# frankyeh/UNet-Studio

Measured on AMD Instinct MI355X. Metric: voxels/sec 3D U-Net train step @128^3 bf16, higher is better.
Workload: dtype bf16

## Files before the change

include/unet.hpp:

```cpp
#ifndef UNET_HPP
#define UNET_HPP
#ifdef QT_CORE_LIB
    #undef slots
#endif
#include <torch/torch.h>
#ifdef QT_CORE_LIB
    #define slots Q_SLOTS
#endif
#include <array>
#include <deque>
#include <map>
#include <mutex>
#include <string>
#include <vector>

#if __has_include("TIPL/tipl.hpp")
#include "TIPL/tipl.hpp"
namespace unet_types { typedef tipl::vector<3> vector3; typedef tipl::shape<3> shape3; }
#else
namespace unet_types {
struct vector3 {
    float v[3];
    vector3(float x = 1.f, float y = 1.f, float z = 1.f) : v{x, y, z} {}
    float& operator[](size_t i) { return v[i]; }
    const float& operator[](size_t i) const { return v[i]; }
};
struct shape3 {
    unsigned v[3];
    shape3(unsigned x = 0, unsigned y = 0, unsigned z = 0) : v{x, y, z} {}
    unsigned& operator[](size_t i) { return v[i]; }
    const unsigned& operator[](size_t i) const { return v[i]; }
    size_t size() const { return (size_t)v[0] * v[1] * v[2]; }
};
inline std::ostream& operator<<(std::ostream& o, const vector3& a) { return o << a[0] << " " << a[1] << " " << a[2]; }
inline std::ostream& operator<<(std::ostream& o, const shape3& a) { return o << a[0] << " " << a[1] << " " << a[2]; }
}
#endif

struct unet_plan;
struct unet_comm;

struct UNet3dImpl : torch::nn::Module
{
public:
    int in_count = 1;
    int out_count = 1;
    std::string architecture,preproc,postproc,orientation,fov_strategy,error_msg;
public:
    std::shared_ptr<torch::optim::SGD> optimizer;

    std::vector<float> testing_errors,training_errors;
    std::vector<unsigned int> single_component_label;
    mutable std::mutex error_mutex;
    auto get_training_errors(void) const
    {
        std::scoped_lock<std::mutex> lock(error_mutex);
        return std::vector<float>(training_errors);
    }
    auto get_testing_errors(void) const
    {
        std::scoped_lock<std::mutex> lock(error_mutex);
        return std::vector<float>(testing_errors);
    }

public:
    unet_types::vector3 voxel_size = {1.0f,1.0f,1.0f};
    unet_types::shape3 dim = {192,224,192};
    std::deque<torch::nn::Sequential> encoding,decoding,decoding_tail;
    std::vector<torch::nn::Sequential> output;
    int create_layer(torch::nn::Sequential& layers,const std::string& def, int in_c);
public:
    std::string get_info(void) const;
public:
    UNet3dImpl(void){}
    UNet3dImpl(int32_t in_count_,int32_t out_count_,std::string);
    ~UNet3dImpl(void);
    void copy_from(const UNet3dImpl& r);
    void add_gradient_from(const UNet3dImpl& r);
    void create_optimizer(float learning_rate);
public:
    std::vector<torch::Tensor> forward(torch::Tensor inputTensor);

    void set_requires_grad(bool req)
    {
        for (auto& p : parameters())
            p.set_requires_grad(req);
    }
    virtual void train(bool on = true) override
    {
        set_requires_grad(on);
        torch::nn::Module::train(on);
    }
    void print_layers(void);
    torch::Device device(void) const
    {
        return parameters().size() && parameters()[0].defined() ? parameters()[0].device() : torch::kCPU;
    }
    void prepare_for_inference(const torch::Device& device);

public:
    size_t pooled_workspaces(void) const;
    int engine_dtype = 1;
    torch::Tensor flat_params, flat_grads;
    void to_device(const torch::Device& device);
    torch::Tensor loss_and_backward(torch::Tensor input, torch::Tensor target_int64, bool ce, bool dice, bool mse, int collapse_before = 0);
    void sgd_step(float lr, float grad_scale, float clip_norm = 12.0f);
    void bind_optimizer_state(void);
    bool save_optimizer(const std::string& file_name);
    bool load_optimizer(const std::string& file_name);
    void attach_comm(struct unet_comm* comm) { comm_ = comm; reduced_from_ = -1; }
    void broadcast_parameters(int root = 0);
    void broadcast_buffers(int root = 0);
    void allreduce_gradients(void);
    torch::Tensor loss_and_backward_overlapped(torch::Tensor input, torch::Tensor target_int64, bool ce, bool dice, bool mse, int collapse_before = 0);
private:
    friend struct UNetForwardFn;
    std::vector<torch::Tensor> params_, buffers_;
    std::map<std::array<int64_t,3>, unet_plan*> plans_;
    struct WorkspacePool;
    std::shared_ptr<WorkspacePool> ws_pool_;
    std::mutex plans_mutex_;
    torch::Tensor trigger_, momentum_, scratch_;
    struct unet_comm* comm_ = nullptr;
    int64_t reduced_from_ = -1;
    unet_plan* plan_for(int64_t d,int64_t h,int64_t w);
    torch::Tensor workspace_for(unet_plan* plan);
    void bind_views(void);
    void ensure_flat(void);
    void rebind_grads(void);
    std::vector<torch::Tensor> run_forward(unet_plan* plan, torch::Tensor ws, torch::Tensor x, int mode);
    void run_backward(unet_plan* plan, torch::Tensor ws, const std::vector<torch::Tensor>& grad_outs);
};
TORCH_MODULE_IMPL(UNet3d, UNet3dImpl);

bool save_to_file(UNet3d& model,const char* file_name);
bool load_from_file(UNet3d& model,const char* file_name);


#endif
```

include/unet_hip.h:

```cpp
#ifndef UNET_HIP_H
#define UNET_HIP_H
#include <stddef.h>
#include <stdint.h>

#ifdef __cplusplus
extern "C" {
#endif

#define UNET_DTYPE_F32 0
#define UNET_DTYPE_BF16 1

#define UNET_IMPL_AUTO 0
#define UNET_IMPL_DIRECT 1

typedef struct unet_plan unet_plan;

const char* unet_last_error(void);
void unet_set_error(const char* msg);

int unet_init(int* n_devices);
int unet_device_info(int device, char* name, size_t name_len, size_t* total_mem, int* compute_units, int* gcn_arch_is_gfx950);

int unet_plan_create(const char* arch_dsl, int in_c, int out_c, int D, int H, int W, int dtype, int device, int impl,
                     unet_plan** out);
void unet_plan_destroy(unet_plan* plan);

int unet_plan_param_count(const unet_plan* plan, int* n);
int unet_plan_param_shape(const unet_plan* plan, int i, int64_t dims[5], int* ndim);
int unet_plan_param_name(const unet_plan* plan, int i, char* name, size_t name_len);
int unet_plan_param_decay(const unet_plan* plan, int i, int* decay);
int unet_plan_param_fan_in(const unet_plan* plan, int i, int64_t* fan_in, int* is_norm_weight);
int unet_plan_buffer_count(const unet_plan* plan, int* n);
int unet_plan_buffer_shape(const unet_plan* plan, int i, int64_t* numel);
int unet_plan_output_count(const unet_plan* plan, int* n);
int unet_plan_output_shape(const unet_plan* plan, int level, int64_t dims[5]);
int unet_plan_workspace_bytes(const unet_plan* plan, size_t* bytes);
int unet_plan_flops(const unet_plan* plan, double* fwd, double* bwd);
size_t unet_plan_describe(const unet_plan* plan, char* buf, size_t len);

int unet_plan_op_count(const unet_plan* plan, int* n);
int unet_plan_op_info(const unet_plan* plan, int i, int* kind, int* cin, int* cout, int* ks, int* stride, int64_t in_dims[3],
                      int64_t out_dims[3], char* name, size_t name_len);

#define UNET_PROF_CONV_FWD 0
#define UNET_PROF_DGRAD 1
#define UNET_PROF_WGRAD 2
#define UNET_PROF_NORM_FWD 3
#define UNET_PROF_NORM_BWD 4
#define UNET_PROF_OTHER 5
int unet_profile_begin(void);
int unet_profile_end(int max_records, int* op_index, int* category, float* ms, int* n_records);

#define UNET_MODE_PACKS_CURRENT 2
int unet_forward(const unet_plan* plan, const float* const* params, float* const* buffers, const float* x,
                 float* const* outs, void* workspace, int mode, void* stream);

int unet_backward(const unet_plan* plan, const float* const* params, const float* const* grad_outs,
                  float* const* grad_params, float* grad_x, void* workspace, void* stream);

int unet_plan_backward_buckets(const unet_plan* plan, int max_buckets, int* n_buckets, int* op_lo, int64_t* elem_lo);
int unet_backward_part(const unet_plan* plan, const float* const* params, const float* const* grad_outs, float* const* grad_params,
                       float* grad_x, void* workspace, int op_hi, int op_lo, void* stream);

int unet_loss_scratch_bytes(const unet_plan* plan, size_t* bytes);
int unet_loss(const unet_plan* plan, const float* const* outs, const int64_t* target, int cost_mask, int collapse_before,
              float* const* grad_outs, float* losses_out, void* scratch, void* stream);

int unet_forward_loss(const unet_plan* plan, const float* const* params, float* const* buffers, const float* x, float* const* outs,
                      const int64_t* target, int cost_mask, int collapse_before, float* const* grad_outs, float* losses_out,
                      void* loss_scratch, void* workspace, void* stream);
int unet_forward_loss_mode(const unet_plan* plan, const float* const* params, float* const* buffers, const float* x, float* const* outs,
                           const int64_t* target, int cost_mask, int collapse_before, float* const* grad_outs, float* losses_out,
                           void* loss_scratch, void* workspace, int mode, void* stream);

int unet_stream_create_cu_range(int device, int cu_first, int cu_count, void** stream);
int unet_stream_destroy(void* stream);
int unet_plan_side_cu_range(unet_plan* plan, int cu_first, int cu_count);

int unet_pack_filters(const unet_plan* plan, const float* const* params, void* workspace, int with_dgrad, int* made, void* stream);

#define UNET_SUM_MAX_BUFFERS 64
int unet_sum_buffers(const float* const* bufs, int n, float* out, int64_t count, int zero_inputs, void* stream);

int unet_sgd_step(const unet_plan* plan, float* params_flat, float* grads_flat, float* momentum_flat, float lr,
                  float momentum, int nesterov, float weight_decay, float clip_norm, float grad_scale, float* norm_out,
                  void* scratch, void* stream);

int unet_op_scratch_bytes(int cin, int cout, int D, int H, int W, size_t* bytes);
int unet_op_conv3d_fwd(int dtype, int impl, const void* x, const float* w, const float* b, void* y, int cin, int cout, int D,
                       int H, int W, int ks, int stride, void* scratch, void* stream);
int unet_op_conv3d_fwd_fused(int dtype, int impl, const void* x, const float* scale, const float* shift, int act, const float* w,
                             const float* b, void* y, float* stats, int cin, int cout, int D, int H, int W, int ks, int stride,
                             void* scratch, void* stream);
int unet_op_conv3d_pack(int dtype, const float* w, void* wpacked, int cin, int cout, int D, int H, int W, int ks, int stride,
                        void* stream);
int unet_op_conv3d_fwd_packed(int dtype, const void* x, const void* wpacked, const float* b, void* y, float* stats_partials,
                              int cin, int cout, int D, int H, int W, int ks, int stride, void* stream);
int unet_op_conv3d_bwd_data(int dtype, int impl, const void* dy, const float* w, void* dx, int cin, int cout, int D, int H,
                            int W, int ks, int stride, void* scratch, void* stream);
int unet_op_conv3d_fwd_norm(const void* x0, const void* x1, int cin0, int cin1, const float* w, const float* b, const float* gamma,
                            const float* beta, double eps, float* rm, float* rv, double momentum, int use_running, int act, void* y,
                            void* y_act, float* stat, int cout, int D, int H, int W, int stride, void* scratch, void* stream);
int unet_op_conv3d_bwd_data_norm(int transposed, const void* dy, const float* w, void* dx, int accumulate, const void* u, const float* stat,
                                 const float* gamma, int act, float* coef, float* dgamma, float* dbeta, int cin, int cout, int D, int H,
                                 int W, void* scratch, void* stream);
int unet_op_conv3d_bwd_weight(int dtype, int impl, const void* x, const void* dy, float* dw, float* db, int cin, int cout,
                              int D, int H, int W, int ks, int stride, void* scratch, void* stream);
int unet_op_convt_fwd(int dtype, int impl, const void* x, const float* w, const float* b, void* y, int cin, int cout, int D,
                      int H, int W, void* scratch, void* stream);
int unet_op_convt_bwd_data(int dtype, int impl, const void* dy, const float* w, void* dx, int cin, int cout, int D, int H,
                           int W, void* scratch, void* stream);
int unet_op_convt_bwd_weight(int dtype, int impl, const void* x, const void* dy, float* dw, float* db, int cin, int cout,
                             int D, int H, int W, void* scratch, void* stream);
int unet_op_pack_ndhwc(int dtype, const float* x_ncdhw, void* y_ndhwc, int C, int64_t S, void* stream);
int unet_op_unpack_ncdhw(int dtype, const void* x_ndhwc, float* y_ncdhw, int C, int64_t S, void* stream);

#define UNET_COMM_ID_BYTES 128
typedef struct unet_comm unet_comm;
int unet_comm_unique_id(void* id_bytes );
int unet_comm_create(int rank, int world, const void* id_bytes, int device, unet_comm** out);
int unet_comm_create_all(int n, const int* devices, unet_comm** out );
int unet_comm_destroy(unet_comm* comm);
int unet_comm_rank(const unet_comm* comm, int* rank, int* world);
int unet_allreduce_grads(unet_comm* comm, float* flat, int64_t elem_lo, int64_t elem_hi, void* stream);
int unet_allreduce_grads_all(unet_comm* const* comms, int n, float* const* flats, int64_t elem_lo, int64_t elem_hi, void* const* streams);
int unet_comm_broadcast(unet_comm* comm, float* buf, int64_t n, int root, void* stream);
int unet_comm_join(unet_comm* comm, void* stream);

#ifdef __cplusplus
}
#endif
#endif
```

unet-studio_amd/csrc/engine.cpp:

```cpp
#include <hip/hip_runtime.h>

#include <algorithm>
#include <atomic>
#include <cmath>
#include <cstdio>
#include <cstring>
#include <functional>
#include <stdexcept>
#include <string>
#include <mutex>
#include <random>
#include <unordered_map>
#include <vector>

#include "../../include/unet_hip.h"
#include "conv_select.h"
#include "graph.hpp"
#include "kernels.h"

using namespace unet;

namespace {

thread_local std::string g_err;
int fail(const std::string& m) { g_err = m; return 1; }

#define HIP_OK(expr)                                                                              \
    do {                                                                                          \
        hipError_t e_ = (expr);                                                                   \
        if (e_ != hipSuccess) throw std::runtime_error(std::string(#expr) + ": " + hipGetErrorString(e_)); \
    } while (0)

struct DeviceGuard {
    int prev = -1;
    explicit DeviceGuard(int dev) {
        HIP_OK(hipGetDevice(&prev));
        if (prev != dev) HIP_OK(hipSetDevice(dev));
        else prev = -1;
    }
    ~DeviceGuard() { if (prev >= 0) (void)hipSetDevice(prev); }
};

size_t align_up(size_t v, size_t a = 256) { return (v + a - 1) / a * a; }

struct EnvSwitches {
    bool no_side_stream = getenv("UNET_NO_SIDE_STREAM"), no_first_wgrad_fuse = getenv("UNET_NO_FIRST_WGRAD_FUSE"), op_polite = getenv("UNET_OP_POLITE");
};
const EnvSwitches& env() { static const EnvSwitches e; return e; }

struct ProfRec { int op, cat; hipEvent_t e0, e1; };
struct ProfSink { std::vector<ProfRec> recs; };
thread_local ProfSink* g_prof = nullptr;
struct ProfScope {
    ProfRec r{};
    hipStream_t s = nullptr;
    bool on = false;
    ProfScope(int op, int cat, hipStream_t st) {
        if (!g_prof) return;
        on = true; s = st; r.op = op; r.cat = cat;
        if (hipEventCreate(&r.e0) != hipSuccess || hipEventCreate(&r.e1) != hipSuccess) { on = false; return; }
        (void)hipEventRecord(r.e0, s);
    }
    ~ProfScope() {
        if (!on) return;
        (void)hipEventRecord(r.e1, s);
        g_prof->recs.push_back(r);
    }
};

}

struct unet_plan {
    Graph g;
    int dtype = 0, device = 0, impl = 0;
    size_t elsize = 4;
    std::vector<size_t> t_off, g_off;
    std::vector<size_t> a_off;
    std::vector<size_t> n_stat, n_coef;
    std::vector<size_t> w_fwd, w_dgrad;
    std::vector<size_t> wm_fwd, wm_dgrad;
    std::vector<int> n_consumers;
    std::vector<int> first_consumer;
    mutable std::mutex bn_mu;
    mutable std::unordered_map<const void*, std::pair<int, int>> bn_pending;
    mutable std::unordered_map<const void*, std::vector<int>> bn_done;
    std::vector<ConvChoice> conv;
    size_t wgrad_off = 0;
    std::vector<size_t> wz_off;
    std::vector<int> wz_job_of_op;
    std::vector<WgradReduceJob> wz_jobs;
    WgradReduceJob* wz_jobs_dev = nullptr;
    size_t partial_off = 0, partial_bytes = 0;
    size_t ws_bytes = 0;
    size_t loss_bytes = 0;
    std::vector<int64_t> p_off;
    std::vector<PackJob> pack_jobs;
    int64_t pack_blocks = 0;
    PackJob* jobs_dev = nullptr;
    SgdSeg* segs_dev = nullptr;
    int nseg = 0;
    int64_t n_param_elems = 0;

    hipStream_t side = nullptr;
    hipEvent_t ev_fork = nullptr, ev_join = nullptr, ev_pack = nullptr, ev_packd = nullptr;
    int pack_split_op = 0;
    int64_t pack_split_blocks = 0, pack_fwd_blocks = 0;
    size_t head_off = 0;
    size_t deep_part_off = 0, deep_part_bytes = 0, deep_cnt_off = 0;
    static constexpr int deep_ncnt = 4096;
    std::vector<size_t> head_op_off;

    ~unet_plan() {
        if (segs_dev) (void)hipFree(segs_dev);
        if (wz_jobs_dev) (void)hipFree(wz_jobs_dev);
        if (jobs_dev) (void)hipFree(jobs_dev);
        if (ev_fork) (void)hipEventDestroy(ev_fork);
        if (ev_join) (void)hipEventDestroy(ev_join);
        if (ev_pack) (void)hipEventDestroy(ev_pack);
        if (ev_packd) (void)hipEventDestroy(ev_packd);
        if (side) (void)hipStreamDestroy(side);
    }

    ConvGeom op_geom_of(const Op& op) const {
        const Tensor& a = g.tensors[op.src[0]];
        const Tensor& o = g.tensors[op.dst];
        ConvGeom cg;
        cg.Cin = op.cin; cg.Cout = op.cout; cg.D = a.D; cg.H = a.H; cg.W = a.W; cg.Do = o.D; cg.Ho = o.H; cg.Wo = o.W;
        cg.ks = op.ks; cg.stride = op.stride;
        return cg;
    }
    void src_chans(const Op& op, SrcDesc* sd) const {
        for (int k = 0; k < op.nsrc; ++k) sd[k].C = g.tensors[op.src[k]].C;
    }
    std::vector<int> side_polite;
    std::vector<char> wgrad_on_main;
    void choose_polite() {
        side_polite.assign(g.ops.size(), 0);
        wgrad_on_main.assign(g.ops.size(), 0);
        bool first = true, any_deep = false;
        for (size_t i = 0; i < g.ops.size(); ++i) {
            const Op& op = g.ops[i];
            if (op.kind != OP_CONV && op.kind != OP_CONVT) continue;
            if (g.tensors[op.dst].voxels() <= (int64_t)32 * 32 * 32) { any_deep = true; break; }
            if (!first && op.kind == OP_CONV && op.stride == 2) wgrad_on_main[i] = 1;
            first = false;
        }
        if (!any_deep) return;
        for (size_t i = 0; i < g.ops.size(); ++i) {
            const Op& op = g.ops[i];
            if (op.kind == OP_CONV || op.kind == OP_CONVT) side_polite[i] = wgrad_on_main[i] ? 0 : 1;
        }
    }

    bool head_only(size_t t) const {
        if (dtype != UNET_DTYPE_BF16 || g.tensors[t].norm < 0 || g.tensors[t].C % 16) return false;
        int readers = 0;
        for (size_t i = 0; i < g.ops.size(); ++i) {
            const Op& op = g.ops[i];
            if (op.kind == OP_NORM) continue;
            for (int k = 0; k < op.nsrc; ++k) {
                if (op.src[k] != (int)t) continue;
                if (conv[i].fwd != Fwd::head) return false;
                ++readers;
            }
        }
        return readers > 0;
    }
    void layout() {
        choose_polite();
        conv.assign(g.ops.size(), ConvChoice());
        for (size_t i = 0; i < g.ops.size(); ++i) {
            const Op& op = g.ops[i];
            if (op.kind != OP_CONV && op.kind != OP_CONVT) continue;
            SrcDesc sd[2];
            src_chans(op, sd);
            conv[i] = choose_conv(dtype, impl, op_geom_of(op), sd, op.nsrc, op.out_level >= 0, op.kind == OP_CONVT);
        }
        size_t off = 0;
        auto take = [&](size_t bytes) { size_t o = off; off = align_up(off + bytes); return o; };
        t_off.assign(g.tensors.size(), SIZE_MAX);
        g_off.assign(g.tensors.size(), SIZE_MAX);
        n_consumers.assign(g.tensors.size(), 0);
        first_consumer.assign(g.tensors.size(), -1);
        for (size_t oi = 0; oi < g.ops.size(); ++oi) {
            const Op& op = g.ops[oi];
            for (int k = 0; k < op.nsrc && op.kind != OP_NORM; ++k)
                if (op.src[k] >= 0) { ++n_consumers[op.src[k]]; if (first_consumer[op.src[k]] < 0) first_consumer[op.src[k]] = (int)oi; }
        }
        a_off.assign(g.tensors.size(), SIZE_MAX);
        for (size_t i = 0; i < g.tensors.size(); ++i) {
            t_off[i] = take((size_t)g.tensors[i].numel() * elsize);
            if (g.tensors[i].needs_grad) g_off[i] = take((size_t)g.tensors[i].numel() * elsize);
            if (impl == UNET_IMPL_AUTO && (g.tensors[i].norm >= 0 || g.tensors[i].act != ACT_NONE) && !head_only(i))
                a_off[i] = take((size_t)g.tensors[i].numel() * elsize);
        }
        n_stat.resize(g.norms.size()); n_coef.resize(g.norms.size());
        size_t pmax = 0;
        for (size_t i = 0; i < g.norms.size(); ++i) {
            n_stat[i] = take(4 * (size_t)g.norms[i].C * 4);
            n_coef[i] = take(3 * (size_t)g.norms[i].C * 4);
            size_t pb = (size_t)stats_blocks(g.tensors[g.norms[i].tensor].voxels()) * g.norms[i].C * 2 * (dtype == UNET_DTYPE_F32 ? 8 : 4);
            if (pb > pmax) pmax = pb;
        }
        w_fwd.assign(g.ops.size(), SIZE_MAX); w_dgrad.assign(g.ops.size(), SIZE_MAX);
        wm_fwd.assign(g.ops.size(), SIZE_MAX); wm_dgrad.assign(g.ops.size(), SIZE_MAX);
        auto grow = [](size_t& m, size_t b) { if (b > m) m = b; };
        for (size_t i = 0; i < g.ops.size(); ++i) {
            const Op& op = g.ops[i];
            if (op.kind != OP_CONV && op.kind != OP_CONVT) continue;
            const ConvChoice& c = conv[i];
            const ConvGeom cg = op_geom_of(op);
            int k3 = op.kind == OP_CONV ? op.ks * op.ks * op.ks : 8;
            w_fwd[i] = take((size_t)k3 * op.cin * round_up(op.cout, 8) * 4);
            w_dgrad[i] = take((size_t)k3 * op.cout * round_up(op.cin, 8) * 4);
            if (op.kind == OP_CONVT) {
                if (c.mfma_fwd()) { wm_fwd[i] = take(mfma_convt_w_bytes(cg)); wm_dgrad[i] = take(mfma_convt_dgrad_w_bytes(cg)); }
                continue;
            }
            const bool stats = g.tensors[op.dst].norm >= 0;
            SrcDesc sd[2];
            src_chans(op, sd);
            if (c.mfma_fwd()) {
                wm_fwd[i] = take(mfma_conv_w_bytes(cg));
                if (stats) grow(pmax, (size_t)mfma_conv_blocks(cg) * op.cout * 2 * 4);
            }
            if (c.fwd == Fwd::first_f32_mfma && stats) grow(pmax, (size_t)conv_first_f32_mfma_blocks(cg) * op.cout * 2 * 8);
            if (c.fwd == Fwd::f32_mfma && stats) grow(pmax, (size_t)conv_f32_mfma_stat_rows(cg, sd) * op.cout * 2 * 8);
            if (c.dgrad == Dgrad::mfma) {
                wm_dgrad[i] = take(mfma_conv_dgrad_w_bytes(cg));
                if (op.stride == 2) grow(pmax, (size_t)s2_conv_dgrad_rows_max() * op.cin * 2 * 4);
            }
        }
        partial_bytes = pmax ? pmax : 256;
        partial_off = take(partial_bytes);
        size_t wmax = 0, hmax = 0;
        for (size_t i = 0; i < g.ops.size(); ++i) {
            const Op& op = g.ops[i];
            if (op.kind != OP_CONV && op.kind != OP_CONVT) continue;
            const ConvChoice& c = conv[i];
            const ConvGeom cg = op_geom_of(op);
            grow(wmax, wgrad_direct_scratch_bytes(cg, op.kind == OP_CONVT));
            if (op.kind == OP_CONVT) {
                if (c.wgrad == Wgrad::mfma) {
                    grow(wmax, mfma_convt_wgrad_scratch_bytes(cg));
                    grow(wmax, bias_grad_scratch_bytes(cg.Cout, (int64_t)cg.Do * cg.Ho * cg.Wo));
                }
                continue;
            }
            if (c.wgrad == Wgrad::mfma) grow(wmax, mfma_wgrad_scratch_bytes(cg, side_polite[i]));
            if (c.wgrad == Wgrad::f32_mfma) grow(wmax, wgrad_f32_mfma_scratch_bytes(cg));
            if (wgrad_small_supported(cg, op.nsrc)) grow(wmax, wgrad_small_scratch_bytes(cg));
            if (cg.Cin == 1 && (cg.Cout == 16 || cg.Cout == 32)) grow(wmax, conv_first_wgrad_mfma_scratch_bytes(cg));
            if (head_supported(cg, op.nsrc)) grow(hmax, head_bwd_scratch_bytes(cg));
        }
        wgrad_off = take(wmax ? wmax : 256);
        head_off = take(hmax ? hmax : 256);
        if (dtype == UNET_DTYPE_BF16 && impl == UNET_IMPL_AUTO) {
            deep_part_bytes = (size_t)8 << 20;
            deep_part_off = take(deep_part_bytes);
            deep_cnt_off = take((size_t)deep_ncnt * 4);
        }
        head_op_off.assign(g.ops.size(), SIZE_MAX);
        for (size_t i = 0; i < g.ops.size(); ++i)
            if (conv[i].fwd == Fwd::head) head_op_off[i] = take(head_bwd_scratch_bytes(op_geom_of(g.ops[i])));
        wz_off.assign(g.ops.size(), SIZE_MAX);
        for (size_t i = 0; i < g.ops.size(); ++i) {
            const Op& op = g.ops[i];
            const Wgrad w = conv[i].wgrad;
            if (op.out_level >= 0 || (w != Wgrad::first_mfma && w != Wgrad::mfma)) continue;
            const ConvGeom cg = op_geom_of(op);
            if (w == Wgrad::first_mfma) wz_off[i] = take(conv_first_wgrad_mfma_scratch_bytes(cg));
            else if (op.kind == OP_CONV) { if (!mfma_conv_wgrad_direct(cg)) wz_off[i] = take(mfma_wgrad_scratch_bytes(cg, side_polite[i])); }
            else if (!mfma_convt_wgrad_direct(cg)) wz_off[i] = take(mfma_convt_wgrad_scratch_bytes(cg));
        }
        ws_bytes = off;
        p_off.assign(g.params.size() + 1, 0);
        for (size_t i = 0; i < g.params.size(); ++i) {
            int64_t n = 1;
            for (auto d : g.params[i].shape) n *= d;
            p_off[i + 1] = p_off[i] + n;
        }
        wz_jobs.clear();
        wz_job_of_op.assign(g.ops.size(), -1);
        int wz_blk = 0;
        for (size_t i = 0; i < g.ops.size(); ++i) {
            if (wz_off[i] == SIZE_MAX) continue;
            const Op& op = g.ops[i];
            ConvGeom cg = op_geom_of(op);
            WgradReduceJob j;
            j.op = (int)i;
            j.slab_off = (long long)(wz_off[i] / 4);
            j.dw_off = p_off[op.weight];
            j.Cb = op.cout;
            if (op.kind == OP_CONVT) {
                j.nsplit = mfma_convt_wgrad_splits(cg);
                j.n = (long long)8 * op.cin * op.cout;
                j.bias_off = op.bias >= 0 ? j.slab_off + (long long)j.nsplit * j.n : -1;
                j.db_off = op.bias >= 0 ? p_off[op.bias] : -1;
            } else {
                j.nsplit = conv[i].wgrad == Wgrad::first_mfma ? conv_first_wgrad_splits(cg) : mfma_conv_wgrad_splits(cg, side_polite[i]);
                j.n = (long long)27 * op.cin * op.cout;
                j.bias_off = op.bias >= 0 ? j.slab_off + (long long)j.nsplit * j.n : -1;
                j.db_off = op.bias >= 0 ? p_off[op.bias] : -1;
            }
            wz_blk += wgrad_reduce_job_blocks(j, wz_blk);
            wz_job_of_op[i] = (int)wz_jobs.size();
            wz_jobs.push_back(j);
        }
        pack_jobs.clear();
        pack_blocks = 0;
        pack_split_op = -1; pack_split_blocks = 0; pack_fwd_blocks = 0;
        for (int which = 0; which < 2; ++which) {
            for (size_t i = 0; i < g.ops.size(); ++i) {
                const Op& op = g.ops[i];
                if (!conv[i].mfma_fwd()) continue;
                if (which == 0 && pack_split_op < 0 && g.tensors[op.dst].voxels() <= (int64_t)16 * 16 * 16) { pack_split_op = (int)i; pack_split_blocks = pack_blocks; }
                PackJob jb[2];
                int n = op.kind == OP_CONV ? mfma_conv_pack_jobs(op_geom_of(op), conv[i].dgrad == Dgrad::mfma, jb) : mfma_convt_pack_jobs(op_geom_of(op), jb);
                if (which >= n) continue;
                jb[which].src_off = p_off[op.weight];
                jb[which].dst_off = (int64_t)(which == 0 ? wm_fwd[i] : wm_dgrad[i]);
                jb[which].blk0 = pack_blocks;
                pack_blocks += jb[which].total;
                pack_jobs.push_back(jb[which]);
            }
            if (which == 0) pack_fwd_blocks = pack_blocks;
        }
    }
};

namespace {

void norm_fwd_passes(int dtype, const void* raw, int C, int64_t S, float* partial, int rows, bool dbl, bool eval, const float* gamma,
                     const float* beta, double eps, float* stat, float* rm, float* rv, int act, void* act_out, hipStream_t s) {
    if (eval) launch_norm_eval(C, gamma, beta, rm, rv, eps, stat, s);
    else {
        if (!rows) {
            launch_stats_partial(dtype, raw, C, S, partial, s);
            rows = stats_blocks(S);
            dbl = dtype == UNET_DTYPE_F32;
        }
        if (!dbl && act_out && launch_norm_finalize_apply(dtype, partial, rows, C, S, gamma, beta, eps, stat, rm, rv, 0.1, raw, act, act_out, s))
            return;
        launch_norm_finalize(partial, rows, C, S, gamma, beta, eps, stat, rm, rv, 0.1, s, dbl);
    }
    if (act_out) {
        SrcDesc d;
        d.ptr = raw; d.C = C; d.act = act; d.scale = stat + 2 * C; d.shift = stat + 3 * C;
        launch_apply_view(dtype, d, act_out, S, s);
    }
}
void norm_bwd_passes(int dtype, void* g, const void* u, int C, int64_t S, const float* stat, int act, const float* gamma, float* coef,
                     float* dgamma, float* dbeta, float* partial, int rows, bool no_apply, hipStream_t s) {
    if (rows <= 0) {
        launch_norm_bwd_partial(dtype, g, u, C, S, stat, act, partial, s);
        rows = stats_blocks(S);
    }
    if (!no_apply && launch_norm_bwd_finalize_apply(dtype, partial, rows, C, S, gamma, stat, coef, dgamma, dbeta, g, u, act, s)) return;
    launch_norm_bwd_finalize(partial, rows, C, S, gamma, stat, coef, dgamma, dbeta, s, dtype == UNET_DTYPE_F32);
    if (!no_apply) launch_norm_bwd_apply(dtype, g, u, C, S, stat, coef, act, s);
}

struct Exec {
    const unet_plan& p;
    char* ws;
    hipStream_t s;
    bool deep_on = false;
    Exec(const unet_plan& plan, void* workspace, void* stream) : p(plan), ws((char*)workspace), s((hipStream_t)stream) {}
    DeepScratch deep() const {
        DeepScratch d;
        if (deep_on && p.deep_part_bytes) { d.part = (float*)(ws + p.deep_part_off); d.part_bytes = p.deep_part_bytes; d.cnt = (int*)(ws + p.deep_cnt_off); d.ncnt = p.deep_ncnt; }
        return d;
    }
    int* deep_cnt() const { return p.deep_part_bytes ? (int*)(ws + p.deep_cnt_off) : nullptr; }

    void* tptr(int t) const { return ws + p.t_off[t]; }
    void* gptr(int t) const { return p.g_off[t] == SIZE_MAX ? nullptr : ws + p.g_off[t]; }
    float* stat(int n) const { return (float*)(ws + p.n_stat[n]); }
    float* coef(int n) const { return (float*)(ws + p.n_coef[n]); }
    float* partial() const { return (float*)(ws + p.partial_off); }

    SrcDesc raw_src(int t) const {
        const Tensor& T = p.g.tensors[t];
        SrcDesc d;
        d.ptr = tptr(t); d.C = T.C; d.act = T.act;
        if (T.norm >= 0) { d.scale = stat(T.norm) + 2 * T.C; d.shift = stat(T.norm) + 3 * T.C; }
        return d;
    }
    SrcDesc src(int t) const {
        if (p.a_off[t] == SIZE_MAX) return raw_src(t);
        SrcDesc d;
        d.ptr = ws + p.a_off[t]; d.C = p.g.tensors[t].C;
        return d;
    }
    void apply_view(int t) const {
        if (p.a_off[t] != SIZE_MAX) launch_apply_view(p.dtype, raw_src(t), ws + p.a_off[t], p.g.tensors[t].voxels(), s);
    }
    ConvGeom geom(const Op& op) const { return p.op_geom_of(op); }

    void forward(const float* const* params, float* const* buffers, const float* x, float* const* outs, int mode,
                 const std::function<void(int)>* on_head = nullptr) {
        const Graph& g = p.g;
        const bool packs_current = (mode & UNET_MODE_PACKS_CURRENT) != 0;
        mode &= 1;
        std::vector<int> fused_blocks(g.norms.size(), 0);
        std::vector<char> fused_dbl(g.norms.size(), 0);
        std::vector<char> fused_done(g.norms.size(), 0);
        bool packed = false, pack_pending = false, pack2_pending = false;
        if (p.jobs_dev && packs_current) { packed = true; deep_on = true; }
        else if (p.jobs_dev) {
            bool flat = true;
            for (size_t i = 0; i < g.params.size() && flat; ++i) flat = params[i] == params[0] + p.p_off[i];
            if (flat) {
                const int njobs = (int)p.pack_jobs.size();
                if (mode == 1 && p.side && !env().no_side_stream && !g_prof) {
                    HIP_OK(hipEventRecord(p.ev_fork, s));
                    HIP_OK(hipStreamWaitEvent(p.side, p.ev_fork, 0));
                    if (p.pack_split_op > 0 && p.pack_split_blocks > 0) {
                        launch_mfma_pack_batched(params[0], ws, p.jobs_dev, njobs, p.pack_split_blocks, p.side, 0, 0, deep_cnt(), p.deep_ncnt);
                        HIP_OK(hipEventRecord(p.ev_join, p.side));
                        launch_mfma_pack_batched(params[0], ws, p.jobs_dev, njobs, p.pack_fwd_blocks - p.pack_split_blocks, p.side, p.pack_split_blocks);
                        HIP_OK(hipEventRecord(p.ev_pack, p.side));
                        pack2_pending = true;
                        launch_mfma_pack_batched(params[0], ws, p.jobs_dev, njobs, p.pack_blocks - p.pack_fwd_blocks, p.side, p.pack_fwd_blocks);
                        HIP_OK(hipEventRecord(p.ev_packd, p.side));
                    } else {
                        launch_mfma_pack_batched(params[0], ws, p.jobs_dev, njobs, p.pack_blocks, p.side, 0, 0, deep_cnt(), p.deep_ncnt);
                        HIP_OK(hipEventRecord(p.ev_join, p.side));
                    }
                    pack_pending = true;
                } else {
                    ProfScope ps(-1, UNET_PROF_OTHER, s);
                    launch_mfma_pack_batched(params[0], ws, p.jobs_dev, njobs, mode == 1 ? p.pack_blocks : p.pack_fwd_blocks, s, 0, 0, deep_cnt(), p.deep_ncnt);
                }
                packed = true;
                deep_on = true;
            }
        }
        auto need_packs = [&](int op_index = 1 << 30) {
            if (pack_pending) { HIP_OK(hipStreamWaitEvent(s, p.ev_join, 0)); pack_pending = false; }
            if (pack2_pending && op_index >= p.pack_split_op) { HIP_OK(hipStreamWaitEvent(s, p.ev_pack, 0)); pack2_pending = false; }
        };
        for (size_t i = 0; i < g.ops.size(); ++i) {
            const Op& op = g.ops[i];
            ProfScope ps((int)i, (op.kind == OP_CONV || op.kind == OP_CONVT) ? UNET_PROF_CONV_FWD : op.kind == OP_NORM ? UNET_PROF_NORM_FWD : UNET_PROF_OTHER, s);
            switch (op.kind) {
                case OP_PACK_INPUT:
                    launch_pack_input(p.dtype, x, tptr(op.dst), g.in_c, g.tensors[op.dst].voxels(), s);
                    break;
                case OP_CONV:
                case OP_CONVT: {
                    if (op.out_level >= 0 && !(outs && outs[op.out_level])) break;
                    SrcDesc sd[2] = {src(op.src[0]), op.nsrc > 1 ? src(op.src[1]) : SrcDesc()};
                    ConvGeom cg = geom(op);
                    float* wf = (float*)(ws + p.w_fwd[i]);
                    float* wd = (float*)(ws + p.w_dgrad[i]);
                    const int k3 = op.ks * op.ks * op.ks;
                    const ConvChoice& c = p.conv[i];
                    const Tensor& T = g.tensors[op.dst];
                    const bool want_stats = T.norm >= 0 && !(g.norms[T.norm].batch && mode == 0);
                    if (op.kind == OP_CONVT) {
                        if (c.mfma_fwd()) {
                            need_packs((int)i);
                            if (!packed) launch_mfma_pack_convt_w(params[op.weight], ws + p.wm_fwd[i], mode == 1 ? ws + p.wm_dgrad[i] : nullptr, cg, s);
                            if (!(deep_on && launch_deep_convt_fwd(cg, sd, op.nsrc, ws + p.wm_fwd[i], params[op.bias], tptr(op.dst), deep(), s)))
                                launch_mfma_convt_fwd(cg, sd, op.nsrc, ws + p.wm_fwd[i], params[op.bias], tptr(op.dst), s);
                            break;
                        }
                        if (!packs_current) launch_pack_convt_w(params[op.weight], wf, wd, op.cin, op.cout, s);
                        if (c.fwd == Fwd::f32_mfma) launch_convt_f32_mfma(cg, sd, wf, params[op.bias], (float*)tptr(op.dst), s);
                        else launch_convt_fwd_direct(p.dtype, cg, sd, op.nsrc, wf, params[op.bias], tptr(op.dst), s);
                        break;
                    }
                    float* const part = want_stats ? partial() : nullptr;
                    int rows = 0;
                    switch (c.fwd) {
                        case Fwd::deep:
                        case Fwd::mfma:
                            need_packs((int)i);
                            if (!packed)
// ... 278 lines not shown
                            if (can) {
                                const Norm& n = g.norms[Ts.norm];
                                nb = {tptr(ts), stat(Ts.norm), params[n.gamma], coef(Ts.norm), gparams[n.gamma], gparams[n.beta], Ts.act};
                            }
                            if (op.kind == OP_CONVT) {
                                int norm_done = 0;
                                if (deep_on && launch_deep_convt_dgrad(cg, gptr(t), ws + p.wm_dgrad[i], dg, op.nsrc, can ? &nb : nullptr, deep(), &norm_done, s)) {
                                    if (norm_done) { std::lock_guard<std::mutex> lk(p.bn_mu); p.bn_done[ws].push_back(ts); }
                                } else
                                    launch_mfma_convt_dgrad(cg, gptr(t), ws + p.wm_dgrad[i], dg, op.nsrc, s);
                                break;
                            }
                            BnBwdStats bn = {tptr(ts), Ts.norm >= 0 ? stat(Ts.norm) : nullptr, partial(), Ts.act, Ts.C};
                            int rows = 0;
                            const int served = deep_on ? launch_deep_conv_dgrad(cg, gptr(t), ws + p.wm_dgrad[i], dg, op.nsrc, can ? &nb : nullptr, deep(), s) : 0;
                            if (served == 2) { std::lock_guard<std::mutex> lk(p.bn_mu); p.bn_done[ws].push_back(ts); }
                            if (!served) rows = launch_mfma_conv_dgrad(cg, gptr(t), ws + p.wm_dgrad[i], dg, op.nsrc, s, can ? &bn : nullptr);
                            if (rows > 0) { std::lock_guard<std::mutex> lk(p.bn_mu); p.bn_pending[ws] = {ts, rows}; }
                            break;
                        }
                        case Dgrad::f32_mfma: launch_conv_f32_mfma_dgrad(cg, (const float*)gptr(t), wd, dg, op.nsrc, s); break;
                        case Dgrad::direct:
                            if (op.kind == OP_CONVT) launch_convt_dgrad_direct(p.dtype, cg, gptr(t), wd, dg, op.nsrc, s);
                            else launch_conv_dgrad_direct(p.dtype, cg, gptr(t), wd, dg, op.nsrc, s);
                            break;
                    }
                    if (any) mark(op);
                    break;
                }
                case OP_MATERIALIZE: {
                    DstGrad dg[2] = {dst_of(op.src[0]), op.nsrc > 1 ? dst_of(op.src[1]) : DstGrad()};
                    if (dg[0].ptr || (op.nsrc > 1 && dg[1].ptr)) {
                        if (!dry) launch_materialize_bwd(p.dtype, gptr(t), dg, op.nsrc, g.tensors[t].voxels(), s);
                        mark(op);
                    }
                    break;
                }
                case OP_MAXPOOL: {
                    const Tensor& a = g.tensors[op.src[0]];
                    DstGrad d = dst_of(op.src[0]);
                    if (d.ptr) { if (!dry) launch_maxpool_bwd(p.dtype, src(op.src[0]), gptr(t), d, a.D, a.H, a.W, s); mark(op); }
                    break;
                }
                case OP_UPSAMPLE: {
                    const Tensor& a = g.tensors[op.src[0]];
                    DstGrad d = dst_of(op.src[0]);
                    if (d.ptr) { if (!dry) launch_upsample_bwd(p.dtype, gptr(t), d, a.D, a.H, a.W, s); mark(op); }
                    break;
                }
                case OP_PACK_INPUT:
                    if (!dry && (grad_x)) launch_unpack_ncdhw(p.dtype, gptr(t), grad_x, g.in_c, g.tensors[t].voxels(), s);
                    break;
                default: break;
            }
        }
        pending.insert(pending.begin(), held.begin(), held.end());
        held.clear();
        issue_pending();
        flush_wz(sb);
        if (sb != s) {
            HIP_OK(hipEventRecord(p.ev_join, sb));
            HIP_OK(hipStreamWaitEvent(s, p.ev_join, 0));
        }
    }
};

void check_launch() { HIP_OK(hipGetLastError()); }

}

extern "C" {

const char* unet_last_error(void) { return g_err.c_str(); }
void unet_set_error(const char* msg) { g_err = msg ? msg : ""; }

int unet_init(int* n_devices) {
    int n = 0;
    hipError_t e = hipGetDeviceCount(&n);
    if (e != hipSuccess) { if (n_devices) *n_devices = 0; return fail(std::string("hipGetDeviceCount: ") + hipGetErrorString(e)); }
    if (n_devices) *n_devices = n;
    return 0;
}

int unet_device_info(int device, char* name, size_t name_len, size_t* total_mem, int* compute_units, int* is_gfx950) {
    hipDeviceProp_t pr;
    hipError_t e = hipGetDeviceProperties(&pr, device);
    if (e != hipSuccess) return fail(std::string("hipGetDeviceProperties: ") + hipGetErrorString(e));
    if (name && name_len) { std::strncpy(name, pr.name, name_len - 1); name[name_len - 1] = 0; }
    if (total_mem) *total_mem = pr.totalGlobalMem;
    if (compute_units) *compute_units = pr.multiProcessorCount;
    if (is_gfx950) *is_gfx950 = std::strncmp(pr.gcnArchName, "gfx950", 6) == 0;
    return 0;
}

static bool create_cu_range_stream(int device, int cu_first, int cu_count, hipStream_t* out);
int unet_plan_create(const char* arch, int in_c, int out_c, int D, int H, int W, int dtype, int device, int impl, unet_plan** out) {
    if (!arch || !out) return fail("unet_plan_create: null argument");
    if (dtype != UNET_DTYPE_F32 && dtype != UNET_DTYPE_BF16) return fail("unet_plan_create: unknown dtype");
    unet_plan* p = nullptr;
    try {
        p = new unet_plan();
        p->g = Graph::build(arch, in_c, out_c, D, H, W);
        for (auto& n : p->g.norms) p->g.tensors[n.tensor].needs_grad = true;
        p->dtype = dtype; p->device = device; p->impl = impl; p->elsize = dtype == UNET_DTYPE_F32 ? 4 : 2;
        p->layout();
        {
            size_t off = 0;
            int oc = out_c;
            for (size_t l = 0; l < p->g.outputs.size(); ++l) {
                const auto& o = p->g.outputs[l];
                int64_t S = (int64_t)(D >> l) * (H >> l) * (W >> l);
                if (S <= 0) S = 1;
                off = align_up(off + (size_t)S * 8);
                off = align_up(off + (size_t)(4 + 2 * oc) * 4);
                (void)o;
            }
            off = align_up(off + (size_t)1024 * (3 + 2 * oc) * 4);
            off = align_up(off + (size_t)1024 * (3 + 2 * oc) * 4);
            p->loss_bytes = off;
        }
        std::vector<SgdSeg> segs;
        int64_t o = 0;
        for (auto& pr : p->g.params) {
            int64_t n = 1;
            for (auto d : pr.shape) n *= d;
            SgdSeg sg;
            sg.offset = o; sg.count = n; sg.wd = pr.decay ? 1.f : 0.f;
            segs.push_back(sg);
            o += n;
        }
        p->n_param_elems = o;
        p->nseg = (int)segs.size();
        int nd = 0;
        if (hipGetDeviceCount(&nd) == hipSuccess && nd > 0) {
            DeviceGuard dg(device);
            int pr_least = 0, pr_greatest = 0;
            (void)hipDeviceGetStreamPriorityRange(&pr_least, &pr_greatest);
            HIP_OK(hipStreamCreateWithPriority(&p->side, hipStreamNonBlocking, pr_least));
            const unsigned evf = hipEventDisableTiming | hipEventDisableSystemFence;
            HIP_OK(hipEventCreateWithFlags(&p->ev_fork, evf));
            HIP_OK(hipEventCreateWithFlags(&p->ev_join, evf));
            HIP_OK(hipEventCreateWithFlags(&p->ev_pack, evf));
            HIP_OK(hipEventCreateWithFlags(&p->ev_packd, evf));
            HIP_OK(hipMalloc((void**)&p->segs_dev, segs.size() * sizeof(SgdSeg)));
            HIP_OK(hipMemcpy(p->segs_dev, segs.data(), segs.size() * sizeof(SgdSeg), hipMemcpyHostToDevice));
            if (!p->wz_jobs.empty()) {
                HIP_OK(hipMalloc((void**)&p->wz_jobs_dev, p->wz_jobs.size() * sizeof(WgradReduceJob)));
                HIP_OK(hipMemcpy(p->wz_jobs_dev, p->wz_jobs.data(), p->wz_jobs.size() * sizeof(WgradReduceJob), hipMemcpyHostToDevice));
            }
            if (!p->pack_jobs.empty()) {
                HIP_OK(hipMalloc((void**)&p->jobs_dev, p->pack_jobs.size() * sizeof(PackJob)));
                HIP_OK(hipMemcpy(p->jobs_dev, p->pack_jobs.data(), p->pack_jobs.size() * sizeof(PackJob), hipMemcpyHostToDevice));
            }
        }
        *out = p;
        return 0;
    } catch (const std::exception& e) {
        delete p;
        return fail(e.what());
    }
}

void unet_plan_destroy(unet_plan* p) { delete p; }

int unet_plan_param_count(const unet_plan* p, int* n) { *n = (int)p->g.params.size(); return 0; }
int unet_plan_param_shape(const unet_plan* p, int i, int64_t dims[5], int* ndim) {
    if (i < 0 || i >= (int)p->g.params.size()) return fail("parameter index out of range");
    const auto& s = p->g.params[i].shape;
    *ndim = (int)s.size();
    for (size_t k = 0; k < s.size(); ++k) dims[k] = s[k];
    return 0;
}
int unet_plan_param_name(const unet_plan* p, int i, char* name, size_t name_len) {
    if (i < 0 || i >= (int)p->g.params.size()) return fail("parameter index out of range");
    if (name && name_len) { std::strncpy(name, p->g.params[i].name.c_str(), name_len - 1); name[name_len - 1] = 0; }
    return 0;
}
int unet_plan_param_decay(const unet_plan* p, int i, int* decay) {
    if (i < 0 || i >= (int)p->g.params.size()) return fail("parameter index out of range");
    *decay = p->g.params[i].decay;
    return 0;
}
int unet_plan_param_fan_in(const unet_plan* p, int i, int64_t* fan_in, int* is_norm_weight) {
    if (i < 0 || i >= (int)p->g.params.size()) return fail("parameter index out of range");
    *fan_in = p->g.params[i].fan_in; *is_norm_weight = p->g.params[i].norm_weight;
    return 0;
}
int unet_plan_buffer_count(const unet_plan* p, int* n) { *n = (int)p->g.buffers.size(); return 0; }
int unet_plan_buffer_shape(const unet_plan* p, int i, int64_t* numel) {
    if (i < 0 || i >= (int)p->g.buffers.size()) return fail("buffer index out of range");
    *numel = p->g.buffers[i];
    return 0;
}
int unet_plan_output_count(const unet_plan* p, int* n) { *n = (int)p->g.outputs.size(); return 0; }
int unet_plan_output_shape(const unet_plan* p, int l, int64_t dims[5]) {
    if (l < 0 || l >= (int)p->g.outputs.size()) return fail("output level out of range");
    const auto& o = p->g.outputs[l];
    dims[0] = 1; dims[1] = o.C; dims[2] = o.D; dims[3] = o.H; dims[4] = o.W;
    return 0;
}
int unet_plan_workspace_bytes(const unet_plan* p, size_t* bytes) { *bytes = p->ws_bytes; return 0; }
int unet_plan_flops(const unet_plan* p, double* fwd, double* bwd) { *fwd = p->g.flops_fwd; *bwd = p->g.flops_bwd; return 0; }
size_t unet_plan_describe(const unet_plan* p, char* buf, size_t len) {
    std::string d = p->g.describe();
    if (buf && len) { std::strncpy(buf, d.c_str(), len - 1); buf[len - 1] = 0; }
    return d.size() + 1;
}

int unet_forward(const unet_plan* p, const float* const* params, float* const* buffers, const float* x, float* const* outs,
                 void* workspace, int mode, void* stream) {
    try {
        if (!p || !params || !x || !workspace) throw std::runtime_error("unet_forward: null argument");
        if (mode & ~(1 | UNET_MODE_PACKS_CURRENT)) throw std::runtime_error("unet_forward: unknown mode bits (0 = eval, 1 = train, optionally | UNET_MODE_PACKS_CURRENT)");
        if (!p->g.buffers.empty() && !buffers) throw std::runtime_error("unet_forward: architecture has bnorm layers but buffers is null");
        DeviceGuard dg(p->device);
        Exec ex(*p, workspace, stream);
        ex.forward(params, buffers, x, outs, mode);
        check_launch();
        return 0;
    } catch (const std::exception& e) { return fail(e.what()); }
}

int unet_backward(const unet_plan* p, const float* const* params, const float* const* grad_outs, float* const* grad_params,
                  float* grad_x, void* workspace, void* stream) {
    try {
        if (!p || !params || !grad_params || !workspace) throw std::runtime_error("unet_backward: null argument");
        if (grad_x) throw std::runtime_error("unet_backward: grad_x must be NULL -- dL/dx is not computed (the input carries no gradient, as in train.cpp:619-628)");
        DeviceGuard dg(p->device);
        Exec ex(*p, workspace, stream);
        ex.backward(params, grad_outs, grad_params, grad_x);
        check_launch();
        return 0;
    } catch (const std::exception& e) { return fail(e.what()); }
}

int unet_backward_part(const unet_plan* p, const float* const* params, const float* const* grad_outs, float* const* grad_params,
                       float* grad_x, void* workspace, int op_hi, int op_lo, void* stream) {
    try {
        if (!p || !params || !grad_params || !workspace) throw std::runtime_error("unet_backward_part: null argument");
        if (op_lo < 0 || op_hi < op_lo) throw std::runtime_error("unet_backward_part: invalid op range");
        if (grad_x) throw std::runtime_error("unet_backward_part: grad_x must be NULL -- dL/dx is not computed");
        DeviceGuard dg(p->device);
        Exec ex(*p, workspace, stream);
        ex.backward(params, grad_outs, grad_params, grad_x, op_hi, op_lo);
        check_launch();
        return 0;
    } catch (const std::exception& e) { return fail(e.what()); }
}

int unet_plan_backward_buckets(const unet_plan* p, int max_buckets, int* n_buckets, int* op_lo, int64_t* elem_lo) {
    try {
        if (!p || !n_buckets || !op_lo || !elem_lo || max_buckets < 1) throw std::runtime_error("unet_plan_backward_buckets: bad argument");
        const Graph& g = p->g;
        const int nops = (int)g.ops.size();
        std::vector<int64_t> first(nops, INT64_MAX);
        bool monotone = true;
        int64_t prev = -1;
        for (int i = 0; i < nops; ++i) {
            const Op& op = g.ops[i];
            if (op.kind != OP_CONV && op.kind != OP_CONVT) continue;
            int64_t f = p->p_off[op.weight];
            if (op.bias >= 0 && p->p_off[op.bias] < f) f = p->p_off[op.bias];
            first[i] = f;
            if (f <= prev) monotone = false;
            prev = f;
            const Tensor& T = g.tensors[op.dst];
            if (T.norm >= 0) {
                const Norm& n = g.norms[T.norm];
                if (p->p_off[n.gamma] < f || p->p_off[n.beta] < f) monotone = false;
            }
        }
        int nb = 0;
        if (monotone && max_buckets > 1) {
            const double thr = (double)p->n_param_elems / ((double)max_buckets - 0.5);
            int64_t hi = p->n_param_elems;
            for (int i = nops - 1; i > 0 && nb < max_buckets - 1; --i) {
                if (first[i] == INT64_MAX) continue;
                if ((double)(hi - first[i]) >= thr) { op_lo[nb] = i; elem_lo[nb] = first[i]; hi = first[i]; ++nb; }
            }
        }
        op_lo[nb] = 0; elem_lo[nb] = 0; ++nb;
        *n_buckets = nb;
        return 0;
    } catch (const std::exception& e) { return fail(e.what()); }
}

int unet_plan_op_count(const unet_plan* p, int* n) { *n = (int)p->g.ops.size(); return 0; }
int unet_plan_op_info(const unet_plan* p, int i, int* kind, int* cin, int* cout, int* ks, int* stride, int64_t in_dims[3],
                      int64_t out_dims[3], char* name, size_t name_len) {
    if (i < 0 || i >= (int)p->g.ops.size()) return fail("op index out of range");
    const Op& op = p->g.ops[i];
    if (kind) *kind = (int)op.kind;
    if (cin) *cin = op.cin;
    if (cout) *cout = op.cout;
    if (ks) *ks = op.ks;
    if (stride) *stride = op.stride;
    const Tensor* a = op.nsrc > 0 && op.src[0] >= 0 ? &p->g.tensors[op.src[0]] : nullptr;
    const Tensor* o = op.dst >= 0 ? &p->g.tensors[op.dst] : nullptr;
    if (in_dims) { in_dims[0] = a ? a->D : 0; in_dims[1] = a ? a->H : 0; in_dims[2] = a ? a->W : 0; }
    if (out_dims) { out_dims[0] = o ? o->D : 0; out_dims[1] = o ? o->H : 0; out_dims[2] = o ? o->W : 0; }
    if (name && name_len) { std::strncpy(name, op.name.c_str(), name_len - 1); name[name_len - 1] = 0; }
    return 0;
}

int unet_profile_begin(void) {
    if (g_prof) return fail("unet_profile_begin: a profile is already open on this thread");
// ... 90 lines not shown
int unet_loss(const unet_plan* p, const float* const* outs, const int64_t* target, int cost_mask, int collapse_before,
              float* const* grad_outs, float* losses_out, void* scratch, void* stream) {
    try {
        LossRun lr(p, outs, target, cost_mask, collapse_before, grad_outs, losses_out, scratch);
        DeviceGuard dg(p->device);
        hipStream_t s = (hipStream_t)stream;
        lr.prepare(s);
        for (size_t k = 0; k < lr.levels(); ++k) { lr.level_partial(k, 0, s); lr.level_finish(k, 0, s); }
        check_launch();
        return 0;
    } catch (const std::exception& e) { return fail(e.what()); }
}

int unet_forward_loss(const unet_plan* p, const float* const* params, float* const* buffers, const float* x, float* const* outs,
                      const int64_t* target, int cost_mask, int collapse_before, float* const* grad_outs, float* losses_out,
                      void* loss_scratch, void* workspace, void* stream) {
    return unet_forward_loss_mode(p, params, buffers, x, outs, target, cost_mask, collapse_before, grad_outs, losses_out, loss_scratch, workspace, 1,
                                  stream);
}

int unet_forward_loss_mode(const unet_plan* p, const float* const* params, float* const* buffers, const float* x, float* const* outs,
                           const int64_t* target, int cost_mask, int collapse_before, float* const* grad_outs, float* losses_out,
                           void* loss_scratch, void* workspace, int mode, void* stream) {
    try {
        if ((mode & 1) != 1 || (mode & ~(1 | UNET_MODE_PACKS_CURRENT)))
            throw std::runtime_error("unet_forward_loss_mode: mode must be 1 (train), optionally | UNET_MODE_PACKS_CURRENT");
        if (!p || !params || !x || !workspace || !outs) throw std::runtime_error("unet_forward_loss: null argument");
        if (!p->g.buffers.empty() && !buffers) throw std::runtime_error("unet_forward_loss: architecture has bnorm layers but buffers is null");
        LossRun lr(p, outs, target, cost_mask, collapse_before, grad_outs, losses_out, loss_scratch);
        DeviceGuard dg(p->device);
        hipStream_t s = (hipStream_t)stream;
        const bool side = p->side && !env().no_side_stream && !g_prof;
        Exec ex(*p, workspace, stream);
        if (!side) {
            ex.forward(params, buffers, x, outs, mode);
            lr.prepare(s);
            for (size_t k = 0; k < lr.levels(); ++k) { lr.level_partial(k, 0, s); lr.level_finish(k, 0, s); }
            check_launch();
            return 0;
        }
        hipStream_t sd = p->side;
        bool prepared = false;
        constexpr bool per_level = false;
        std::function<void(int)> on_head = [&](int level) {
            if (level < 1 || (size_t)level >= lr.levels()) return;
            if (!per_level && level != 1) return;
            HIP_OK(hipEventRecord(p->ev_fork, s));
            HIP_OK(hipStreamWaitEvent(sd, p->ev_fork, 0));
            if (!prepared) { lr.prepare(sd); prepared = true; }
            for (size_t k = per_level ? (size_t)level : lr.levels() - 1; k >= (size_t)level; --k) {
                lr.level_partial(k, 1, sd);
                lr.level_finish(k, 1, sd);
            }
        };
        ex.forward(params, buffers, x, outs, mode, &on_head);
        if (!prepared) {
            HIP_OK(hipEventRecord(p->ev_fork, s));
            HIP_OK(hipStreamWaitEvent(sd, p->ev_fork, 0));
            lr.prepare(sd);
        }
        lr.level_partial(0, 0, s);
        HIP_OK(hipEventRecord(p->ev_join, sd));
        HIP_OK(hipStreamWaitEvent(s, p->ev_join, 0));
        lr.level_finish(0, 0, s);
        check_launch();
        return 0;
    } catch (const std::exception& e) { return fail(e.what()); }
}

static bool create_cu_range_stream(int device, int cu_first, int cu_count, hipStream_t* out) {
    hipDeviceProp_t prop;
    if (cu_count <= 0 || hipGetDeviceProperties(&prop, device) != hipSuccess || prop.multiProcessorCount % 8 != 0) return false;
    const int per_xcd = prop.multiProcessorCount / 8;
    if (cu_count >= per_xcd) return false;
    std::vector<uint32_t> mask((prop.multiProcessorCount + 31) / 32, 0u);
    for (int c = 0; c < cu_count; ++c) {
        const int cu = ((cu_first + c) % per_xcd + per_xcd) % per_xcd;
        for (int x = 0; x < 8; ++x) { const int bit = cu * 8 + x; mask[bit / 32] |= 1u << (bit % 32); }
    }
    if (hipExtStreamCreateWithCUMask(out, (uint32_t)mask.size(), mask.data()) != hipSuccess) { (void)hipGetLastError(); return false; }
    return true;
}

int unet_stream_create_cu_range(int device, int cu_first, int cu_count, void** stream) {
    try {
        if (!stream) throw std::runtime_error("unet_stream_create_cu_range: null argument");
        DeviceGuard dg(device);
        hipStream_t st = nullptr;
        if (!create_cu_range_stream(device, cu_first, cu_count, &st)) throw std::runtime_error("unet_stream_create_cu_range: the device / driver does not take this CU range");
        *stream = (void*)st;
        return 0;
    } catch (const std::exception& e) { return fail(e.what()); }
}
int unet_stream_destroy(void* stream) {
    if (stream && hipStreamDestroy((hipStream_t)stream) != hipSuccess) return fail("hipStreamDestroy failed");
    return 0;
}
int unet_plan_side_cu_range(unet_plan* p, int cu_first, int cu_count) {
    try {
        if (!p) throw std::runtime_error("unet_plan_side_cu_range: null plan");
        if (!p->side) return 0;
        DeviceGuard dg(p->device);
        hipStream_t st = nullptr;
        if (!create_cu_range_stream(p->device, cu_first, cu_count, &st)) throw std::runtime_error("unet_plan_side_cu_range: the device / driver does not take this CU range");
        HIP_OK(hipStreamSynchronize(p->side));
        HIP_OK(hipStreamDestroy(p->side));
        p->side = st;
        return 0;
    } catch (const std::exception& e) { return fail(e.what()); }
}

int unet_pack_filters(const unet_plan* p, const float* const* params, void* workspace, int with_dgrad, int* made, void* stream) {
    try {
        if (!p || !params || !workspace || !made) throw std::runtime_error("unet_pack_filters: null argument");
        *made = 0;
        if (!p->jobs_dev || p->pack_jobs.empty()) return 0;
        for (size_t i = 0; i < p->g.params.size(); ++i)
            if (params[i] != params[0] + p->p_off[i]) return 0;
        DeviceGuard dg(p->device);
        launch_mfma_pack_batched(params[0], workspace, p->jobs_dev, (int)p->pack_jobs.size(), with_dgrad ? p->pack_blocks : p->pack_fwd_blocks,
                                 (hipStream_t)stream, 0, 0, p->deep_part_bytes ? (int*)((char*)workspace + p->deep_cnt_off) : nullptr, p->deep_ncnt);
        check_launch();
        *made = 1;
        return 0;
    } catch (const std::exception& e) { return fail(e.what()); }
}

int unet_sum_buffers(const float* const* bufs, int n, float* out, int64_t count, int zero_inputs, void* stream) {
    try {
        if (!bufs || !out || n < 1 || n > UNET_SUM_MAX_BUFFERS || count < 0) throw std::runtime_error("unet_sum_buffers: bad argument");
        for (int k = 0; k < n; ++k)
            if (!bufs[k] || (reinterpret_cast<uintptr_t>(bufs[k]) & 15)) throw std::runtime_error("unet_sum_buffers: null or misaligned buffer");
        if (reinterpret_cast<uintptr_t>(out) & 15) throw std::runtime_error("unet_sum_buffers: misaligned output");
        if (count == 0) return 0;
        launch_sum_buffers(bufs, n, out, count, zero_inputs, (hipStream_t)stream);
        check_launch();
        return 0;
    } catch (const std::exception& e) { return fail(e.what()); }
}

int unet_sgd_step(const unet_plan* p, float* params, float* grads, float* mom, float lr, float momentum, int nesterov, float wd,
                  float clip_norm, float grad_scale, float* norm_out, void* scratch, void* stream) {
    try {
        if (!p || !params || !grads || !mom || !scratch) throw std::runtime_error("unet_sgd_step: null argument");
        if (!p->segs_dev) throw std::runtime_error("unet_sgd_step: plan was created without a device");
        DeviceGuard dg(p->device);
        hipStream_t s = (hipStream_t)stream;
        const int nblk = 1024;
        float* partial = (float*)scratch;
        launch_sumsq_partial(grads, p->n_param_elems, grad_scale, partial, nblk, s);
        launch_sgd(params, grads, mom, p->n_param_elems, p->segs_dev, p->nseg, partial, nblk, lr, momentum, nesterov, wd, clip_norm,
                   grad_scale, norm_out, s);
        check_launch();
        return 0;
    } catch (const std::exception& e) { return fail(e.what()); }
}

struct OpScratch {
    size_t half, pack, partials;
    OpScratch(int cin, int cout)
        : half(align_up((size_t)27 * round_up(cin, 8) * round_up(cout, 8) * 4)), pack(2 * half),
          partials(pack + align_up((size_t)160 * round_up(cin, 32) * round_up(cout, 32))) {}
};
int unet_op_scratch_bytes(int cin, int cout, int D, int H, int W, size_t* bytes) {
    size_t b = OpScratch(cin, cout).partials + 4096;
    if (D > 0 && H > 0 && W > 0) {
        int64_t S = (int64_t)D * H * W;
        size_t blocks = (size_t)(S / 32 + 4096);
        b += align_up(blocks * cout * 2 * 8);
    }
    if ((int64_t)cin * cout <= 1024) {
        size_t w = ((size_t)1024 * 1024 + (size_t)1024 * cout) * 4 + 1024;
        if (w > b) b = w;
    }
    if (cout <= 8 || cin == 1) {
        size_t w = (size_t)512 * ((size_t)27 * cin * cout + cout) * 4 + 1024;
        if (w > b) b = w;
    }
    if (cin % 16 == 0 && cout % 16 == 0 && D > 0 && H > 0 && W > 0) {
        ConvGeom g;
        g.Cin = cin; g.Cout = cout; g.D = g.Do = D; g.H = g.Ho = H; g.W = g.Wo = W; g.ks = 3; g.stride = 1;
        b = std::max(b, wgrad_f32_mfma_scratch_bytes(g));
        size_t w = std::max(mfma_wgrad_scratch_bytes(g, 0), mfma_wgrad_scratch_bytes(g, 1));
        if (w > b) b = w;
        g.stride = 2; g.Do = (D - 1) / 2 + 1; g.Ho = (H - 1) / 2 + 1; g.Wo = (W - 1) / 2 + 1;
        w = std::max(mfma_wgrad_scratch_bytes(g, 0), mfma_wgrad_scratch_bytes(g, 1));
        if (w > b) b = w;
        g.Do = 2 * D; g.Ho = 2 * H; g.Wo = 2 * W;
        w = mfma_convt_wgrad_scratch_bytes(g);
        if (w > b) b = w;
    }
    *bytes = b;
    return 0;
}

static ConvGeom op_geom(int cin, int cout, int D, int H, int W, int ks, int stride, bool transposed) {
    ConvGeom g;
    g.Cin = cin; g.Cout = cout; g.D = D; g.H = H; g.W = W; g.ks = ks; g.stride = stride;
    if (transposed) { g.Do = 2 * D; g.Ho = 2 * H; g.Wo = 2 * W; }
    else {
        int pad = (ks - 1) / 2;
        g.Do = (D + 2 * pad - ks) / stride + 1; g.Ho = (H + 2 * pad - ks) / stride + 1; g.Wo = (W + 2 * pad - ks) / stride + 1;
    }
    return g;
}
static void op_pack(const float* w, int cin, int cout, int k3, bool transposed, void* scratch, float** wf, float** wd, hipStream_t s) {
    *wf = (float*)scratch; *wd = (float*)((char*)scratch + OpScratch(cin, cout).half);
    if (transposed) launch_pack_convt_w(w, *wf, *wd, cin, cout, s);
    else launch_pack_conv_w(w, *wf, *wd, cin, cout, k3, s);
}
#define OP_TRY(...) try { __VA_ARGS__; check_launch(); return 0; } catch (const std::exception& e) { return fail(e.what()); }
static DeepScratch op_deep() {
    static std::mutex mu;
    static std::unordered_map<int, DeepScratch> per_dev;
    int dev = 0;
    HIP_OK(hipGetDevice(&dev));
    std::lock_guard<std::mutex> lk(mu);
    auto it = per_dev.find(dev);
    if (it != per_dev.end()) return it->second;
    DeepScratch d;
    d.part_bytes = (size_t)8 << 20; d.ncnt = 4096;
    char* base = nullptr;
    HIP_OK(hipMalloc((void**)&base, d.part_bytes + (size_t)d.ncnt * 4));
    HIP_OK(hipMemset(base + d.part_bytes, 0, (size_t)d.ncnt * 4));
    d.part = (float*)base; d.cnt = (int*)(base + d.part_bytes);
    per_dev[dev] = d;
    return d;
}

int unet_op_conv3d_fwd(int dtype, int impl, const void* x, const float* w, const float* b, void* y, int cin, int cout, int D, int H,
                       int W, int ks, int stride, void* scratch, void* stream) {
    OP_TRY({
        hipStream_t s = (hipStream_t)stream;
        ConvGeom g = op_geom(cin, cout, D, H, W, ks, stride, false);
        float *wf, *wd;
        SrcDesc sd; sd.ptr = x; sd.C = cin;
        const ConvChoice c = choose_conv(dtype, impl, g, &sd, 1, false, false);
        if (c.mfma_fwd()) {
            void* wm = (char*)scratch + OpScratch(cin, cout).pack;
            launch_mfma_pack_conv_w(w, wm, nullptr, g, s);
            if (!launch_deep_conv_fwd(g, &sd, 1, wm, b, y, nullptr, op_deep(), s)) launch_mfma_conv_fwd(g, &sd, 1, wm, b, y, nullptr, s);
        } else if (c.fwd == Fwd::first_mfma) {
            launch_conv_first_mfma(g, &sd, w, b, y, nullptr, s);
        } else if (c.fwd == Fwd::first_f32_mfma) {
            (void)launch_conv_first_f32_mfma(g, &sd, w, b, (float*)y, nullptr, s);
        } else {
            op_pack(w, cin, cout, ks * ks * ks, false, scratch, &wf, &wd, s);
            if (c.fwd == Fwd::f32_mfma) (void)launch_conv_f32_mfma(g, &sd, 1, wf, b, (float*)y, s);
            else launch_conv_fwd_direct(dtype, g, &sd, 1, wf, b, y, nullptr, s);
        }
    })
}
int unet_op_conv3d_fwd_fused(int dtype, int impl, const void* x, const float* scale, const float* shift, int act, const float* w,
                             const float* b, void* y, float* stats, int cin, int cout, int D, int H, int W, int ks, int stride,
                             void* scratch, void* stream) {
    OP_TRY({
        hipStream_t s = (hipStream_t)stream;
        ConvGeom g = op_geom(cin, cout, D, H, W, ks, stride, false);
        float *wf, *wd;
        SrcDesc sd; sd.ptr = x; sd.C = cin; sd.scale = scale; sd.shift = shift; sd.act = act;
        int64_t So = (int64_t)g.Do * g.Ho * g.Wo;
        const OpScratch L(cin, cout);
        float* part = (float*)((char*)scratch + L.partials);
        const ConvChoice c = choose_conv(dtype, impl, g, &sd, 1, false, false);
        if (c.mfma_fwd()) {
            void* wm = (char*)scratch + L.pack;
            launch_mfma_pack_conv_w(w, wm, nullptr, g, s);
            int rows = launch_mfma_conv_fwd(g, &sd, 1, wm, b, y, stats ? part : nullptr, s);
            if (stats) launch_stats_sum(part, rows, cout, stats, s);
        } else if (c.fwd == Fwd::first_mfma) {
            int rows = launch_conv_first_mfma(g, &sd, w, b, y, stats ? part : nullptr, s);
            if (stats) launch_stats_sum(part, rows, cout, stats, s);
        } else {
            op_pack(w, cin, cout, ks * ks * ks, false, scratch, &wf, &wd, s);
            if (c.fwd == Fwd::f32_mfma) {
                const int rows = launch_conv_f32_mfma(g, &sd, 1, wf, b, (float*)y, s, stats ? (double*)part : nullptr);
                if (stats) launch_stats_sum(part, rows, cout, stats, s, true);
            } else {
                launch_conv_fwd_direct(dtype, g, &sd, 1, wf, b, y, nullptr, s);
                if (stats) {
                    launch_stats_partial(dtype, y, cout, So, part, s);
                    launch_stats_sum(part, stats_blocks(So), cout, stats, s, dtype == UNET_DTYPE_F32);
                }
            }
        }
    })
}
int unet_op_conv3d_pack(int dtype, const float* w, void* wpacked, int cin, int cout, int D, int H, int W, int ks, int stride,
                        void* stream) {
    OP_TRY({
        ConvGeom g = op_geom(cin, cout, D, H, W, ks, stride, false);
        SrcDesc sd; sd.C = cin;
        if (!choose_conv(dtype, UNET_IMPL_AUTO, g, &sd, 1, false, false).mfma_fwd())
            throw std::runtime_error("unet_op_conv3d_pack: shape not covered by the MFMA kernels");
        launch_mfma_pack_conv_w(w, wpacked, nullptr, g, (hipStream_t)stream);
    })
}
int unet_op_conv3d_fwd_packed(int dtype, const void* x, const void* wpacked, const float* b, void* y, float* stats_partials,
                              int cin, int cout, int D, int H, int W, int ks, int stride, void* stream) {
    OP_TRY({
        ConvGeom g = op_geom(cin, cout, D, H, W, ks, stride, false);
        SrcDesc sd; sd.ptr = x; sd.C = cin;
        if (!choose_conv(dtype, UNET_IMPL_AUTO, g, &sd, 1, false, false).mfma_fwd())
            throw std::runtime_error("unet_op_conv3d_fwd_packed: shape not covered by the MFMA kernels");
        launch_mfma_conv_fwd(g, &sd, 1, wpacked, b, y, stats_partials, (hipStream_t)stream);
    })
// ... 785 lines not shown
```

unet-studio_amd/csrc/kernels.h:

```cpp
#pragma once
#include <hip/hip_runtime.h>
#include <cstdint>

#include "../../include/unet_atlas.h"
#include "../../include/unet_augment.h"
#include "../../include/unet_components.h"
#include "../../include/unet_distance.h"
#include "../../include/unet_feed.h"
#include "../../include/unet_hip.h"
#include "../../include/unet_postproc.h"
#include "../../include/unet_preproc.h"
#include "../../include/unet_qc.h"
#include "../../include/unet_register.h"
#include "../../include/unet_space.h"
#include "../../include/unet_table.h"
#include "../../include/unet_tiles.h"

namespace unet {

struct SrcDesc {
    const void* ptr = nullptr;
    int C = 0;
    const float* scale = nullptr;
    const float* shift = nullptr;
    int act = 0;
};
struct DstGrad {
    void* ptr = nullptr;
    int C = 0;
    int accumulate = 0;
};

struct ConvGeom {
    int Cin = 0, Cout = 0;
    int D = 0, H = 0, W = 0;
    int Do = 0, Ho = 0, Wo = 0;
    int ks = 3, stride = 1;
};

__host__ __device__ static inline int round_up(int a, int b) { return (a + b - 1) / b * b; }

void launch_pack_conv_w(const float* w, float* w_fwd, float* w_dgrad, int Cin, int Cout, int k3, hipStream_t s);
void launch_pack_convt_w(const float* w, float* w_fwd, float* w_dgrad, int Cin, int Cout, hipStream_t s);

void launch_pack_input(int dtype, const float* x_ncdhw, void* y, int C, int64_t S, hipStream_t s);
void launch_export(int dtype, SrcDesc src, float* y_ncdhw, int64_t S, hipStream_t s);
void launch_import_grad(int dtype, const float* g_ncdhw, void* g, int C, int64_t S, int accumulate, hipStream_t s);

void launch_conv_fwd_direct(int dtype, const ConvGeom& g, const SrcDesc* src, int nsrc, const float* w_fwd, const float* bias,
                            void* out, float* out_ncdhw, hipStream_t s);
void launch_conv_dgrad_direct(int dtype, const ConvGeom& g, const void* dy, const float* w_dgrad, const DstGrad* dst, int ndst,
                              hipStream_t s);
size_t wgrad_direct_scratch_bytes(const ConvGeom& g, int transposed);
void launch_conv_wgrad_direct(int dtype, const ConvGeom& g, const SrcDesc* src, int nsrc, const void* dy, float* dw, float* db,
                              void* scratch, hipStream_t s);
void launch_convt_fwd_direct(int dtype, const ConvGeom& g, const SrcDesc* src, int nsrc, const float* w_fwd, const float* bias,
                             void* out, hipStream_t s);
void launch_convt_dgrad_direct(int dtype, const ConvGeom& g, const void* dy, const float* w_dgrad, const DstGrad* dst, int ndst,
                               hipStream_t s);
void launch_convt_wgrad_direct(int dtype, const ConvGeom& g, const SrcDesc* src, int nsrc, const void* dy, float* dw, float* db,
                               void* scratch, hipStream_t s);

int stats_blocks(int64_t S);
void launch_stats_partial(int dtype, const void* x, int C, int64_t S, float* partial, hipStream_t s);
void launch_norm_finalize(const float* partial, int nblk, int C, int64_t S, const float* gamma, const float* beta, double eps,
                          float* stat, float* running_mean, float* running_var, double momentum, hipStream_t s, bool dbl = false);
void launch_stats_sum(const float* partial, int nblk, int C, float* out, hipStream_t s, bool dbl = false);
void launch_norm_eval(int C, const float* gamma, const float* beta, const float* rm, const float* rv, double eps, float* stat,
                      hipStream_t s);

void launch_act_bwd(int dtype, void* g, const void* u, int act, int64_t n, hipStream_t s);
void launch_norm_bwd_partial(int dtype, void* g, const void* u, int C, int64_t S, const float* stat, int act, float* partial,
                             hipStream_t s);
void launch_norm_bwd_finalize(const float* partial, int nblk, int C, int64_t S, const float* gamma, const float* stat, float* coef,
                              float* dgamma, float* dbeta, hipStream_t s, bool dbl = false);
bool launch_norm_finalize_apply(int dtype, const float* partial, int nblk, int C, int64_t S, const float* gamma, const float* beta, double eps,
                                float* stat, float* running_mean, float* running_var, double momentum, const void* raw, int act, void* out,
                                hipStream_t s);
bool launch_norm_bwd_finalize_apply(int dtype, const float* partial, int nblk, int C, int64_t S, const float* gamma, const float* stat,
                                    float* coef, float* dgamma, float* dbeta, void* g, const void* u, int act, hipStream_t s);
void launch_norm_bwd_apply(int dtype, void* g, const void* u, int C, int64_t S, const float* stat, const float* coef, int act,
                           hipStream_t s);

void launch_maxpool_fwd(int dtype, SrcDesc src, void* out, int D, int H, int W, hipStream_t s);
void launch_maxpool_bwd(int dtype, SrcDesc src, const void* gout, DstGrad dst, int D, int H, int W, hipStream_t s);
void launch_upsample_fwd(int dtype, SrcDesc src, void* out, int D, int H, int W, hipStream_t s);
void launch_upsample_bwd(int dtype, const void* gout, DstGrad dst, int D, int H, int W, hipStream_t s);
void launch_materialize(int dtype, const SrcDesc* src, int nsrc, void* out, int64_t S, hipStream_t s);
void launch_apply_view(int dtype, SrcDesc src, void* out, int64_t S, hipStream_t s);
void launch_materialize_bwd(int dtype, const void* gout, const DstGrad* dst, int ndst, int64_t S, hipStream_t s);
void launch_export_bwd(int dtype, const float* g_ncdhw, DstGrad dst, int64_t S, hipStream_t s);
void launch_unpack_ncdhw(int dtype, const void* g, float* out_ncdhw, int C, int64_t S, hipStream_t s);

void launch_target_half(const int64_t* t, int64_t* o, int D, int H, int W, hipStream_t s);
int loss_blocks(int64_t S);
void launch_loss_partial(const float* logits, const int64_t* target, int C, int64_t S, int collapse, float* partial, hipStream_t s);
void launch_loss_finalize(const float* partial, int nblk, int oc, float level_weight, int cost_mask, float* level_out, float* totals,
                          int set_stats, hipStream_t s);
void launch_loss_grad(const float* logits, const int64_t* target, int C, int64_t S, int collapse, const float* level_out,
                      float level_weight, int cost_mask, float* dlogits, hipStream_t s);

void launch_sum_buffers(const float* const* bufs, int n, float* out, int64_t count, int zero_inputs, hipStream_t s);

struct SgdSeg { int64_t offset, count; float wd; };
void launch_sumsq_partial(const float* g, int64_t n, float scale, float* partial, int nblk, hipStream_t s);
void launch_sgd(float* p, float* g, float* m, int64_t n, const SgdSeg* segs_dev, int nseg, const float* partial, int nblk,
                float lr, float momentum, int nesterov, float weight_decay, float clip_norm, float grad_scale, float* norm_out,
                hipStream_t s);

struct PackJob { int64_t src_off, dst_off, total, blk0; int Ci, Co, CK, T, mode, A, B, pad; };
int mfma_conv_pack_jobs(const ConvGeom& g, bool want_dgrad, PackJob* out2);
int mfma_convt_pack_jobs(const ConvGeom& g, PackJob* out2);
void launch_mfma_pack_batched(const float* params_base, void* ws, const PackJob* jobs_dev, int njobs, int64_t nblocks, hipStream_t s,
                              int64_t blk_base = 0, int max_grid = 0, int* zero = nullptr, int nzero = 0);
bool mfma_conv_fwd_supported(int dtype, const ConvGeom& g, const SrcDesc* src, int nsrc);
size_t mfma_conv_w_bytes(const ConvGeom& g);
void launch_mfma_pack_conv_w(const float* w, void* w_mfma_fwd, void* w_mfma_dgrad, const ConvGeom& g, hipStream_t s);
int launch_mfma_conv_fwd(const ConvGeom& g, const SrcDesc* src, int nsrc, const void* w_mfma, const float* bias, void* out,
                         float* stats_partial, hipStream_t s);
bool conv_first_mfma_supported(int dtype, const ConvGeom& g, const SrcDesc* src, int nsrc);
int conv_first_mfma_blocks(const ConvGeom& g);
int launch_conv_first_mfma(const ConvGeom& g, const SrcDesc* src, const float* w, const float* bias, void* out, float* stats_partial,
                           hipStream_t s);
int mfma_conv_blocks(const ConvGeom& g);
bool mfma_wgrad_z_supported(int dtype, const ConvGeom& g, const SrcDesc* src, int nsrc);
size_t mfma_wgrad_z_scratch_bytes(const ConvGeom& g, int polite = 0);
int mfma_wgrad_z_splits(const ConvGeom& g, int polite = 0);
int launch_mfma_wgrad_z(const ConvGeom& g, const SrcDesc* src, int nsrc, const void* dy, bool want_bias, void* scratch, hipStream_t s,
                        int polite = 0);
void wgrad_reduce(const float* slab, const float* bias_slab, int nsplit, int64_t n, int Cb, float* dw, float* db, hipStream_t s);
struct WgradReduceJob { long long slab_off, bias_off, dw_off, db_off, n; int nsplit, Cb, ly, blk0, nblk, op; };
int wgrad_reduce_job_blocks(WgradReduceJob& j, int blk0);
void launch_wgrad_reduce_batched(const WgradReduceJob* jobs_dev, int job0, int njobs, int blk_base, int nblocks, const void* ws, float* gflat,
                                 hipStream_t s);
bool mfma_wgrad_supported(int dtype, const ConvGeom& g, const SrcDesc* src, int nsrc);
size_t mfma_wgrad_scratch_bytes(const ConvGeom& g, int polite = 0);
int mfma_conv_wgrad_splits(const ConvGeom& g, int polite = 0);
int mfma_convt_wgrad_splits(const ConvGeom& g);
bool mfma_conv_wgrad_direct(const ConvGeom& g);
bool mfma_convt_wgrad_direct(const ConvGeom& g);
int conv_first_wgrad_splits(const ConvGeom& g);
void launch_mfma_conv_wgrad(const ConvGeom& g, const SrcDesc* src, int nsrc, const void* dy, float* dw, float* db, void* scratch,
                            hipStream_t s, bool defer_reduce = false, int polite = 0);
bool head_supported(const ConvGeom& g, int nsrc);
size_t head_bwd_scratch_bytes(const ConvGeom& g);
void launch_head_fwd(int dtype, const ConvGeom& g, const SrcDesc& src, const float* w, const float* bias, void* y, float* out_ncdhw,
                     hipStream_t s);
void launch_head_bwd(int dtype, const ConvGeom& g, const SrcDesc& src, const float* dy_ncdhw, const void* dy_cl, const float* w,
                     DstGrad dst, float* dw, float* db, void* scratch, hipStream_t s, bool defer_reduce = false);
void launch_head_bwd_reduce(const ConvGeom& g, float* dw, float* db, const void* scratch, hipStream_t s);
bool conv_first_wgrad_mfma_supported(int dtype, const ConvGeom& g, const SrcDesc* src, int nsrc);
size_t conv_first_wgrad_mfma_scratch_bytes(const ConvGeom& g);
struct NormBwdFuse { const void* u; const float* stat; const float* coef; int act; };
void launch_conv_first_wgrad_mfma(const ConvGeom& g, const SrcDesc* src, const void* dy, float* dw, float* db, void* scratch, hipStream_t s,
                                  bool defer_reduce = false, const NormBwdFuse* nb_fuse = nullptr);
bool wgrad_small_supported(const ConvGeom& g, int nsrc);
size_t wgrad_small_scratch_bytes(const ConvGeom& g);
void launch_conv_wgrad_small(int dtype, const ConvGeom& g, const SrcDesc* src, int nsrc, const void* dy, float* dw, float* db,
                             void* scratch, hipStream_t s);
bool mfma_convt_wgrad_supported(int dtype, const ConvGeom& g, const SrcDesc* src, int nsrc);
size_t mfma_convt_wgrad_scratch_bytes(const ConvGeom& g);
void launch_mfma_convt_wgrad(const ConvGeom& g, const SrcDesc* src, const void* dy, float* dw, void* scratch, hipStream_t s,
                             bool defer_reduce = false, float* db = nullptr, int polite = 0);
int launch_colsum_partial8(int dtype, const void* x, int C, int64_t S, float* partial, hipStream_t s);
size_t bias_grad_scratch_bytes(int C, int64_t S);
void launch_bias_grad(int dtype, const void* dy, int C, int64_t S, float* db, void* scratch, hipStream_t s);
bool mfma_conv_dgrad_supported(int dtype, const ConvGeom& g, const SrcDesc* src, int nsrc);
size_t mfma_conv_dgrad_w_bytes(const ConvGeom& g);
struct BnBwdStats { const void* u; const float* stat; float* partial; int act, C; };
int launch_mfma_conv_dgrad(const ConvGeom& g, const void* dy, const void* w_mfma_dgrad, const DstGrad* dst, int ndst, hipStream_t s,
                           const BnBwdStats* bn = nullptr);
int launch_s2_conv_fwd(const ConvGeom& g, const SrcDesc* src, int nsrc, const void* w_mfma, const float* bias, void* out, float* stats_partial,
                       hipStream_t s);
int launch_s2_conv_dgrad(const ConvGeom& g, const void* dy, const void* w_s2_dgrad, const DstGrad* dst, int ndst, hipStream_t s,
                         const BnBwdStats* bn);
int s2_conv_dgrad_rows_max();
bool launch_s2_convt_fwd(const ConvGeom& g, const SrcDesc* src, int nsrc, const void* w_mfma, const float* bias, void* out, hipStream_t s);
bool launch_s2_convt_dgrad(const ConvGeom& g, const void* dy, const void* w_mfma_dgrad, const DstGrad* dst, int ndst, hipStream_t s);
int s2_wgrad_splits(int Ca, int Cb, int cD, int cH, int cW);
int launch_s2_wgrad(int ks, const void* fine, const void* fine2, int C0, int Ca, int fD, int fH, int fW, const void* coarse, int Cb, int cD, int cH,
                    int cW, bool want_bias, int bias_from_a, void* scratch, hipStream_t s, int polite);
constexpr int64_t DEEP_MAX_VOXELS = 512;
struct DeepScratch { float* part = nullptr; size_t part_bytes = 0; int* cnt = nullptr; int ncnt = 0; };
struct DeepNormFwd {
    const float* gamma; const float* beta; double eps; float* stat; float* rm; float* rv; double momentum; int use_running; int act;
    void* act_out;
};
struct DeepNormBwd {
    const void* u; const float* stat; const float* gamma; float* coef; float* dgamma; float* dbeta; int act;
};
bool deep_conv_applies(int dtype, int64_t out_voxels, int cin, int cout);
bool launch_deep_conv_fwd(const ConvGeom& g, const SrcDesc* src, int nsrc, const void* w_mfma, const float* bias, void* out,
                          const DeepNormFwd* nf, const DeepScratch& sc, hipStream_t s);
bool launch_deep_convt_fwd(const ConvGeom& g, const SrcDesc* src, int nsrc, const void* w_mfma, const float* bias, void* out,
                           const DeepScratch& sc, hipStream_t s);
int launch_deep_conv_dgrad(const ConvGeom& g, const void* dy, const void* w_mfma_dgrad, const DstGrad* dst, int ndst, const DeepNormBwd* nb,
                           const DeepScratch& sc, hipStream_t s);
bool launch_deep_convt_dgrad(const ConvGeom& g, const void* dy, const void* w_mfma_dgrad, const DstGrad* dst, int ndst, const DeepNormBwd* nb,
                             const DeepScratch& sc, int* norm_done, hipStream_t s);
bool mfma_convt_supported(int dtype, const ConvGeom& g, const SrcDesc* src, int nsrc);
size_t mfma_convt_w_bytes(const ConvGeom& g);
size_t mfma_convt_dgrad_w_bytes(const ConvGeom& g);
void launch_mfma_pack_convt_w(const float* w, void* w_mfma_fwd, void* w_mfma_dgrad, const ConvGeom& g, hipStream_t s);
void launch_mfma_convt_fwd(const ConvGeom& g, const SrcDesc* src, int nsrc, const void* w_mfma, const float* bias, void* out, hipStream_t s);
void launch_mfma_convt_dgrad(const ConvGeom& g, const void* dy, const void* w_mfma_dgrad, const DstGrad* dst, int ndst, hipStream_t s);

bool conv_f32_mfma_supported(int dtype, const ConvGeom& g, const SrcDesc* src, int nsrc);
int conv_f32_mfma_stat_rows(const ConvGeom& g, const SrcDesc* src);
int launch_conv_f32_mfma(const ConvGeom& g, const SrcDesc* src, int nsrc, const float* w_fwd, const float* bias, float* out,
                         hipStream_t s, double* stats_partial = nullptr);
bool conv_first_f32_mfma_supported(int dtype, const ConvGeom& g, const SrcDesc* src, int nsrc);
int conv_first_f32_mfma_blocks(const ConvGeom& g);
int launch_conv_first_f32_mfma(const ConvGeom& g, const SrcDesc* src, const float* w, const float* bias, float* out, double* stats_partial,
                               hipStream_t s);
bool convt_f32_mfma_supported(int dtype, const ConvGeom& g, const SrcDesc* src, int nsrc);
void launch_convt_f32_mfma(const ConvGeom& g, const SrcDesc* src, const float* w_fwd, const float* bias, float* out, hipStream_t s);
bool wgrad_f32_mfma_supported(int dtype, const ConvGeom& g, const SrcDesc* src, int nsrc);
size_t wgrad_f32_mfma_scratch_bytes(const ConvGeom& g);
void launch_wgrad_f32_mfma(const ConvGeom& g, const SrcDesc* src, int nsrc, const float* dy, float* dw, float* db, void* scratch,
                           hipStream_t s);
void slab_reduce_public(const float* slab, int nsplit, int64_t n, float* out, hipStream_t s);
bool conv_f32_mfma_dgrad_supported(int dtype, const ConvGeom& g, const DstGrad* dst, int ndst);
void launch_conv_f32_mfma_dgrad(const ConvGeom& g, const float* dy, const float* w_dgrad, const DstGrad* dst, int ndst, hipStream_t s);

size_t augment_scratch_bytes(const UnetAugmentRecipe& r);
void launch_augment(const UnetAugmentRecipe& r, float* image, float* label, void* scratch, hipStream_t st);
size_t simulate_scratch_bytes(const UnetSimulateRecipe& r);
void launch_simulate_modality(const UnetSimulateRecipe& r, float* t1w, const float* label, void* scratch, hipStream_t st);

size_t qc_scratch_bytes(int out_c, int64_t S, int collapse);
void launch_qc_counts(const float* logits, const float* label, const float* image0, int out_c, int64_t S, int collapse, int shift,
                      uint64_t* counts, void* scratch, hipStream_t s);

size_t feed_scratch_bytes(int64_t S);
void launch_feed_label_max(const float* label, int64_t S, int* out_max, void* scratch, hipStream_t s);
void launch_feed_prepare(const float* image0, float* label, int64_t S, int normalize, int shift, int* label_max, void* scratch,
                         hipStream_t s);
void launch_feed_target(const float* label, int64_t S, int normalize, int64_t* target, void* scratch, hipStream_t s);

size_t postproc_scratch_bytes(int planes, int64_t S);
void launch_postproc_softmax(const float* logits, int C, int64_t S, float thr, float* lp, float* fg, uint16_t* lab, hipStream_t s);
void launch_postproc_argmax_planes(const float* lp, int np, int64_t S, const float* fg, float thr, uint16_t* lab, hipStream_t s);
void launch_postproc_defragment(int W, int H, int D, int each, float thr, double ratio, float* fg, float* lp, int np, uint16_t* lab,
                                void* scratch, hipStream_t s);
void launch_postproc_plane_op(int op, float t, int W, int H, int D, float* lp, int np, void* scratch, hipStream_t s);

int64_t space_bricks(int w, int h, int d);
size_t space_scratch_bytes(int64_t dst_voxels, int channels);
void launch_space_resample(const float* src, int sw, int sh, int sd, float* dst, int dw, int dh, int dd, int channels,
                           const UnetSpaceMap& map, int mode, int normalize, void* scratch, hipStream_t s);
void launch_space_postproc(const float* logits, int C, int mw, int mh, int md, const UnetSpaceMap& map, int nw, int nh, int nd, float thr,
                           float* lp, float* fg, uint16_t* lab, hipStream_t s);

void launch_tiles_blend(const float* tiles, int C, int tw, int th, int td, const UnetTilePlan& plan, int cw, int ch, int cd, float* canvas,
                        hipStream_t s);
void launch_tiles_postproc(const float* tiles, int C, int tw, int th, int td, const UnetTilePlan& plan, int cw, int ch, int cd, float thr,
                           float* lp, float* fg, uint16_t* lab, hipStream_t s);

int64_t preproc_filter_blocks(int w, int h, int d, int channels);
size_t preproc_scratch_bytes(int64_t values);
void launch_preproc_filter(const float* src, float* dst, int w, int h, int d, int channels, int kind, int impl, hipStream_t s);
void launch_preproc_downsample(const float* src, float* dst, int w, int h, int d, int channels, hipStream_t s);
void launch_preproc_upsample(const float* src, float* dst, int w, int h, int d, int channels, hipStream_t s);
// ... 40 lines not shown
```

unet-studio_amd/csrc/kernels_elem.hip:

```cpp
#include "device_util.h"

namespace unet {

template <typename T> __global__ void k_pack_input(const float* __restrict__ x, T* __restrict__ y, int C, int64_t S) {
    int64_t i = (int64_t)blockIdx.x * 256 + threadIdx.x;
    if (i >= S * C) return;
    int c = (int)(i % C); int64_t v = i / C;
    st<T>(y, i, x[(int64_t)c * S + v]);
}
void launch_pack_input(int dtype, const float* x, void* y, int C, int64_t S, hipStream_t s) {
    UNET_DISPATCH(dtype, (k_pack_input<T><<<cdiv64(S * C, 256), 256, 0, s>>>(x, (T*)y, C, S)));
}

template <typename T> __global__ void k_export(SrcDesc src, float* __restrict__ y, int64_t S) {
    int64_t i = (int64_t)blockIdx.x * 256 + threadIdx.x;
    if (i >= S * src.C) return;
    int c = (int)(i / S); int64_t v = i % S;
    y[i] = view_ld<T>(src, v, c);
}
void launch_export(int dtype, SrcDesc src, float* y, int64_t S, hipStream_t s) {
    UNET_DISPATCH(dtype, (k_export<T><<<cdiv64(S * src.C, 256), 256, 0, s>>>(src, y, S)));
}
void launch_unpack_ncdhw(int dtype, const void* g, float* out, int C, int64_t S, hipStream_t s) {
    SrcDesc d;
    d.ptr = g; d.C = C;
    launch_export(dtype, d, out, S, s);
}

template <typename T> __global__ void k_import_grad(const float* __restrict__ g, T* __restrict__ o, int C, int64_t S, int acc) {
    int64_t i = (int64_t)blockIdx.x * 256 + threadIdx.x;
    if (i >= S * C) return;
    int c = (int)(i % C); int64_t v = i / C;
    float val = g[(int64_t)c * S + v];
    if (acc) val += ld<T>(o, i);
    st<T>(o, i, val);
}
void launch_import_grad(int dtype, const float* g, void* o, int C, int64_t S, int accumulate, hipStream_t s) {
    UNET_DISPATCH(dtype, (k_import_grad<T><<<cdiv64(S * C, 256), 256, 0, s>>>(g, (T*)o, C, S, accumulate)));
}
void launch_export_bwd(int dtype, const float* g, DstGrad dst, int64_t S, hipStream_t s) {
    if (!dst.ptr) return;
    launch_import_grad(dtype, g, dst.ptr, dst.C, S, dst.accumulate, s);
}

static inline int64_t stats_vpb(int64_t S) {
    int64_t vpb = (S + 1023) / 1024;
    return vpb < 32 ? 32 : vpb;
}
int stats_blocks(int64_t S) {
    int64_t vpb = stats_vpb(S);
    return (int)((S + vpb - 1) / vpb);
}
static inline int pow2_ge(int c) { int p = 1; while (p < c && p < 256) p <<= 1; return p; }

template <typename T> struct StatAcc { typedef float type; };
template <> struct StatAcc<float> { typedef double type; };

template <typename T, int MODE>
__global__ void __launch_bounds__(256) k_stats_partial(const T* __restrict__ x, T* __restrict__ gbuf, int C, int64_t S, int64_t VPB,
                                                       int CW, const float* __restrict__ stat, int act, float* __restrict__ partial_) {
    typedef typename StatAcc<T>::type A;
    A* partial = (A*)partial_;
    __shared__ A red[2][256];
    int NV = 256 / CW, cl = threadIdx.x % CW, lane = threadIdx.x / CW;
    int64_t v0 = (int64_t)blockIdx.x * VPB, v1 = v0 + VPB < S ? v0 + VPB : S;
    for (int cg = 0; cg < C; cg += CW) {
        int c = cg + cl;
        A s1 = 0, s2 = 0;
        if (c < C) {
            float mean = 0.f, rstd = 1.f, sc = 1.f, sh = 0.f;
            if (MODE == 1) { mean = stat[c]; rstd = stat[C + c]; sc = stat[2 * C + c]; sh = stat[3 * C + c]; }
            for (int64_t v = v0 + lane; v < v1; v += NV) {
                float u = ld<T>(x, v * C + c);
                if (MODE == 0) { s1 += (A)u; s2 += (A)u * (A)u; }
                else {
                    float dv = ld<T>(gbuf, v * C + c) * act_d(fmaf(u, sc, sh), act);
                    s1 += (A)dv; s2 += (A)dv * (A)((u - mean) * rstd);
                }
            }
        }
        red[0][threadIdx.x] = s1; red[1][threadIdx.x] = s2;
        __syncthreads();
        if (lane == 0 && c < C) {
            A a = 0, b = 0;
            for (int l = 0; l < NV; ++l) { a += red[0][l * CW + cl]; b += red[1][l * CW + cl]; }
            partial[((int64_t)blockIdx.x * C + c) * 2 + 0] = a;
            partial[((int64_t)blockIdx.x * C + c) * 2 + 1] = b;
        }
        __syncthreads();
    }
}
void launch_stats_partial(int dtype, const void* x, int C, int64_t S, float* partial, hipStream_t s) {
    int nb = stats_blocks(S);
    UNET_DISPATCH(dtype, (k_stats_partial<T, 0><<<nb, 256, 0, s>>>((const T*)x, nullptr, C, S, stats_vpb(S), pow2_ge(C), nullptr, 0, partial)));
}
__device__ __forceinline__ void unpack8(uint4 v, float* f) {
    f[0] = __uint_as_float(v.x << 16); f[1] = __uint_as_float(v.x & 0xffff0000u);
    f[2] = __uint_as_float(v.y << 16); f[3] = __uint_as_float(v.y & 0xffff0000u);
    f[4] = __uint_as_float(v.z << 16); f[5] = __uint_as_float(v.z & 0xffff0000u);
    f[6] = __uint_as_float(v.w << 16); f[7] = __uint_as_float(v.w & 0xffff0000u);
}
__global__ void __launch_bounds__(256) k_norm_bwd_stats8(const uint4* __restrict__ u8, const uint4* __restrict__ g8, int C, int64_t S,
                                                         int64_t VPB, const float* __restrict__ stat, int act, float* __restrict__ partial) {
    __shared__ float red[256][17];
    const int G8 = C / 8, NV = 256 / G8, grp = threadIdx.x % G8, lane = threadIdx.x / G8, c0 = grp * 8;
    const int64_t v0 = (int64_t)blockIdx.x * VPB, v1 = v0 + VPB < S ? v0 + VPB : S;
    float mean[8], rstd[8], sc[8], sh[8], s1[8], s2[8];
#pragma unroll
    for (int e = 0; e < 8; ++e) {
        mean[e] = stat[c0 + e]; rstd[e] = stat[C + c0 + e]; sc[e] = stat[2 * C + c0 + e]; sh[e] = stat[3 * C + c0 + e];
        s1[e] = 0.f; s2[e] = 0.f;
    }
    for (int64_t v = v0 + lane; v < v1; v += 2 * NV) {
        const bool two = v + NV < v1;
        const uint4 ru0 = u8[v * G8 + grp], rg0 = g8[v * G8 + grp];
        uint4 ru1 = ru0, rg1 = make_uint4(0u, 0u, 0u, 0u);
        if (two) { ru1 = u8[(v + NV) * G8 + grp]; rg1 = g8[(v + NV) * G8 + grp]; }
        float uf[8], gf[8];
        unpack8(ru0, uf);
        unpack8(rg0, gf);
#pragma unroll
        for (int e = 0; e < 8; ++e) {
            float dv = gf[e] * act_d(fmaf(uf[e], sc[e], sh[e]), act);
            s1[e] += dv; s2[e] = fmaf(dv, (uf[e] - mean[e]) * rstd[e], s2[e]);
        }
        if (two) {
            unpack8(ru1, uf);
            unpack8(rg1, gf);
#pragma unroll
            for (int e = 0; e < 8; ++e) {
                float dv = gf[e] * act_d(fmaf(uf[e], sc[e], sh[e]), act);
                s1[e] += dv; s2[e] = fmaf(dv, (uf[e] - mean[e]) * rstd[e], s2[e]);
            }
        }
    }
    const int ln = threadIdx.x & 63, wv = threadIdx.x >> 6;
    if (G8 <= 32) {
#pragma unroll
        for (int e = 0; e < 8; ++e) {
            float a = s1[e], b = s2[e];
            for (int m = G8; m < 64; m <<= 1) { a += __shfl_xor(a, m); b += __shfl_xor(b, m); }
            s1[e] = a; s2[e] = b;
        }
        if (ln < G8) {
#pragma unroll
            for (int e = 0; e < 8; ++e) { red[wv * G8 + ln][e] = s1[e]; red[wv * G8 + ln][8 + e] = s2[e]; }
        }
        __syncthreads();
        if (threadIdx.x < G8 * 8) {
            const int gg = threadIdx.x / 8, e = threadIdx.x % 8;
            float a = 0.f, b = 0.f;
#pragma unroll
            for (int w = 0; w < 4; ++w) { a += red[w * G8 + gg][e]; b += red[w * G8 + gg][8 + e]; }
// ... 819 lines not shown
        if (!(q >= 1e-6f && q <= 1.0f - 1e-6f)) g = 0.f;
        float dl = q * (g - dot) + w_ce * (q - (c == tt ? 1.f : 0.f)) / n;
        if (k && c == 0) d0 = dl;
        else dlogits[(int64_t)(k ? c + k - 1 : c) * S + v] = dl;
    }
    if (k) {
        float m0 = -INFINITY;
        for (int c = 0; c < k; ++c) m0 = fmaxf(m0, logits[(int64_t)c * S + v]);
        float s0 = 0.f;
        for (int c = 0; c < k; ++c) s0 += __expf(logits[(int64_t)c * S + v] - m0);
        for (int c = 0; c < k; ++c) dlogits[(int64_t)c * S + v] = d0 * __expf(logits[(int64_t)c * S + v] - m0) / s0;
    }
}
template <int OCMAX>
__global__ void __launch_bounds__(256) k_loss_grad_v4(const float* __restrict__ logits, const int64_t* __restrict__ target, int C, int64_t S,
                                                      const float* __restrict__ level_out, float weight, int cost_mask,
                                                      float* __restrict__ dlogits) {
    const int oc = C;
    const int64_t q4 = (int64_t)blockIdx.x * 256 + threadIdx.x;
    if (q4 >= (S >> 2)) return;
    const float w_ce = (!(cost_mask & 7) || (cost_mask & 1)) ? weight : 0.f;
    const float w_dice = (cost_mask & 2) ? weight : 0.f, w_mse = (cost_mask & 4) ? weight : 0.f;
    const float n = level_out[3];
    const float dden = (float)(oc - 1 > 1 ? oc - 1 : 1), eps = 1e-5f;
    float dice_hit[OCMAX], dice_miss[OCMAX];
#pragma unroll
    for (int c = 0; c < OCMAX; ++c) {
        dice_hit[c] = dice_miss[c] = 0.f;
        if (c >= 1 && c < oc) {
            const float den = level_out[4 + oc + c] + eps, in2 = 2.f * level_out[4 + c] + eps;
            dice_hit[c] = w_dice * (-(2.f * 1.f * den - in2) / (den * den)) / dden;
            dice_miss[c] = w_dice * (-(2.f * 0.f * den - in2) / (den * den)) / dden;
        }
    }
    const longlong2 t01 = ((const longlong2*)target)[2 * q4], t23 = ((const longlong2*)target)[2 * q4 + 1];
    const int64_t tv[4] = {t01.x, t01.y, t23.x, t23.y};
    float4 pl[OCMAX];
#pragma unroll
    for (int c = 0; c < OCMAX; ++c)
        pl[c] = c < oc ? ((const float4*)(logits + (int64_t)c * S))[q4] : make_float4(-INFINITY, -INFINITY, -INFINITY, -INFINITY);
    float out[OCMAX][4];
#pragma unroll
    for (int j = 0; j < 4; ++j) {
        const int64_t t = tv[j];
        const bool valid = t < C;
        const int tt = (int)t;
        float lg[OCMAX], mx = -INFINITY;
#pragma unroll
        for (int c = 0; c < OCMAX; ++c) { lg[c] = j == 0 ? pl[c].x : j == 1 ? pl[c].y : j == 2 ? pl[c].z : pl[c].w; mx = fmaxf(mx, lg[c]); }
        float sum = 0.f;
#pragma unroll
        for (int c = 0; c < OCMAX; ++c) { lg[c] = c < oc ? __expf(lg[c] - mx) : 0.f; sum += lg[c]; }
        const float inv = 1.f / sum;
        float g[OCMAX], dot = 0.f;
#pragma unroll
        for (int c = 0; c < OCMAX; ++c) {
            g[c] = 0.f;
            if (c < oc) {
                const float q = lg[c] * inv, p = clamp_p(q);
                float gg = 0.f;
                gg += w_mse * (2.f * p - (c == tt ? 2.f : 0.f)) / n;
                if (c >= 1) gg += c == tt ? dice_hit[c] : dice_miss[c];
                if (!(q >= 1e-6f && q <= 1.0f - 1e-6f)) gg = 0.f;
                dot = fmaf(gg, q, dot);
                g[c] = gg; lg[c] = q;
            }
        }
#pragma unroll
        for (int c = 0; c < OCMAX; ++c)
            out[c][j] = (c < oc && valid) ? lg[c] * (g[c] - dot) + w_ce * (lg[c] - (c == tt ? 1.f : 0.f)) / n : 0.f;
    }
#pragma unroll
    for (int c = 0; c < OCMAX; ++c)
        if (c < oc) ((float4*)(dlogits + (int64_t)c * S))[q4] = make_float4(out[c][0], out[c][1], out[c][2], out[c][3]);
}
void launch_loss_grad(const float* logits, const int64_t* target, int C, int64_t S, int collapse, const float* level_out, float weight,
                      int cost_mask, float* dlogits, hipStream_t s) {
    if (loss_v4_ok(logits, target, dlogits, C, S, collapse)) {
        k_loss_grad_v4<8><<<cdiv64(S >> 2, 256), 256, 0, s>>>(logits, target, C, S, level_out, weight, cost_mask, dlogits);
        return;
    }
    k_loss_grad<<<cdiv64(S, 256), 256, 0, s>>>(logits, target, C, S, collapse, level_out, weight, cost_mask, dlogits);
}

struct SumBufs { const float* in[UNET_SUM_MAX_BUFFERS]; int n; };
__global__ void __launch_bounds__(256) k_sum_buffers(SumBufs b, float* __restrict__ out, int64_t count, int zero_inputs) {
    for (int64_t i0 = ((int64_t)blockIdx.x * 256 + threadIdx.x) * 4; i0 < count; i0 += (int64_t)gridDim.x * 1024) {
        if (i0 + 3 < count) {
            float4 acc = *(const float4*)(b.in[0] + i0);
            for (int k = 1; k < b.n; ++k) {
                const float4 v = *(const float4*)(b.in[k] + i0);
                acc.x += v.x; acc.y += v.y; acc.z += v.z; acc.w += v.w;
            }
            *(float4*)(out + i0) = acc;
            if (zero_inputs)
                for (int k = 0; k < b.n; ++k)
                    if (b.in[k] != out) *(float4*)(const_cast<float*>(b.in[k]) + i0) = make_float4(0.f, 0.f, 0.f, 0.f);
        } else {
            for (int j = 0; j < 4 && i0 + j < count; ++j) {
                float acc = b.in[0][i0 + j];
                for (int k = 1; k < b.n; ++k) acc += b.in[k][i0 + j];
                out[i0 + j] = acc;
                if (zero_inputs)
                    for (int k = 0; k < b.n; ++k)
                        if (b.in[k] != out) const_cast<float*>(b.in[k])[i0 + j] = 0.f;
            }
        }
    }
}
void launch_sum_buffers(const float* const* bufs, int n, float* out, int64_t count, int zero_inputs, hipStream_t s) {
    SumBufs b;
    b.n = n;
    for (int k = 0; k < UNET_SUM_MAX_BUFFERS; ++k) b.in[k] = k < n ? bufs[k] : nullptr;
    int64_t nb = (count + 1023) / 1024;
    if (nb > 4096) nb = 4096;
    k_sum_buffers<<<(unsigned)nb, 256, 0, s>>>(b, out, count, zero_inputs);
}

__global__ void __launch_bounds__(256) k_sumsq_partial(const float* __restrict__ g, int64_t n, float scale, float* __restrict__ partial) {
    __shared__ double red[256];
    double acc = 0.0;
    for (int64_t i0 = ((int64_t)blockIdx.x * 256 + threadIdx.x) * 4; i0 < n; i0 += (int64_t)gridDim.x * 1024) {
        float r = 0.f;
        if (i0 + 3 < n) {
            const float4 v = *(const float4*)(g + i0);
            const float a0 = v.x * scale, a1 = v.y * scale, a2 = v.z * scale, a3 = v.w * scale;
            r = fmaf(a0, a0, fmaf(a1, a1, fmaf(a2, a2, a3 * a3)));
        } else {
            for (int j = 0; j < 4; ++j)
                if (i0 + j < n) { float x = g[i0 + j] * scale; r = fmaf(x, x, r); }
        }
        acc += (double)r;
    }
    red[threadIdx.x] = acc;
    __syncthreads();
    for (int o = 128; o > 0; o >>= 1) {
        if ((int)threadIdx.x < o) red[threadIdx.x] += red[threadIdx.x + o];
        __syncthreads();
    }
    if (threadIdx.x == 0) partial[blockIdx.x] = (float)red[0];
}
void launch_sumsq_partial(const float* g, int64_t n, float scale, float* partial, int nblk, hipStream_t s) {
    k_sumsq_partial<<<nblk, 256, 0, s>>>(g, n, scale, partial);
}

constexpr int SGD_MAXSEG = 1024;
__global__ void __launch_bounds__(256) k_sgd(float* __restrict__ p, float* __restrict__ g, float* __restrict__ m, int64_t n,
                                             const SgdSeg* __restrict__ segs, int nseg, const float* __restrict__ partial, int nblk,
                                             float lr, float momentum, int nesterov, float wdecay, float clip_norm, float grad_scale, float* norm_out) {
    __shared__ double red[256];
    __shared__ float s_coef;
    __shared__ int64_t s_off[SGD_MAXSEG];
    __shared__ float s_wd[SGD_MAXSEG];
    double part = 0.0;
    for (int b = threadIdx.x; b < nblk; b += 256) part += partial[b];
    red[threadIdx.x] = part;
    const int ns = nseg < SGD_MAXSEG ? nseg : SGD_MAXSEG;
    for (int k = threadIdx.x; k < ns; k += 256) { s_off[k] = segs[k].offset; s_wd[k] = segs[k].wd; }
    __syncthreads();
    for (int o = 128; o > 0; o >>= 1) {
        if ((int)threadIdx.x < o) red[threadIdx.x] += red[threadIdx.x + o];
        __syncthreads();
    }
    if (threadIdx.x == 0) {
        float norm = (float)sqrt(red[0]);
        float coef = clip_norm / (norm + 1e-6f);
        s_coef = coef > 1.f ? 1.f : coef;
        if (blockIdx.x == 0 && norm_out) *norm_out = norm;
    }
    __syncthreads();
    const float coef = s_coef * grad_scale;
    auto seg_of = [&](int64_t i) {
        int lo = 0, hi = nseg - 1;
        while (lo < hi) {
            int mid = (lo + hi + 1) >> 1;
            int64_t off = mid < SGD_MAXSEG ? s_off[mid] : segs[mid].offset;
            if (off <= i) lo = mid; else hi = mid - 1;
        }
        return lo;
    };
    auto wd_of = [&](int sg) { return (sg < SGD_MAXSEG ? s_wd[sg] : segs[sg].wd) * wdecay; };
    auto upd = [&](float& pv, float& gv, float& mv, float wd) {
        float d = fmaf(wd, pv, gv * coef);
        float b = fmaf(momentum, mv, d);
        mv = b;
        pv = pv - lr * (nesterov ? fmaf(momentum, b, d) : b);
        gv = 0.f;
    };
    const int64_t n4 = n >> 2;
    for (int64_t q = (int64_t)blockIdx.x * 256 + threadIdx.x; q < n4; q += (int64_t)gridDim.x * 256) {
        const int64_t i = q * 4;
        const int sg = seg_of(i);
        const int64_t next = sg + 1 < nseg ? (sg + 1 < SGD_MAXSEG ? s_off[sg + 1] : segs[sg + 1].offset) : n;
        float4 pv = *(float4*)(p + i), gv = *(float4*)(g + i), mv = *(float4*)(m + i);
        float w0 = wd_of(sg), w1 = w0, w2 = w0, w3 = w0;
        if (next < i + 4) { w1 = wd_of(seg_of(i + 1)); w2 = wd_of(seg_of(i + 2)); w3 = wd_of(seg_of(i + 3)); }
        upd(pv.x, gv.x, mv.x, w0); upd(pv.y, gv.y, mv.y, w1); upd(pv.z, gv.z, mv.z, w2); upd(pv.w, gv.w, mv.w, w3);
        *(float4*)(p + i) = pv; *(float4*)(m + i) = mv; *(float4*)(g + i) = gv;
    }
    if (blockIdx.x == 0 && threadIdx.x < (n & 3)) {
        const int64_t i = (n4 << 2) + threadIdx.x;
        float pv = p[i], gv = g[i], mv = m[i];
        upd(pv, gv, mv, wd_of(seg_of(i)));
        p[i] = pv; m[i] = mv; g[i] = gv;
    }
}
void launch_sgd(float* p, float* g, float* m, int64_t n, const SgdSeg* segs, int nseg, const float* partial, int nblk, float lr,
                float momentum, int nesterov, float wdecay, float clip_norm, float grad_scale, float* norm_out, hipStream_t s) {
    int64_t nb = (n / 4 + 255) / 256;
    if (nb < 1) nb = 1;
    if (nb > 2048) nb = 2048;
    k_sgd<<<(unsigned)nb, 256, 0, s>>>(p, g, m, n, segs, nseg, partial, nblk, lr, momentum, nesterov, wdecay, clip_norm, grad_scale, norm_out);
}

}
```

unet-studio_amd/csrc/kernels_mfma_conv.hip:

```cpp
#include <type_traits>
#include <cstdlib>
#include "mfma_util.h"

namespace unet {

enum PackMode {
    PK_CONV_FWD = 0,
    PK_CONV_DGRAD = 1,
    PK_CONVT_DGRAD = 2,
    PK_CONVT_FWD = 3,
    PK_CONV_S2_DGRAD = 4
};
constexpr int PACK_LDS_ELEMS = 16 * (32 * 27 + 1);
template <int CK, int T, int MODE>
__device__ __forceinline__ void pack_unit_t(const float* __restrict__ w, __bf16* __restrict__ out, int unit, int Co, int A, int B, __bf16* lds) {
    constexpr int KSTEPS = CK == 32 ? T : (T + 1) / 2;
    const int NTT = Co / 16;
    const int q = unit / NTT, nt = unit % NTT, o0 = nt * 16;
    constexpr int RS = CK * T + 1;
    constexpr int n = 16 * CK * T, U = 8;
    for (int e0 = threadIdx.x; e0 < n; e0 += 256 * U) {
        float v[U];
        int dst[U];
#pragma unroll
        for (int u = 0; u < U; ++u) {
            const int e = e0 + u * 256;
            int r = 0, c = 0, t = 0;
            int64_t src = -1;
            if (e < n) {
                if constexpr (MODE == PK_CONV_FWD || MODE == PK_CONVT_DGRAD) {
                    const int Ax = MODE == PK_CONV_FWD ? A : B;
                    r = e / (CK * T); const int rem = e % (CK * T); c = rem / T; t = rem % T;
                    src = ((int64_t)(o0 + r) * Ax + q * CK) * T + rem;
                } else if constexpr (MODE == PK_CONV_DGRAD) {
                    c = e / (16 * 27); const int rem = e % (16 * 27); r = rem / 27; t = 26 - rem % 27;
                    src = ((int64_t)(q * CK + c) * A + o0) * 27 + rem;
                } else if constexpr (MODE == PK_CONVT_FWD) {
                    const int t8 = o0 / B, co0 = o0 % B;
                    c = e / 16; r = e % 16; t = 0;
                    src = ((int64_t)(q * CK + c) * B + co0 + r) * 8 + t8;
                } else {
                    const int pp = o0 / A, ci0 = o0 % A;
                    c = e / (16 * 8); const int rem = e % (16 * 8); r = rem / 8; t = rem % 8;
                    const int pk[3] = {(pp >> 2) & 1, (pp >> 1) & 1, pp & 1}, kk[3] = {(t >> 2) & 1, (t >> 1) & 1, t & 1};
                    int ft[3];
                    bool ok = true;
#pragma unroll
                    for (int d = 0; d < 3; ++d) {
                        if (pk[d] == 0) { ok = ok && kk[d] == 0; ft[d] = 1; }
                        else ft[d] = kk[d] == 0 ? 2 : 0;
                    }
                    if (ok) src = ((int64_t)(q * CK + c) * A + ci0 + r) * 27 + (ft[0] * 9 + ft[1] * 3 + ft[2]);
                }
            }
            dst[u] = e < n ? r * RS + c * T + t : -1;
            v[u] = src >= 0 ? w[src] : 0.f;
        }
#pragma unroll
        for (int u = 0; u < U; ++u)
            if (dst[u] >= 0) lds[dst[u]] = (__bf16)v[u];
    }
    __syncthreads();
    for (int f = threadIdx.x; f < KSTEPS * 64; f += 256) {
        const int ks = f >> 6, lane = f & 63, row = lane & 15;
        int tap, c0;
        if (CK == 32) { tap = ks; c0 = 8 * (lane >> 4); }
        else { tap = 2 * ks + (lane >> 5); c0 = 8 * ((lane >> 4) & 1); }
        bf16x8 o;
#pragma unroll
        for (int e = 0; e < 8; ++e) o[e] = tap < T ? lds[row * RS + (c0 + e) * T + tap] : (__bf16)0.f;
        *(bf16x8*)(out + ((((int64_t)q * KSTEPS + ks) * NTT + nt) * 64 + lane) * 8) = o;
    }
}
__device__ __forceinline__ void pack_unit(const float* __restrict__ w, __bf16* __restrict__ out, int unit, int Ci, int Co, int CK, int T,
                                          int mode, int A, int B, __bf16* lds) {
    switch (mode) {
        case PK_CONV_FWD:
            if (CK == 32) pack_unit_t<32, 27, PK_CONV_FWD>(w, out, unit, Co, A, B, lds); else pack_unit_t<16, 27, PK_CONV_FWD>(w, out, unit, Co, A, B, lds);
            break;
        case PK_CONV_DGRAD:
            if (CK == 32) pack_unit_t<32, 27, PK_CONV_DGRAD>(w, out, unit, Co, A, B, lds); else pack_unit_t<16, 27, PK_CONV_DGRAD>(w, out, unit, Co, A, B, lds);
            break;
        case PK_CONVT_DGRAD:
            if (CK == 32) pack_unit_t<32, 8, PK_CONVT_DGRAD>(w, out, unit, Co, A, B, lds); else pack_unit_t<16, 8, PK_CONVT_DGRAD>(w, out, unit, Co, A, B, lds);
            break;
        case PK_CONVT_FWD: pack_unit_t<32, 1, PK_CONVT_FWD>(w, out, unit, Co, A, B, lds); break;
        default: pack_unit_t<32, 8, PK_CONV_S2_DGRAD>(w, out, unit, Co, A, B, lds); break;
    }
}
__global__ void __launch_bounds__(256) k_mfma_pack(const float* __restrict__ w, __bf16* __restrict__ out, int Ci, int Co, int CK, int T,
                                                   int mode, int A, int B) {
    __shared__ __bf16 lds[PACK_LDS_ELEMS];
    pack_unit(w, out, blockIdx.x, Ci, Co, CK, T, mode, A, B, lds);
}
__global__ void __launch_bounds__(256) k_mfma_pack_batched(const float* __restrict__ params_base, char* __restrict__ ws,
                                                           const PackJob* __restrict__ jobs, int njobs, int64_t blk_base, int64_t nunits,
                                                           int* __restrict__ zero, int nzero) {
    __shared__ __bf16 lds[PACK_LDS_ELEMS];
    if (zero && blockIdx.x == 0)
        for (int i = threadIdx.x; i < nzero; i += 256) zero[i] = 0;
    for (int64_t u = blockIdx.x; u < nunits; u += gridDim.x) {
        const int64_t blk = blk_base + u;
        int lo = 0, hi = njobs - 1;
        while (lo < hi) {
            int mid = (lo + hi + 1) >> 1;
            if (jobs[mid].blk0 <= blk) lo = mid; else hi = mid - 1;
        }
        const PackJob jb = jobs[lo];
        pack_unit(params_base + jb.src_off, (__bf16*)(ws + jb.dst_off), (int)(blk - jb.blk0), jb.Ci, jb.Co, jb.CK, jb.T,
                  jb.mode, jb.A, jb.B, lds);
        __syncthreads();
    }
}
void launch_mfma_pack_batched(const float* params_base, void* ws, const PackJob* jobs_dev, int njobs, int64_t nblocks, hipStream_t s,
                              int64_t blk_base, int max_grid, int* zero, int nzero) {
    if (njobs <= 0 || nblocks <= 0) return;
    const int64_t grid = (max_grid > 0 && nblocks > max_grid) ? max_grid : nblocks;
    k_mfma_pack_batched<<<(unsigned)grid, 256, 0, s>>>(params_base, (char*)ws, jobs_dev, njobs, blk_base, nblocks, zero, nzero);
}

static inline int pick_ck(int Ci, bool allow32) { return (allow32 && Ci % 32 == 0) ? 32 : 16; }
static size_t pack_bytes(int Ci, int Co, int CK, int T) {
    int KSTEPS = CK == 32 ? T : (T + 1) / 2;
    return (size_t)(Ci / CK) * KSTEPS * (Co / 16) * 64 * 16;
}
static PackJob make_job(int Ci, int Co, int CK, int T, int mode, int A, int B) {
    PackJob j;
    j.src_off = 0; j.dst_off = 0; j.blk0 = 0;
    j.Ci = Ci; j.Co = Co; j.CK = CK; j.T = T; j.mode = mode; j.A = A; j.B = B; j.pad = 0;
    j.total = (int64_t)(Ci / CK) * (Co / 16);
    return j;
}
static void run_pack(const float* w, void* out, int Ci, int Co, int CK, int T, int mode, int A, int B, hipStream_t s) {
    k_mfma_pack<<<(unsigned)((Ci / CK) * (Co / 16)), 256, 0, s>>>(w, (__bf16*)out, Ci, Co, CK, T, mode, A, B);
}

template <int S, int KD, int PAD, int BZ, int BY, int BX, int CK, int NT, bool SC, int NW, bool ONE>
__global__ void __launch_bounds__(NW * 64, (NW == 8 && NT == 1) ? 4 : 2) k_mfma_conv_p(MfmaConvArgs a) {
    constexpr int NTHR = NW * 64;
    constexpr int HZ = (BZ - 1) * S + KD, HY = (BY - 1) * S + KD, HX = (BX - 1) * S + KD, NVOX = HZ * HY * HX;
    constexpr int G = CK / 8;
    constexpr bool SWZ = CK == 32 && S == 1 && KD == 3;
    constexpr int VS = SWZ ? 64 : (CK == 32 ? 96 : 32);
    constexpr int HXP = SWZ ? (HX + 3) / 4 * 4 : HX;
    constexpr int TXM = BX < 16 ? BX : 16;
    constexpr int TYM = 16 / TXM;
    constexpr int MT = BZ * BY * BX / 16, MTW = MT / NW;
    constexpr int T = KD * KD * KD;
    constexpr int KSTEPS = CK == 32 ? T : (T + 1) / 2;
    constexpr int UNITS = NVOX * G, ITERS = (UNITS + NTHR - 1) / NTHR;
    constexpr int NKX = SWZ ? 3 : 1;
    constexpr bool WLDS = KSTEPS * NT <= 32;
    constexpr int TILE_B = HZ * HY * HXP * VS;
    constexpr int WPIECES = KSTEPS * NT * 64, WITERS = WLDS ? (WPIECES + NTHR - 1) / NTHR : 1;
    static_assert(MT % NW == 0 && MTW >= 1, "tile must give every wave at least one m-tile");
    extern __shared__ __attribute__((aligned(16))) char smem[];

    const ConvGeom& g = a.g;
    const int tid = threadIdx.x, wave = tid >> 6, lane = tid & 63, j = lane & 15, gq = lane >> 4;
    const int nblk = a.tiles_x * a.tiles_y * a.tiles_z;
    const int nt0 = blockIdx.y * NT, NTT = g.Cout / 16;
    const int C0 = a.src[0].C;
    const int lg = tid % G;
    const int nchunk = ONE ? 1 : g.Cin / CK;
    const bf16x8* wp = (const bf16x8*)a.w;
// ... 1116 lines not shown
```

unet-studio_amd/csrc/unet_host.cpp:

```cpp
#include "../../include/unet.hpp"
#include "../../include/unet_hip.h"

#include <c10/hip/HIPStream.h>
#include <hip/hip_runtime_api.h>

#include <functional>
#include <sstream>
#include <thread>

namespace {

void check(int rc) { if (rc) throw std::runtime_error(unet_last_error()); }

void* stream_of(const torch::Device& d) {
    return d.is_cuda() ? (void*)c10::hip::getCurrentHIPStream(d.index()).stream() : nullptr;
}

struct Holder : torch::nn::Module {};

}

struct UNet3dImpl::WorkspacePool {
    struct Entry { torch::Tensor buf; hipEvent_t ev = nullptr; };
    static constexpr size_t MAX_IDLE = 4;
    std::mutex m;
    std::map<unet_plan*, std::vector<Entry>> idle;
    ~WorkspacePool() { clear(); }
    void clear() {
        std::scoped_lock<std::mutex> lock(m);
        for (auto& kv : idle)
            for (auto& e : kv.second)
                if (e.ev) (void)hipEventDestroy(e.ev);
        idle.clear();
    }
    size_t count() {
        std::scoped_lock<std::mutex> lock(m);
        size_t n = 0;
        for (auto& kv : idle) n += kv.second.size();
        return n;
    }
};

UNet3dImpl::UNet3dImpl(int32_t in_count_, int32_t out_count_, std::string architecture_)
    : in_count(in_count_), out_count(out_count_), architecture(architecture_)
{
    fov_strategy = "align_top";
    preproc = "";
    postproc = "softmax+create_mask+argmax";
    unet_plan* probe = nullptr;
    check(unet_plan_create(architecture_.c_str(), in_count_, out_count_, 1024, 1024, 1024, engine_dtype, 0, UNET_IMPL_AUTO, &probe));
    int n = 0;
    unet_plan_param_count(probe, &n);
    std::vector<std::vector<int64_t>> shapes(n);
    std::vector<std::string> names(n);
    std::vector<int64_t> fan(n);
    std::vector<int> isnw(n);
    int64_t total = 0;
    for (int i = 0; i < n; ++i) {
        int64_t d[5]; int nd = 0; char nm[128];
        check(unet_plan_param_shape(probe, i, d, &nd));
        check(unet_plan_param_name(probe, i, nm, sizeof(nm)));
        check(unet_plan_param_fan_in(probe, i, &fan[i], &isnw[i]));
        shapes[i].assign(d, d + nd);
        names[i] = nm;
        int64_t e = 1;
        for (auto v : shapes[i]) e *= v;
        total += e;
    }
    flat_params = torch::zeros({total});
    flat_grads = torch::zeros({total});
    int64_t off = 0;
    std::map<std::string, std::shared_ptr<Holder>> tops, subs;
    for (int i = 0; i < n; ++i) {
        int64_t e = 1;
        for (auto v : shapes[i]) e *= v;
        auto view = torch::from_blob(flat_params.data_ptr<float>() + off, shapes[i], torch::TensorOptions().dtype(torch::kFloat32));
        if (fan[i] > 0) view.uniform_(-1.0 / std::sqrt((double)fan[i]), 1.0 / std::sqrt((double)fan[i]));
        else view.fill_(isnw[i] ? 1.0f : 0.0f);
        off += e;
        size_t p1 = names[i].find('.'), p2 = names[i].rfind('.');
        std::string top = names[i].substr(0, p1), mid = names[i].substr(p1 + 1, p2 - p1 - 1), leaf = names[i].substr(p2 + 1);
        if (!tops.count(top)) tops[top] = register_module(top, std::make_shared<Holder>());
        std::string key = top + "." + mid;
        if (!subs.count(key)) subs[key] = tops[top]->register_module(mid, std::make_shared<Holder>());
        params_.push_back(subs[key]->register_parameter(leaf, view, true));
    }
    int nb = 0;
    unet_plan_buffer_count(probe, &nb);
    for (int i = 0; i < nb; ++i) {
        int64_t ne = 0;
        unet_plan_buffer_shape(probe, i, &ne);
        buffers_.push_back(register_buffer("bnorm" + std::to_string(i / 2) + (i % 2 ? "_running_var" : "_running_mean"),
                                           i % 2 ? torch::ones({ne}) : torch::zeros({ne})));
    }
    unet_plan_destroy(probe);
    trigger_ = torch::zeros({1}, torch::requires_grad(true));
    bind_views();
}

UNet3dImpl::~UNet3dImpl(void)
{
    for (auto& kv : plans_) unet_plan_destroy(kv.second);
}

void UNet3dImpl::bind_views(void)
{
    int64_t off = 0;
    auto opts = torch::TensorOptions().dtype(torch::kFloat32).device(flat_params.device());
    for (auto& p : params_) {
        int64_t e = p.numel();
        torch::NoGradGuard ng;
        p.set_data(torch::from_blob(flat_params.data_ptr<float>() + off, p.sizes(), opts));
        p.mutable_grad() = torch::from_blob(flat_grads.data_ptr<float>() + off, p.sizes(), opts);
        off += e;
    }
}

void UNet3dImpl::to_device(const torch::Device& device)
{
    if (flat_params.defined() && flat_params.device() != device) {
        flat_params = flat_params.to(device);
        flat_grads = flat_grads.to(device);
        for (auto& b : buffers_) b.set_data(b.to(device));
        bind_views();
    }
    ensure_flat();
}

void UNet3dImpl::ensure_flat(void)
{
    if (params_.empty()) return;
    auto dev = params_[0].device();
    bool ok = flat_params.defined() && flat_params.device() == dev && params_[0].data_ptr() == flat_params.data_ptr();
    if (!ok) {
        torch::NoGradGuard ng;
        std::vector<torch::Tensor> ps, gs;
        for (auto& p : params_) {
            ps.push_back(p.detach().to(dev).reshape({-1}).to(torch::kFloat32));
            gs.push_back(p.grad().defined() ? p.grad().detach().to(dev).reshape({-1}).to(torch::kFloat32) : torch::zeros({p.numel()}, ps.back().options()));
        }
        flat_params = torch::cat(ps).contiguous();
        flat_grads = torch::cat(gs).contiguous();
        bind_views();
    }
    if (!trigger_.defined() || trigger_.device() != dev) {
        trigger_ = torch::zeros({1}, torch::TensorOptions().device(dev).requires_grad(true));
        if (momentum_.defined()) {
            if (optimizer) {
                const char* lo = (const char*)momentum_.data_ptr();
                const char* hi = lo + momentum_.numel() * sizeof(float);
                for (auto& kv : optimizer->state()) {
                    auto& ps = static_cast<torch::optim::SGDParamState&>(*kv.second);
                    const char* q = ps.momentum_buffer().defined() ? (const char*)ps.momentum_buffer().data_ptr() : nullptr;
                    if (q && q >= lo && q < hi) ps.momentum_buffer(torch::Tensor());
                }
            }
            momentum_ = momentum_.to(dev);
        }
        scratch_ = torch::Tensor();
        std::scoped_lock<std::mutex> lock(plans_mutex_);
        for (auto& kv : plans_) unet_plan_destroy(kv.second);
        plans_.clear();
        if (ws_pool_) ws_pool_->clear();
    }
    for (auto& b : buffers_)
        if (b.device() != dev) b.set_data(b.to(dev));
}

void UNet3dImpl::rebind_grads(void)
{
    torch::NoGradGuard ng;
    int64_t off = 0;
    auto opts = torch::TensorOptions().dtype(torch::kFloat32).device(flat_grads.device());
    for (auto& p : params_) {
        int64_t e = p.numel();
        float* slot = flat_grads.data_ptr<float>() + off;
        if (!p.grad().defined() || p.grad().data_ptr() != (void*)slot) {
            auto alias = torch::from_blob(slot, p.sizes(), opts);
            if (p.grad().defined()) alias.copy_(p.grad()); else alias.zero_();
            p.mutable_grad() = alias;
        }
        off += e;
    }
}

int UNet3dImpl::create_layer(torch::nn::Sequential&, const std::string& def, int)
{
    throw std::runtime_error("create_layer(" + def + "): layers are lowered into the HIP plan by unet_plan_create");
}

unet_plan* UNet3dImpl::plan_for(int64_t d, int64_t h, int64_t w)
{
    std::scoped_lock<std::mutex> lock(plans_mutex_);
    std::array<int64_t, 3> key = {d, h, w};
    auto it = plans_.find(key);
    if (it != plans_.end()) return it->second;
    unet_plan* p = nullptr;
    auto dev = device();
    check(unet_plan_create(architecture.c_str(), in_count, out_count, (int)d, (int)h, (int)w, engine_dtype,
                           dev.is_cuda() ? dev.index() : 0, UNET_IMPL_AUTO, &p));
    plans_[key] = p;
    return p;
}

size_t UNet3dImpl::pooled_workspaces(void) const { return ws_pool_ ? ws_pool_->count() : 0; }

torch::Tensor UNet3dImpl::workspace_for(unet_plan* plan)
{
    auto dev = device();
    std::shared_ptr<WorkspacePool> pool;
    {
        std::scoped_lock<std::mutex> lock(plans_mutex_);
        if (!ws_pool_) ws_pool_ = std::make_shared<WorkspacePool>();
        pool = ws_pool_;
    }
    WorkspacePool::Entry e;
    {
        std::scoped_lock<std::mutex> lock(pool->m);
        auto& v = pool->idle[plan];
        if (!v.empty()) { e = v.back(); v.pop_back(); }
    }
    c10::DeviceGuard guard(dev);
    void* const lease_stream = stream_of(dev);
    if (e.buf.defined()) {
        if (e.ev) (void)hipStreamWaitEvent((hipStream_t)lease_stream, e.ev, 0);
    } else {
        size_t bytes = 0;
        unet_plan_workspace_bytes(plan, &bytes);
        e.buf = torch::empty({(int64_t)bytes}, torch::TensorOptions().dtype(torch::kUInt8).device(dev));
        if (dev.is_cuda() && hipEventCreateWithFlags(&e.ev, hipEventDisableTiming) != hipSuccess) e.ev = nullptr;
    }
    std::weak_ptr<WorkspacePool> wp = pool;
    auto back = [wp, e, plan, dev, lease_stream](void*) mutable {
        auto p = wp.lock();
        if (e.ev && dev.is_cuda()) {
            c10::DeviceGuard g(dev);
            (void)hipEventRecord(e.ev, (hipStream_t)lease_stream);
        }
        if (p) {
            std::scoped_lock<std::mutex> lock(p->m);
            auto& v = p->idle[plan];
            if (v.size() < WorkspacePool::MAX_IDLE) { v.push_back(e); return; }
        }
        if (e.ev) (void)hipEventDestroy(e.ev);
    };
    return torch::from_blob(e.buf.data_ptr(), e.buf.sizes(), back, e.buf.options());
}

std::vector<torch::Tensor> UNet3dImpl::run_forward(unet_plan* plan, torch::Tensor ws, torch::Tensor x, int mode)
{
    std::vector<const float*> pp;
    for (auto& p : params_) pp.push_back(p.data_ptr<float>());
    std::vector<float*> bp;
    for (auto& b : buffers_) bp.push_back(b.data_ptr<float>());
    int nl = 0;
    unet_plan_output_count(plan, &nl);
    std::vector<torch::Tensor> outs(nl);
    std::vector<float*> op(nl, nullptr);
    for (int l = 0; l < nl; ++l) {
        int64_t d[5];
        unet_plan_output_shape(plan, l, d);
        if (d[1]) {
            outs[l] = torch::empty({d[0], d[1], d[2], d[3], d[4]}, torch::TensorOptions().dtype(torch::kFloat32).device(x.device()));
            op[l] = outs[l].data_ptr<float>();
        }
    }
    check(unet_forward(plan, pp.data(), bp.empty() ? nullptr : bp.data(), x.data_ptr<float>(), op.data(), ws.data_ptr(), mode,
                       stream_of(x.device())));
    return outs;
}

void UNet3dImpl::run_backward(unet_plan* plan, torch::Tensor ws, const std::vector<torch::Tensor>& grad_outs)
{
    rebind_grads();
    std::vector<const float*> pp, go;
    std::vector<float*> gp;
    std::vector<torch::Tensor> keep;
    int64_t off = 0;
    for (auto& p : params_) {
        pp.push_back(p.data_ptr<float>());
        gp.push_back(flat_grads.data_ptr<float>() + off);
        off += p.numel();
    }
    for (auto& t : grad_outs) {
        if (t.defined()) { keep.push_back(t.contiguous()); go.push_back(keep.back().data_ptr<float>()); }
        else go.push_back(nullptr);
    }
    check(unet_backward(plan, pp.data(), go.data(), gp.data(), nullptr, ws.data_ptr(), stream_of(flat_params.device())));
}

struct UNetForwardFn : torch::autograd::Function<UNetForwardFn> {
    static torch::autograd::variable_list forward(torch::autograd::AutogradContext* ctx, torch::Tensor x, torch::Tensor trigger,
                                                  int64_t self, int64_t plan, torch::Tensor ws) {
        (void)trigger;
        auto* m = reinterpret_cast<UNet3dImpl*>(self);
        auto outs = m->run_forward(reinterpret_cast<unet_plan*>(plan), ws, x, 1);
        ctx->saved_data["self"] = self;
        ctx->saved_data["plan"] = plan;
        ctx->saved_data["ws"] = ws;
        return outs;
    }
    static torch::autograd::variable_list backward(torch::autograd::AutogradContext* ctx, torch::autograd::variable_list grads) {
        auto* m = reinterpret_cast<UNet3dImpl*>(ctx->saved_data["self"].toInt());
        m->run_backward(reinterpret_cast<unet_plan*>(ctx->saved_data["plan"].toInt()), ctx->saved_data["ws"].toTensor(), grads);
        return {torch::Tensor(), torch::Tensor(), torch::Tensor(), torch::Tensor(), torch::Tensor()};
    }
};

std::vector<torch::Tensor> UNet3dImpl::forward(torch::Tensor inputTensor)
{
    if (inputTensor.dim() != 5 || inputTensor.size(0) != 1 || inputTensor.size(1) != in_count)
        throw std::runtime_error("UNet3d::forward expects a {1,in_count,D,H,W} tensor");
    ensure_flat();
    if (inputTensor.device() != device())
        throw std::runtime_error("UNet3d::forward: input and model are on different devices");
    auto x = inputTensor.to(torch::kFloat32).contiguous();
    unet_plan* plan = plan_for(x.size(2), x.size(3), x.size(4));
    auto ws = workspace_for(plan);
    if (is_training() && torch::GradMode::is_enabled())
        return UNetForwardFn::apply(x, trigger_, reinterpret_cast<int64_t>(this), reinterpret_cast<int64_t>(plan), ws);
    return run_forward(plan, ws, x, is_training() ? 1 : 0);
}

void UNet3dImpl::prepare_for_inference(const torch::Device& device)
{
    to_device(device);
    eval();
    for (size_t i = 0; i + 1 < buffers_.size(); i += 2) {
        buffers_[i].zero_();
        buffers_[i + 1].fill_(1.0f);
    }
}

void UNet3dImpl::copy_from(const UNet3dImpl& r)
{
    torch::NoGradGuard no_grad;
    ensure_flat();
    const_cast<UNet3dImpl&>(r).ensure_flat();
    if (flat_params.sizes() == r.flat_params.sizes())
        flat_params.copy_(r.flat_params);
    else {
        auto rhs = r.parameters(), lhs = parameters();
        for (size_t i = 0; i < rhs.size() && i < lhs.size(); ++i)
            if (lhs[i].sizes() == rhs[i].sizes()) lhs[i].copy_(rhs[i]);
    }
    for (size_t i = 0; i < r.buffers_.size() && i < buffers_.size(); ++i)
        if (buffers_[i].sizes() == r.buffers_[i].sizes()) buffers_[i].copy_(r.buffers_[i]);
    voxel_size = r.voxel_size;
    dim = r.dim;
    fov_strategy = r.fov_strategy;
    postproc = r.postproc;
    preproc = r.preproc;
}

void UNet3dImpl::add_gradient_from(const UNet3dImpl& r)
{
    torch::NoGradGuard no_grad;
    ensure_flat();
    rebind_grads();
    const_cast<UNet3dImpl&>(r).ensure_flat();
    const_cast<UNet3dImpl&>(r).rebind_grads();
    flat_grads.add_(r.flat_grads.to(flat_grads.device()).to(torch::kFloat32));
}

void UNet3dImpl::create_optimizer(float learning_rate)
{
    std::vector<torch::Tensor> decay_params, no_decay_params;
    for (auto& p : named_parameters()) {
        auto v = p.value();
        const auto& name = p.key();
        bool no_decay = name.find("bias") != std::string::npos || v.dim() <= 1;
        (no_decay ? no_decay_params : decay_params).push_back(v);
    }
    std::vector<torch::optim::OptimizerParamGroup> groups;
    auto opt_d = std::make_unique<torch::optim::SGDOptions>(learning_rate);
    opt_d->momentum(0.99); opt_d->nesterov(true); opt_d->weight_decay(3e-5);
    auto opt_nd = std::make_unique<torch::optim::SGDOptions>(learning_rate);
    opt_nd->momentum(0.99); opt_nd->nesterov(true); opt_nd->weight_decay(0.0);
    groups.push_back(torch::optim::OptimizerParamGroup(decay_params, std::move(opt_d)));
    groups.push_back(torch::optim::OptimizerParamGroup(no_decay_params, std::move(opt_nd)));
    optimizer = std::make_shared<torch::optim::SGD>(groups, torch::optim::SGDOptions(learning_rate));
}

std::string UNet3dImpl::get_info(void) const
{
    std::ostringstream out;
    out << "in: " << in_count << " out: " << out_count << std::endl;
    out << "dim: " << dim << " reso: " << voxel_size << std::endl;
    out << "structure: " << architecture << std::endl;
    if (!preproc.empty()) out << "preproc: " << preproc << std::endl;
    if (!postproc.empty()) out << "postproc: " << postproc << std::endl;
    return out.str();
}

void UNet3dImpl::print_layers(void)
{
    for (auto& p : named_parameters()) std::cout << p.key() << " " << p.value().sizes() << std::endl;
}

torch::Tensor UNet3dImpl::loss_and_backward(torch::Tensor input, torch::Tensor target, bool ce, bool dice, bool mse, int collapse_before)
{
    ensure_flat();
    auto x = input.to(torch::kFloat32).contiguous();
    unet_plan* plan = plan_for(x.size(2), x.size(3), x.size(4));
    auto ws = workspace_for(plan);
    auto outs = run_forward(plan, ws, x, 1);
    size_t sb = 0;
    unet_loss_scratch_bytes(plan, &sb);
    auto sc = torch::empty({(int64_t)sb}, torch::TensorOptions().dtype(torch::kUInt8).device(x.device()));
    auto losses = torch::empty({4}, torch::TensorOptions().dtype(torch::kFloat32).device(x.device()));
    std::vector<torch::Tensor> gouts;
    std::vector<const float*> op;
    std::vector<float*> gp;
    for (auto& o : outs) {
        gouts.push_back(o.defined() ? torch::empty_like(o) : torch::Tensor());
        op.push_back(o.defined() ? o.data_ptr<float>() : nullptr);
        gp.push_back(o.defined() ? gouts.back().data_ptr<float>() : nullptr);
    }
    auto t = target.to(torch::kLong).contiguous();
    int mask = (ce ? 1 : 0) | (dice ? 2 : 0) | (mse ? 4 : 0);
    check(unet_loss(plan, op.data(), t.data_ptr<int64_t>(), mask, collapse_before, gp.data(), losses.data_ptr<float>(), sc.data_ptr(),
                    stream_of(x.device())));
    run_backward(plan, ws, gouts);
    return losses;
}

void UNet3dImpl::broadcast_parameters(int root)
{
    if (!comm_) throw std::runtime_error("broadcast_parameters: no communicator attached");
    ensure_flat();
    void* st = stream_of(flat_params.device());
    check(unet_comm_broadcast(comm_, flat_params.data_ptr<float>(), flat_params.numel(), root, st));
    for (auto& b : buffers_) check(unet_comm_broadcast(comm_, b.data_ptr<float>(), b.numel(), root, st));
    check(unet_comm_join(comm_, st));
}

void UNet3dImpl::broadcast_buffers(int root)
{
    if (!comm_) throw std::runtime_error("broadcast_buffers: no communicator attached");
    if (buffers_.empty()) return;
    ensure_flat();
    void* st = stream_of(flat_params.device());
    for (auto& b : buffers_) check(unet_comm_broadcast(comm_, b.data_ptr<float>(), b.numel(), root, st));
    check(unet_comm_join(comm_, st));
}

void UNet3dImpl::allreduce_gradients(void)
{
    if (!comm_) throw std::runtime_error("allreduce_gradients: no communicator attached");
    ensure_flat();
    rebind_grads();
    void* st = stream_of(flat_grads.device());
    const int64_t hi = reduced_from_ >= 0 ? reduced_from_ : flat_grads.numel();
    check(unet_allreduce_grads(comm_, flat_grads.data_ptr<float>(), 0, hi, st));
    for (auto& b : buffers_) check(unet_comm_broadcast(comm_, b.data_ptr<float>(), b.numel(), 0, st));
    check(unet_comm_join(comm_, st));
    reduced_from_ = -1;
}

torch::Tensor UNet3dImpl::loss_and_backward_overlapped(torch::Tensor input, torch::Tensor target, bool ce, bool dice, bool mse, int collapse_before)
{
    if (!comm_) return loss_and_backward(input, target, ce, dice, mse, collapse_before);
    ensure_flat();
    rebind_grads();
    auto x = input.to(torch::kFloat32).contiguous();
    unet_plan* plan = plan_for(x.size(2), x.size(3), x.size(4));
    auto ws = workspace_for(plan);
    auto outs = run_forward(plan, ws, x, 1);
    size_t sb = 0;
    unet_loss_scratch_bytes(plan, &sb);
    auto sc = torch::empty({(int64_t)sb}, torch::TensorOptions().dtype(torch::kUInt8).device(x.device()));
    auto losses = torch::empty({4}, torch::TensorOptions().dtype(torch::kFloat32).device(x.device()));
    std::vector<torch::Tensor> gouts;
    std::vector<const float*> op, go;
    std::vector<float*> gp;
    for (auto& o : outs) {
        gouts.push_back(o.defined() ? torch::empty_like(o) : torch::Tensor());
        op.push_back(o.defined() ? o.data_ptr<float>() : nullptr);
        gp.push_back(o.defined() ? gouts.back().data_ptr<float>() : nullptr);
        go.push_back(gp.back());
    }
    auto t = target.to(torch::kLong).contiguous();
    int mask = (ce ? 1 : 0) | (dice ? 2 : 0) | (mse ? 4 : 0);
    void* st = stream_of(x.device());
    check(unet_loss(plan, op.data(), t.data_ptr<int64_t>(), mask, collapse_before, gp.data(), losses.data_ptr<float>(), sc.data_ptr(), st));
    std::vector<const float*> pp;
    std::vector<float*> gw;
    int64_t off = 0;
    for (auto& p : params_) { pp.push_back(p.data_ptr<float>()); gw.push_back(flat_grads.data_ptr<float>() + off); off += p.numel(); }
    int nb = 0, op_lo[8];
    int64_t elem_lo[8];
    check(unet_plan_backward_buckets(plan, 3, &nb, op_lo, elem_lo));
    int op_hi = 1 << 30;
    int64_t elem_hi = flat_grads.numel();
    for (int k = 0; k < nb; ++k) {
        check(unet_backward_part(plan, pp.data(), go.data(), gw.data(), nullptr, ws.data_ptr(), op_hi, op_lo[k], st));
        if (k + 1 < nb) {
            check(unet_allreduce_grads(comm_, flat_grads.data_ptr<float>(), elem_lo[k], elem_hi, st));
            reduced_from_ = elem_lo[k];
        }
        op_hi = op_lo[k]; elem_hi = elem_lo[k];
    }
    return losses;
}

void UNet3dImpl::bind_optimizer_state(void)
{
    ensure_flat();
    if (!momentum_.defined() || momentum_.device() != flat_params.device() || momentum_.numel() != flat_params.numel())
        momentum_ = momentum_.defined() && momentum_.numel() == flat_params.numel() ? momentum_.to(flat_params.device()) : torch::zeros_like(flat_params);
    if (!optimizer) return;
    torch::NoGradGuard ng;
    auto& st = optimizer->state();
    auto opts = torch::TensorOptions().dtype(torch::kFloat32).device(momentum_.device());
    int64_t off = 0;
    for (auto& p : params_) {
        float* slot = momentum_.data_ptr<float>() + off;
        off += p.numel();
        void* key = p.unsafeGetTensorImpl();
        auto it = st.find(key);
        if (it == st.end()) {
            auto ps = std::make_unique<torch::optim::SGDParamState>();
            ps->momentum_buffer(torch::from_blob(slot, p.sizes(), opts));
            st[key] = std::move(ps);
            continue;
        }
        auto& ps = static_cast<torch::optim::SGDParamState&>(*it->second);
        if (ps.momentum_buffer().defined() && ps.momentum_buffer().data_ptr() == (void*)slot) continue;
        auto alias = torch::from_blob(slot, p.sizes(), opts);
        if (ps.momentum_buffer().defined()) alias.copy_(ps.momentum_buffer().reshape(p.sizes()));
        ps.momentum_buffer(alias);
    }
}

bool UNet3dImpl::save_optimizer(const std::string& file_name)
{
    try {
        if (!optimizer) throw std::runtime_error("save_optimizer: no optimizer (create_optimizer first)");
        bind_optimizer_state();
        torch::save(*optimizer, file_name);
        return true;
    } catch (const std::exception& e) { error_msg = std::string("cannot save optimizer: ") + e.what(); return false; }
}

bool UNet3dImpl::load_optimizer(const std::string& file_name)
{
    try {
        if (!optimizer) throw std::runtime_error("load_optimizer: no optimizer (create_optimizer first)");
        torch::load(*optimizer, file_name);
        bind_optimizer_state();
        return true;
    } catch (const std::exception& e) { error_msg = std::string("cannot load optimizer: ") + e.what(); return false; }
}

void UNet3dImpl::sgd_step(float lr, float grad_scale, float clip_norm)
{
    ensure_flat();
    rebind_grads();
    bind_optimizer_state();
    if (!scratch_.defined()) scratch_ = torch::empty({65536 + 16}, torch::TensorOptions().dtype(torch::kUInt8).device(flat_params.device()));
    if (plans_.empty()) throw std::runtime_error("sgd_step before any forward");
    check(unet_sgd_step(plans_.begin()->second, flat_params.data_ptr<float>(), flat_grads.data_ptr<float>(), momentum_.data_ptr<float>(), lr,
                        0.99f, 1, 3e-5f, clip_norm, grad_scale, (float*)((char*)scratch_.data_ptr() + 65536), scratch_.data_ptr(),
                        stream_of(flat_params.device())));
}
```

unet-studio_amd/engine.py:

```python
import ctypes as C
import os

_HERE = os.path.dirname(os.path.abspath(__file__))
LIB_PATH = os.environ.get("UNET_HIP_LIBRARY") or os.path.join(_HERE, "libunet_hip.so")

DTYPE_F32, DTYPE_BF16 = 0, 1
IMPL_AUTO, IMPL_DIRECT = 0, 1

if not os.path.exists(LIB_PATH):
    raise ImportError(
        "libunet_hip.so not found at %s: build it first (python -c 'import __graft_entry__ as g; g.build()' "
        "or unet-studio_amd/csrc/build.sh); there is no CPU fallback" % LIB_PATH)

import torch

lib = C.CDLL(LIB_PATH)

_vp, _i, _sz, _f = C.c_void_p, C.c_int, C.c_size_t, C.c_float
_pp = C.POINTER(C.c_void_p)


def _sig(name, res, *args):
    fn = getattr(lib, name)
    fn.restype = res
    fn.argtypes = list(args)
    return fn


_sig("unet_last_error", C.c_char_p)
_sig("unet_init", _i, C.POINTER(_i))
_sig("unet_device_info", _i, _i, C.c_char_p, _sz, C.POINTER(_sz), C.POINTER(_i), C.POINTER(_i))
_sig("unet_plan_create", _i, C.c_char_p, _i, _i, _i, _i, _i, _i, _i, _i, C.POINTER(_vp))
_sig("unet_plan_destroy", None, _vp)
_sig("unet_plan_param_count", _i, _vp, C.POINTER(_i))
_sig("unet_plan_param_shape", _i, _vp, _i, C.POINTER(C.c_int64), C.POINTER(_i))
_sig("unet_plan_param_name", _i, _vp, _i, C.c_char_p, _sz)
_sig("unet_plan_param_decay", _i, _vp, _i, C.POINTER(_i))
_sig("unet_plan_param_fan_in", _i, _vp, _i, C.POINTER(C.c_int64), C.POINTER(_i))
_sig("unet_plan_buffer_count", _i, _vp, C.POINTER(_i))
_sig("unet_plan_buffer_shape", _i, _vp, _i, C.POINTER(C.c_int64))
_sig("unet_plan_output_count", _i, _vp, C.POINTER(_i))
_sig("unet_plan_output_shape", _i, _vp, _i, C.POINTER(C.c_int64))
_sig("unet_plan_workspace_bytes", _i, _vp, C.POINTER(_sz))
_sig("unet_plan_flops", _i, _vp, C.POINTER(C.c_double), C.POINTER(C.c_double))
_sig("unet_plan_describe", _sz, _vp, C.c_char_p, _sz)
_sig("unet_plan_op_count", _i, _vp, C.POINTER(_i))
_sig("unet_plan_op_info", _i, _vp, _i, C.POINTER(_i), C.POINTER(_i), C.POINTER(_i), C.POINTER(_i), C.POINTER(_i), C.POINTER(C.c_int64),
     C.POINTER(C.c_int64), C.c_char_p, _sz)
_sig("unet_profile_begin", _i)
_sig("unet_profile_end", _i, _i, C.POINTER(_i), C.POINTER(_i), C.POINTER(_f), C.POINTER(_i))
_sig("unet_forward", _i, _vp, _pp, _pp, _vp, _pp, _vp, _i, _vp)
_sig("unet_backward", _i, _vp, _pp, _pp, _pp, _vp, _vp, _vp)
_sig("unet_backward_part", _i, _vp, _pp, _pp, _pp, _vp, _vp, _i, _i, _vp)
_sig("unet_plan_backward_buckets", _i, _vp, _i, C.POINTER(_i), C.POINTER(_i), C.POINTER(C.c_int64))
_sig("unet_loss_scratch_bytes", _i, _vp, C.POINTER(_sz))
_sig("unet_loss", _i, _vp, _pp, _vp, _i, _i, _pp, _vp, _vp, _vp)
_sig("unet_forward_loss", _i, _vp, _pp, _pp, _vp, _pp, _vp, _i, _i, _pp, _vp, _vp, _vp, _vp)
_sig("unet_forward_loss_mode", _i, _vp, _pp, _pp, _vp, _pp, _vp, _i, _i, _pp, _vp, _vp, _vp, _i, _vp)
_sig("unet_sum_buffers", _i, _pp, _i, _vp, C.c_int64, _i, _vp)
_sig("unet_stream_create_cu_range", _i, _i, _i, _i, _vp)
_sig("unet_stream_destroy", _i, _vp)
_sig("unet_plan_side_cu_range", _i, _vp, _i, _i)
_sig("unet_pack_filters", _i, _vp, _vp, _vp, _i, _vp, _vp)
_sig("unet_sgd_step", _i, _vp, _vp, _vp, _vp, _f, _f, _i, _f, _f, _f, _vp, _vp, _vp)
_sig("unet_set_error", None, C.c_char_p)
_sig("unet_comm_unique_id", _i, _vp)
_sig("unet_comm_create", _i, _i, _i, _vp, _i, C.POINTER(_vp))
_sig("unet_comm_create_all", _i, _i, C.POINTER(_i), C.POINTER(_vp))
_sig("unet_comm_destroy", _i, _vp)
_sig("unet_comm_rank", _i, _vp, C.POINTER(_i), C.POINTER(_i))
_sig("unet_allreduce_grads", _i, _vp, _vp, C.c_int64, C.c_int64, _vp)
_sig("unet_allreduce_grads_all", _i, _pp, _i, _pp, C.c_int64, C.c_int64, _pp)
_sig("unet_comm_broadcast", _i, _vp, _vp, C.c_int64, _i, _vp)
_sig("unet_comm_join", _i, _vp, _vp)
_sig("unet_op_scratch_bytes", _i, _i, _i, _i, _i, _i, C.POINTER(_sz))
_sig("unet_op_conv3d_fwd", _i, _i, _i, _vp, _vp, _vp, _vp, _i, _i, _i, _i, _i, _i, _i, _vp, _vp)
_sig("unet_op_conv3d_pack", _i, _i, _vp, _vp, _i, _i, _i, _i, _i, _i, _i, _vp)
_sig("unet_op_conv3d_fwd_packed", _i, _i, _vp, _vp, _vp, _vp, _vp, _i, _i, _i, _i, _i, _i, _i, _vp)
_sig("unet_op_conv3d_fwd_fused", _i, _i, _i, _vp, _vp, _vp, _i, _vp, _vp, _vp, _vp, _i, _i, _i, _i, _i, _i, _i, _vp, _vp)
_sig("unet_op_conv3d_bwd_data", _i, _i, _i, _vp, _vp, _vp, _i, _i, _i, _i, _i, _i, _i, _vp, _vp)
_sig("unet_op_conv3d_fwd_norm", _i, _vp, _vp, _i, _i, _vp, _vp, _vp, _vp, C.c_double, _vp, _vp, C.c_double, _i, _i, _vp, _vp, _vp,
     _i, _i, _i, _i, _i, _vp, _vp)
_sig("unet_op_conv3d_bwd_data_norm", _i, _i, _vp, _vp, _vp, _i, _vp, _vp, _vp, _i, _vp, _vp, _vp, _i, _i, _i, _i, _i, _vp, _vp)
_sig("unet_op_conv3d_bwd_weight", _i, _i, _i, _vp, _vp, _vp, _vp, _i, _i, _i, _i, _i, _i, _i, _vp, _vp)
_sig("unet_op_convt_fwd", _i, _i, _i, _vp, _vp, _vp, _vp, _i, _i, _i, _i, _i, _vp, _vp)
_sig("unet_op_convt_bwd_data", _i, _i, _i, _vp, _vp, _vp, _i, _i, _i, _i, _i, _vp, _vp)
_sig("unet_op_convt_bwd_weight", _i, _i, _i, _vp, _vp, _vp, _vp, _i, _i, _i, _i, _i, _vp, _vp)
_sig("unet_op_pack_ndhwc", _i, _i, _vp, _vp, _i, C.c_int64, _vp)
_sig("unet_op_unpack_ncdhw", _i, _i, _vp, _vp, _i, C.c_int64, _vp)

EXPORTS = [
    "unet_last_error", "unet_init", "unet_device_info", "unet_plan_create", "unet_plan_destroy", "unet_plan_param_count",
    "unet_plan_param_shape", "unet_plan_param_name", "unet_plan_param_decay", "unet_plan_param_fan_in", "unet_plan_buffer_count",
    "unet_plan_buffer_shape", "unet_plan_output_count", "unet_plan_output_shape", "unet_plan_workspace_bytes",
    "unet_plan_flops", "unet_plan_describe", "unet_plan_op_count", "unet_plan_op_info", "unet_profile_begin", "unet_profile_end", "unet_forward", "unet_backward", "unet_backward_part", "unet_plan_backward_buckets", "unet_loss_scratch_bytes", "unet_loss", "unet_forward_loss", "unet_forward_loss_mode", "unet_sum_buffers",
    "unet_sgd_step", "unet_pack_filters", "unet_stream_create_cu_range", "unet_stream_destroy", "unet_plan_side_cu_range", "unet_set_error", "unet_comm_unique_id", "unet_comm_create", "unet_comm_create_all", "unet_comm_destroy", "unet_comm_rank",
    "unet_allreduce_grads", "unet_allreduce_grads_all", "unet_comm_broadcast", "unet_comm_join", "unet_op_scratch_bytes", "unet_op_conv3d_fwd", "unet_op_conv3d_fwd_fused", "unet_op_conv3d_pack", "unet_op_conv3d_fwd_packed", "unet_op_conv3d_bwd_data", "unet_op_conv3d_fwd_norm", "unet_op_conv3d_bwd_data_norm", "unet_op_conv3d_bwd_weight",
    "unet_op_convt_fwd", "unet_op_convt_bwd_data", "unet_op_convt_bwd_weight", "unet_op_pack_ndhwc", "unet_op_unpack_ncdhw",
]


MODE_PACKS_CURRENT = 2


class UNetError(RuntimeError):
    """What the C++ host rethrows as std::runtime_error (unet.cpp:53,66,88,117)."""


def check(rc):
    if rc != 0:
        raise UNetError(lib.unet_last_error().decode("utf-8", "replace"))


def ptr_array(ptrs):
    arr = (C.c_void_p * max(1, len(ptrs)))()
    for i, p in enumerate(ptrs):
        arr[i] = p
    return arr


class Plan:

    def __init__(self, arch, in_c, out_c, size, dtype=DTYPE_BF16, device=0, impl=IMPL_AUTO):
        self.handle = C.c_void_p()
        self._pid = os.getpid()
        D, H, W = size
        check(lib.unet_plan_create(arch.encode(), in_c, out_c, D, H, W, dtype, device, impl, C.byref(self.handle)))
        self.arch, self.in_c, self.out_c, self.size, self.dtype, self.device = arch, in_c, out_c, (D, H, W), dtype, device
        n = C.c_int()
        check(lib.unet_plan_param_count(self.handle, C.byref(n)))
        self.param_shapes, self.param_decay, self.param_fan_in, self.param_is_norm_weight, self.param_names = [], [], [], [], []
        dims, nd, dec, fan, isn = (C.c_int64 * 5)(), C.c_int(), C.c_int(), C.c_int64(), C.c_int()
        for i in range(n.value):
            check(lib.unet_plan_param_shape(self.handle, i, dims, C.byref(nd)))
            self.param_shapes.append(tuple(dims[k] for k in range(nd.value)))
            nm = C.create_string_buffer(128)
            check(lib.unet_plan_param_name(self.handle, i, nm, 128))
            self.param_names.append(nm.value.decode())
            check(lib.unet_plan_param_decay(self.handle, i, C.byref(dec)))
            self.param_decay.append(bool(dec.value))
            check(lib.unet_plan_param_fan_in(self.handle, i, C.byref(fan), C.byref(isn)))
            self.param_fan_in.append(fan.value)
            self.param_is_norm_weight.append(bool(isn.value))
        check(lib.unet_plan_buffer_count(self.handle, C.byref(n)))
        self.buffer_numel = []
        ne = C.c_int64()
        for i in range(n.value):
            check(lib.unet_plan_buffer_shape(self.handle, i, C.byref(ne)))
            self.buffer_numel.append(ne.value)
        check(lib.unet_plan_output_count(self.handle, C.byref(n)))
        self.output_shapes = []
        for l in range(n.value):
            check(lib.unet_plan_output_shape(self.handle, l, dims))
            self.output_shapes.append(tuple(dims[k] for k in range(5)))
        b = C.c_size_t()
        check(lib.unet_plan_workspace_bytes(self.handle, C.byref(b)))
        self.workspace_bytes = b.value
        check(lib.unet_loss_scratch_bytes(self.handle, C.byref(b)))
        self.loss_scratch_bytes = b.value
        f, g = C.c_double(), C.c_double()
        check(lib.unet_plan_flops(self.handle, C.byref(f), C.byref(g)))
        self.flops_fwd, self.flops_bwd = f.value, g.value

    def backward_buckets(self, max_buckets=3):
        n = C.c_int()
        ops, el = (C.c_int * max_buckets)(), (C.c_int64 * max_buckets)()
        check(lib.unet_plan_backward_buckets(self.handle, max_buckets, C.byref(n), ops, el))
        return [(ops[k], el[k]) for k in range(n.value)]

    def ops(self):
        n = C.c_int()
        check(lib.unet_plan_op_count(self.handle, C.byref(n)))
        out = []
        k, ci, co, ks, st = C.c_int(), C.c_int(), C.c_int(), C.c_int(), C.c_int()
        di, do = (C.c_int64 * 3)(), (C.c_int64 * 3)()
        for i in range(n.value):
            nm = C.create_string_buffer(128)
            check(lib.unet_plan_op_info(self.handle, i, C.byref(k), C.byref(ci), C.byref(co), C.byref(ks), C.byref(st), di, do, nm, 128))
            out.append({"kind": k.value, "cin": ci.value, "cout": co.value, "ks": ks.value, "stride": st.value,
                        "in_dims": tuple(di), "out_dims": tuple(do), "name": nm.value.decode()})
        return out

    def describe(self):
        n = lib.unet_plan_describe(self.handle, None, 0)
        buf = C.create_string_buffer(n)
        lib.unet_plan_describe(self.handle, buf, n)
        return buf.value.decode()

    def __del__(self):
        h = getattr(self, "handle", None)
        if h is not None and h.value and lib is not None and getattr(self, "_pid", None) == os.getpid():
            lib.unet_plan_destroy(h)
            self.handle = C.c_void_p()


PROF_CATEGORIES = ["conv_fwd", "dgrad", "wgrad", "norm_fwd", "norm_bwd", "other"]


class profile:

    def __init__(self, max_records=1 << 16):
        self.max_records, self.records = max_records, []

    def __enter__(self):
        check(lib.unet_profile_begin())
        return self

    def __exit__(self, *exc):
        n = C.c_int()
        op, cat, ms = (C.c_int * self.max_records)(), (C.c_int * self.max_records)(), (C.c_float * self.max_records)()
        rc = lib.unet_profile_end(self.max_records, op, cat, ms, C.byref(n))
        self.records = [(op[i], PROF_CATEGORIES[cat[i]], ms[i]) for i in range(n.value)]
        if exc[0] is None:
            check(rc)
        return False


COMM_ID_BYTES = 128


class Comm:

    def __init__(self, rank, world, id_bytes, device=0):
        self.handle = C.c_void_p()
        self._pid = os.getpid()
        buf = (C.c_char * COMM_ID_BYTES).from_buffer_copy(bytes(id_bytes))
        check(lib.unet_comm_create(rank, world, buf, device, C.byref(self.handle)))
        self.rank, self.world, self.device = rank, world, device

    @staticmethod
    def unique_id():
        buf = (C.c_char * COMM_ID_BYTES)()
        check(lib.unet_comm_unique_id(buf))
        return bytes(buf)

    @classmethod
    def single(cls, device=0):
        return cls(0, 1, cls.unique_id(), device)

    @classmethod
    def from_torch_distributed(cls, device, group=None):
        import torch.distributed as dist
        rank, world = dist.get_rank(group), dist.get_world_size(group)
        box = [cls.unique_id() if rank == 0 else None]
        dist.broadcast_object_list(box, src=0, group=group)
        return cls(rank, world, box[0], device)

    def allreduce(self, flat, lo, hi, stream):
        check(lib.unet_allreduce_grads(self.handle, flat.data_ptr(), int(lo), int(hi), stream))
# ... 13 lines not shown
```

unet-studio_amd/train.py:

```python
import math
import os

import torch
import torch.distributed as dist


class TrainingParam:

    def __init__(self, batch_size=32, epoch=10000, learning_rate=0.001, seed=0, cost_ce=True, cost_dice=True, cost_mse=True):
        self.batch_size, self.epoch, self.learning_rate, self.seed = batch_size, epoch, learning_rate, seed
        self.cost_ce, self.cost_dice, self.cost_mse = cost_ce, cost_dice, cost_mse


class SyntheticVolumes:

    def __init__(self, in_count, out_count, size, device, base_seed=0, cache=0):
        self.in_count, self.out_count, self.size, self.device, self.base_seed = in_count, out_count, tuple(size), device, base_seed
        self._cache, self._cache_n = {}, cache

    def __call__(self, index):
        if index in self._cache:
            return self._cache[index]
        g = torch.Generator(device=self.device)
        g.manual_seed(self.base_seed + index)
        x = torch.rand((1, self.in_count) + self.size, generator=g, device=self.device, dtype=torch.float32)
        t = torch.randint(0, self.out_count, (1,) + self.size, generator=g, device=self.device, dtype=torch.int64)
        if len(self._cache) < self._cache_n:
            self._cache[index] = (x, t)
        return x, t


class Trainer:

    def __init__(self, model, param, source, rank=0, world_size=1, group=None, comm=None):
        self.model, self.param, self.source = model, param, source
        self.rank, self.world_size, self.group, self.comm = rank, world_size, group, comm
        if comm is not None:
            self.rank, self.world_size = comm.rank, comm.world
        self.overlap = True
        self.packs_reuse = hasattr(model, "_run_forward_loss")
        self.in_flight = max(1, int(os.environ.get("UNET_MICRO_IN_FLIGHT", "1")))
        self.pack_after_update = False
        self._packed_size, self._packed_version = None, None
        self.stats_direct = hasattr(model, "_run_forward_loss")
        self._lanes, self._gbufs, self._gptrs = None, [], []
        self.cur_epoch = 0
        model.train()
        if model.optimizer is None:
            model.create_optimizer(param.learning_rate)
        self._stats = torch.zeros(4, dtype=torch.float32, device=model.device())
        self._acc = None

    def lr_at(self, epoch):
        return self.param.learning_rate * math.pow(1.0 - float(epoch) / self.param.epoch, 0.9)

    def step(self):
        p, m = self.param, self.model
        cur_data_index = self.cur_epoch * p.batch_size
        for g in m.optimizer.param_groups:
            g["lr"] = self.lr_at(self.cur_epoch)
        count = 0
        mine = list(range(self.rank, p.batch_size, self.world_size))
        works = []
        info = getattr(self.source, "sample_info", None)
        if info is not None:
            if self._acc is None:
                self._acc = torch.zeros(5, dtype=torch.float32, device=m.device())
                self._stats = self._acc[:4]
            collapse, counted = {}, {}
            for b in mine:
                is_template, is_shifted = info(cur_data_index + b)
                collapse[b] = self.source.max_template_label + 1 if is_shifted else 0
                counted[b] = not self.source.has_subject_data or not is_template
            kc = {b: {"collapse_before": collapse[b]} if collapse[b] else {} for b in mine}
        else:
            kc, counted = {b: {} for b in mine}, None
        multi = self.world_size > 1 or self.comm is not None
        overlap = (multi and self.overlap and hasattr(m, "forward_backward_bucketed") and p.batch_size >= self.world_size)
        stream = torch.cuda.current_stream(m.device()).cuda_stream if self.comm is not None else None

        def reduce_bucket(lo, hi):
            if hi > lo and self.comm is not None:
                self.comm.allreduce(m.flat_grads, lo, hi, stream)
            elif hi > lo:
                works.append(dist.all_reduce(m.flat_grads[lo:hi], op=dist.ReduceOp.SUM, group=self.group, async_op=True))

        lanes_on = (self.in_flight > 1 and len(mine) > 1 and hasattr(m, "make_lane") and not m.buffers())
        if lanes_on or not mine or not self.stats_direct or counted is not None:
            (self._acc if counted is not None else self._stats).zero_()
        if lanes_on:
            losses_all = self._step_in_lanes(mine, cur_data_index, kc)
            for b, l in zip(mine, losses_all):
                if counted is None or counted[b]:
                    self._stats += l
            count = len(mine)
            mine = []
            overlap = False
        packed_sizes = set()
        if self._packed_size is not None and self._packed_version == getattr(m, "_params_version", None):
            packed_sizes.add(self._packed_size)
        for k, b in enumerate(mine):
            x, t = self.source(cur_data_index + b)
            last_size = tuple(x.shape[2:])
            kw = {"packs_current": True} if (self.packs_reuse and last_size in packed_sizes) else {}
            packed_sizes.add(last_size)
            first_direct = k == 0 and self.stats_direct and counted is None
            kw.update(kc[b])
            if first_direct:
                kw["losses_out"] = self._stats
            if overlap and k == len(mine) - 1:
                losses = m.forward_backward_bucketed(x, t, reduce_bucket, p.cost_ce, p.cost_dice, p.cost_mse, **kw)
            else:
                losses = m.forward_backward(x, t, p.cost_ce, p.cost_dice, p.cost_mse, **kw)
            if not first_direct and (counted is None or counted[b]):
                self._stats += losses
            count += 1
        if counted is not None:
            n_counted = sum(1 for b in counted if counted[b])
            if n_counted:
                self._acc[4:5].fill_(float(n_counted))
        stats = self._acc if counted is not None else self._stats
        if self.comm is not None:
            if not overlap:
                self.comm.allreduce(m.flat_grads, 0, m.flat_grads.numel(), stream)
            self.comm.allreduce(stats, 0, stats.numel(), stream)
            self.comm.join(stream)
        elif self.world_size > 1:
            if not overlap:
                dist.all_reduce(m.flat_grads, op=dist.ReduceOp.SUM, group=self.group)
            dist.all_reduce(stats, op=dist.ReduceOp.SUM, group=self.group)
            for w in works:
                w.wait()
        m.optimizer.step(grad_scale=1.0 / p.batch_size, clip_norm=12.0)
        self._packed_size = None
        if self.pack_after_update and mine and not lanes_on and m.pack_filters(last_size):
            self._packed_size, self._packed_version = last_size, m._params_version
        if self.comm is not None and self.world_size > 1:
            for b in m.buffers():
                self.comm.broadcast(b, 0, stream)
            self.comm.join(stream)
        elif self.world_size > 1:
            for b in (m.buffers() if hasattr(m, "buffers") else []):
                dist.broadcast(b, 0, group=self.group)
        self.cur_epoch += 1
        return self._stats

    def _step_in_lanes(self, mine, cur_data_index, kc=None):
        import torch.cuda as tc
        from . import engine as E
        p, m = self.param, self.model
        x0, _ = self.source(cur_data_index + mine[0])
        if self._lanes is None:
            n = int(os.environ.get("UNET_LANE_CUS", "0"))
            self._lanes = [m.make_lane(x0.shape[2:], cu_range=(i * n, n) if n > 0 else None) for i in range(self.in_flight)]
        while len(self._gbufs) < len(mine):
            buf = m.flat_grads if not self._gbufs else torch.zeros_like(m.flat_grads)
            self._gbufs.append(buf)
            self._gptrs.append(m.grad_pointers(buf))
        main = tc.current_stream(m.device())
        for lane in self._lanes:
            lane["stream"].wait_stream(main)
        losses = []
        for k, b in enumerate(mine):
            lane = self._lanes[k % self.in_flight]
            with tc.stream(lane["stream"]):
                x, t = self.source(cur_data_index + b)
                if tuple(x.shape[2:]) != tuple(x0.shape[2:]):
                    raise ValueError("micro-steps in flight need samples of one size (lane plans were made for %s, got %s)"
                                     % (tuple(x0.shape[2:]), tuple(x.shape[2:])))
                l = m.forward_backward_lane(lane, x, t, self._gptrs[k], p.cost_ce, p.cost_dice, p.cost_mse,
                                            packs_current=self.packs_reuse and k >= self.in_flight, **(kc[b] if kc else {}))
            l.record_stream(main)
            losses.append(l)
        for lane in self._lanes:
            main.wait_stream(lane["stream"])
        n = len(mine)
        E.check(E.lib.unet_sum_buffers(E.ptr_array([g.data_ptr() for g in self._gbufs[:n]]), n, m.flat_grads.data_ptr(),
                                       m.flat_grads.numel(), 1, main.cuda_stream))
        return losses

    def validate(self, test_in, test_out, output_model=None):
        m = output_model if output_model is not None else self.model
        was_training = m._training
        m.eval()
        acc = torch.zeros(3, dtype=torch.float64)
        with torch.no_grad():
            for x, t in zip(test_in, test_out):
                outs = m.forward(x)
                losses, _ = m.loss(outs, t, True, True, True, 0, want_grad=False)
                acc += losses[1:4].double().cpu()
        m.train(was_training)
        errors = (acc / max(1, len(test_in))).tolist() if len(test_in) else []
        with self.model.error_mutex:
            for mm in {id(self.model): self.model, id(m): m}.values():
                mm.testing_errors.extend(errors)
        return errors

    def record_errors(self):
        if getattr(self.source, "sample_info", None) is not None and self._acc is not None:
            acc = self._acc.cpu()
            if not float(acc[4]):
                return []
            e = (acc[1:4] / acc[4]).tolist()
        else:
            e = (self._stats[1:4] / float(self.param.batch_size)).tolist()
        with self.model.error_mutex:
            self.model.training_errors.extend(e)
        return e
```

unet-studio_amd/unet3d.py:

```python
import math
import threading

import torch

from . import engine as E

_DT = {"fp32": E.DTYPE_F32, "f32": E.DTYPE_F32, "float32": E.DTYPE_F32, "bf16": E.DTYPE_BF16, "bfloat16": E.DTYPE_BF16}


_NO_FUSED_LOSS = False


def _stream_ptr(device):
    return torch.cuda.current_stream(device).cuda_stream


class SGD:

    def __init__(self, model, lr):
        self.model = model
        self.param_groups = [{"lr": lr, "weight_decay": 3e-5}, {"lr": lr, "weight_decay": 0.0}]
        self.momentum, self.nesterov, self.weight_decay = 0.99, True, 3e-5
        self.momentum_buffer = torch.zeros_like(model.flat_params)
        self.last_grad_norm = torch.zeros(1, device=model.flat_params.device, dtype=torch.float32)
        self._scratch = torch.empty(65536, dtype=torch.uint8, device=model.flat_params.device)

    def step(self, grad_scale=1.0, clip_norm=12.0):
        m = self.model
        lr = self.param_groups[0]["lr"]
        plan = m._any_plan()
        E.check(E.lib.unet_sgd_step(plan.handle, m.flat_params.data_ptr(), m.flat_grads.data_ptr(),
                                    self.momentum_buffer.data_ptr(), lr, self.momentum, int(self.nesterov),
                                    self.weight_decay, clip_norm, grad_scale, self.last_grad_norm.data_ptr(),
                                    self._scratch.data_ptr(), _stream_ptr(m.device())))
        m._params_version += 1

    def zero_grad(self):
        self.model.flat_grads.zero_()

    def state_dict(self):
        return {"momentum_buffer": self.momentum_buffer.clone(), "lr": self.param_groups[0]["lr"]}

    def load_state_dict(self, sd):
        if sd["momentum_buffer"].numel() != self.momentum_buffer.numel():
            raise E.UNetError("optimizer state does not belong to this architecture: %d momentum elements, %d parameters"
                              % (sd["momentum_buffer"].numel(), self.momentum_buffer.numel()))
        self.momentum_buffer.copy_(sd["momentum_buffer"].to(self.momentum_buffer.device))
        for g in self.param_groups:
            g["lr"] = sd["lr"]


class _Forward(torch.autograd.Function):

    @staticmethod
    def forward(ctx, x, trigger, model, plan, ws):
        outs = model._run_forward(plan, ws, x, mode=1)
        ctx.model, ctx.plan, ctx.ws = model, plan, ws
        return tuple(outs)

    @staticmethod
    def backward(ctx, *gouts):
        gouts = [g.contiguous() if g is not None else None for g in gouts]
        ctx.model._run_backward(ctx.plan, ctx.ws, gouts)
        return None, None, None, None, None


class UNet3d:

    def __init__(self, in_count, out_count, architecture, device="cuda:0", dtype="bf16", impl=E.IMPL_AUTO, seed=None):
        self.in_count, self.out_count, self.architecture = int(in_count), int(out_count), architecture
        self.fov_strategy, self.preproc, self.postproc = "align_top", "", "softmax+create_mask+argmax"
        self.orientation, self.error_msg = "", ""
        self.voxel_size, self.dim = (1.0, 1.0, 1.0), (192, 224, 192)
        self.testing_errors, self.training_errors, self.single_component_label = [], [], []
        self.error_mutex = threading.Lock()
        self.optimizer = None
        self._device = torch.device(device)
        self._dtype, self._impl = _DT[dtype], impl
        self._training = True
        self._plans, self._workspaces = {}, {}
        self._params_version = 0
        probe = E.Plan(architecture, self.in_count, self.out_count, self._probe_size(architecture), self._dtype,
                       self._device.index or 0, impl)
        self._probe = probe
        self.param_shapes = probe.param_shapes
        sizes = [int(math.prod(s)) for s in self.param_shapes]
        self._offsets = [0]
        for n in sizes:
            self._offsets.append(self._offsets[-1] + n)
        self.flat_params = torch.zeros(self._offsets[-1], dtype=torch.float32, device=self._device)
        self.flat_grads = torch.zeros_like(self.flat_params)
        self._params = [self.flat_params[self._offsets[i]:self._offsets[i + 1]].view(self.param_shapes[i])
                        for i in range(len(sizes))]
        self._grads = [self.flat_grads[self._offsets[i]:self._offsets[i + 1]].view(self.param_shapes[i])
                       for i in range(len(sizes))]
        self._buffers = [torch.zeros(n, dtype=torch.float32, device=self._device) for n in probe.buffer_numel]
        for i in range(1, len(self._buffers), 2):
            self._buffers[i].fill_(1.0)
        self.num_batches_tracked = 0
        self._pp = E.ptr_array([p.data_ptr() for p in self._params])
        self._gp = E.ptr_array([g.data_ptr() for g in self._grads])
        self._bp = E.ptr_array([b.data_ptr() for b in self._buffers]) if self._buffers else None
        self._trigger = torch.zeros(1, device=self._device, requires_grad=True)
        self.reset_parameters(seed)

    @staticmethod
    def _probe_size(arch):
        n = sum(1 for l in arch.replace("\r", "").split("\n") if l.strip())
        s = 1 << max(n, 3)
        return (s, s, s)

    def parameters(self):
        return list(self._params)

    def grads(self):
        return list(self._grads)

    def buffers(self):
        return list(self._buffers)

    def device(self):
        return self._device

    def to(self, device):
        if torch.device(device) != self._device:
            raise E.UNetError("a UNet3d lives on the device it was constructed on: build one on %s and copy_from()" % device)
        return self

    def train(self, on=True):
        self._training = bool(on)
        return self

    def eval(self):
        return self.train(False)

    def set_requires_grad(self, req):
        self._training = self._training and bool(req)

    def reset_parameters(self, seed=None):
        g = torch.Generator(device="cpu")
        if seed is not None:
            g.manual_seed(seed)
        with torch.no_grad():
            for p, fan, isn in zip(self._params, self._probe.param_fan_in, self._probe.param_is_norm_weight):
                if fan > 0:
                    b = 1.0 / math.sqrt(fan)
                    p.copy_(((torch.rand(p.shape, generator=g) * 2 - 1) * b).to(self._device))
                else:
                    p.fill_(1.0 if isn else 0.0)
        self._params_version += 1

    def load_parameters(self, arrays, buffers=None):
        assert len(arrays) == len(self._params), "parameter count mismatch"
        with torch.no_grad():
            for p, a in zip(self._params, arrays):
                a = torch.as_tensor(a, dtype=torch.float32)
                if a.numel() != p.numel():
                    raise E.UNetError("tensor size mismatch")
                p.copy_(a.reshape(p.shape).to(self._device))
            if buffers is not None:
                for b, a in zip(self._buffers, buffers):
                    b.copy_(torch.as_tensor(a, dtype=torch.float32).reshape(b.shape).to(self._device))
        self._params_version += 1

    def copy_from(self, r):
        with torch.no_grad():
            for a, b in zip(self._params, r._params):
                if a.shape == b.shape:
                    a.copy_(b)
            for a, b in zip(self._buffers, r._buffers):
                if a.shape == b.shape:
                    a.copy_(b)
        self.voxel_size, self.dim = r.voxel_size, r.dim
        self.fov_strategy, self.postproc, self.preproc = r.fov_strategy, r.postproc, r.preproc
        self._params_version += 1

    def add_gradient_from(self, r):
        self.flat_grads.add_(r.flat_grads.to(self._device, torch.float32))

    def create_optimizer(self, learning_rate):
        self.optimizer = SGD(self, learning_rate)
        return self.optimizer

    def save_optimizer(self, file_name):
        try:
            if self.optimizer is None:
                raise E.UNetError("save_optimizer: no optimizer (create_optimizer first)")
            sd = self.optimizer.state_dict()
# ... 223 lines not shown
```

Measured before the change: 800.3 million.

## Fuse SGD update with bf16 MFMA filter packing into one tiled kernel

Adds a combined kernel that runs the SGD momentum update per weight tile through LDS and writes the bf16 packed forward and dgrad filter layouts directly into the training workspace. The next forward can then reuse these packs instead of running a separate pack pass. Per-parameter tile descriptors are built at plan creation and checked against the pack jobs, with a fallback to the plain SGD step when they do not match. The cost is extra bookkeeping of the last plan and workspace, plus a more complex kernel whose pack writes are scattered.

```diff
diff --git a/include/unet.hpp b/include/unet.hpp
--- a/include/unet.hpp
+++ b/include/unet.hpp
@@ -105,6 +105,7 @@
     void to_device(const torch::Device& device);
     torch::Tensor loss_and_backward(torch::Tensor input, torch::Tensor target_int64, bool ce, bool dice, bool mse, int collapse_before = 0);
     void sgd_step(float lr, float grad_scale, float clip_norm = 12.0f);
+    bool pack_in_update = true;
     void bind_optimizer_state(void);
     bool save_optimizer(const std::string& file_name);
     bool load_optimizer(const std::string& file_name);
@@ -121,6 +122,13 @@
     std::shared_ptr<WorkspacePool> ws_pool_;
     std::mutex plans_mutex_;
     torch::Tensor trigger_, momentum_, scratch_;
+    unet_plan* last_plan_ = nullptr;
+    unet_plan* packed_plan_ = nullptr;
+    torch::Tensor last_ws_, packed_ws_;
+    uint64_t packed_stamp_ = 0;
+    uint64_t params_stamp(void) const;
+    torch::Tensor training_workspace(unet_plan* plan, int* mode);
+    void drop_packs(void);
     struct unet_comm* comm_ = nullptr;
     int64_t reduced_from_ = -1;
     unet_plan* plan_for(int64_t d,int64_t h,int64_t w);
diff --git a/include/unet_hip.h b/include/unet_hip.h
--- a/include/unet_hip.h
+++ b/include/unet_hip.h
@@ -86,6 +86,10 @@
                   float momentum, int nesterov, float weight_decay, float clip_norm, float grad_scale, float* norm_out,
                   void* scratch, void* stream);
 
+int unet_sgd_step_packed(const unet_plan* plan, float* params_flat, float* grads_flat, float* momentum_flat, float lr,
+                         float momentum, int nesterov, float weight_decay, float clip_norm, float grad_scale, float* norm_out,
+                         void* workspace, int with_dgrad, int* made, void* scratch, void* stream);
+
 int unet_op_scratch_bytes(int cin, int cout, int D, int H, int W, size_t* bytes);
 int unet_op_conv3d_fwd(int dtype, int impl, const void* x, const float* w, const float* b, void* y, int cin, int cout, int D,
                        int H, int W, int ks, int stride, void* scratch, void* stream);
diff --git a/unet-studio_amd/csrc/engine.cpp b/unet-studio_amd/csrc/engine.cpp
--- a/unet-studio_amd/csrc/engine.cpp
+++ b/unet-studio_amd/csrc/engine.cpp
@@ -97,6 +97,8 @@
     std::vector<PackJob> pack_jobs;
     int64_t pack_blocks = 0;
     PackJob* jobs_dev = nullptr;
+    std::vector<SgdTile> sgd_tiles;
+    SgdTile* tiles_dev = nullptr;
     SgdSeg* segs_dev = nullptr;
     int nseg = 0;
     int64_t n_param_elems = 0;
@@ -114,6 +116,7 @@
         if (segs_dev) (void)hipFree(segs_dev);
         if (wz_jobs_dev) (void)hipFree(wz_jobs_dev);
         if (jobs_dev) (void)hipFree(jobs_dev);
+        if (tiles_dev) (void)hipFree(tiles_dev);
         if (ev_fork) (void)hipEventDestroy(ev_fork);
         if (ev_join) (void)hipEventDestroy(ev_join);
         if (ev_pack) (void)hipEventDestroy(ev_pack);
@@ -326,6 +329,60 @@
             }
             if (which == 0) pack_fwd_blocks = pack_blocks;
         }
+        build_sgd_tiles();
+    }
+
+    void build_sgd_tiles() {
+        sgd_tiles.clear();
+        if (pack_jobs.empty()) return;
+        const size_t np = g.params.size();
+        std::vector<int> jf(np, -1), jd(np, -1), d0(np, 0), d1(np, 0), taps(np, 0);
+        {
+            size_t j = 0;
+            for (int which = 0; which < 2; ++which)
+                for (size_t i = 0; i < g.ops.size(); ++i) {
+                    const Op& op = g.ops[i];
+                    if (!conv[i].mfma_fwd()) continue;
+                    const bool convt = op.kind != OP_CONV;
+                    if (which >= (convt ? 2 : (conv[i].dgrad == Dgrad::mfma ? 2 : 1))) continue;
+                    const ConvGeom cg = op_geom_of(op);
+                    int& slot = which == 0 ? jf[op.weight] : jd[op.weight];
+                    if (j >= pack_jobs.size() || pack_jobs[j].src_off != p_off[op.weight] || slot >= 0) return;
+                    slot = (int)j++;
+                    d0[op.weight] = convt ? cg.Cin : cg.Cout; d1[op.weight] = convt ? cg.Cout : cg.Cin; taps[op.weight] = convt ? 8 : 27;
+                }
+            if (j != pack_jobs.size()) return;
+        }
+        std::vector<int64_t> units(pack_jobs.size(), 0);
+        bool ok = true;
+        for (size_t i = 0; i < np && ok; ++i) {
+            SgdTile t{};
+            t.wd = g.params[i].decay ? 1.f : 0.f;
+            t.job_fwd = jf[i]; t.job_dgrad = jd[i];
+            const int64_t n = p_off[i + 1] - p_off[i];
+            if (jf[i] < 0) {
+                if (jd[i] >= 0) { ok = false; break; }
+                constexpr int64_t chunk = 8192;
+                for (int64_t o = 0; o < n; o += chunk) { t.off = p_off[i] + o; t.count = std::min(chunk, n - o); sgd_tiles.push_back(t); }
+                continue;
+            }
+            if ((int64_t)d0[i] * d1[i] * taps[i] != n) { ok = false; break; }
+            t.off = p_off[i]; t.D1 = d1[i]; t.T = taps[i];
+            for (int a = 0; a < d0[i] && ok; a += SGD_TILE_MAX)
+                for (int b = 0; b < d1[i] && ok; b += SGD_TILE_MAX) {
+                    t.d0 = a; t.n0 = std::min(SGD_TILE_MAX, d0[i] - a); t.d1 = b; t.n1 = std::min(SGD_TILE_MAX, d1[i] - b);
+                    t.count = (int64_t)t.n0 * t.n1 * t.T;
+                    for (int j : {jf[i], jd[i]}) {
+                        if (j < 0) continue;
+                        const int64_t u = sgd_tile_units(t, pack_jobs[j]);
+                        if (u < 0) ok = false; else units[j] += u;
+                    }
+                    sgd_tiles.push_back(t);
+                }
+        }
+        for (size_t j = 0; j < pack_jobs.size() && ok; ++j) ok = units[j] == pack_jobs[j].total;
+        if (!ok) { sgd_tiles.clear(); return; }
+        std::stable_sort(sgd_tiles.begin(), sgd_tiles.end(), [](const SgdTile& a, const SgdTile& b) { return a.count > b.count; });
     }
 };
 
@@ -910,6 +967,10 @@
                 HIP_OK(hipMalloc((void**)&p->jobs_dev, p->pack_jobs.size() * sizeof(PackJob)));
                 HIP_OK(hipMemcpy(p->jobs_dev, p->pack_jobs.data(), p->pack_jobs.size() * sizeof(PackJob), hipMemcpyHostToDevice));
             }
+            if (!p->sgd_tiles.empty()) {
+                HIP_OK(hipMalloc((void**)&p->tiles_dev, p->sgd_tiles.size() * sizeof(SgdTile)));
+                HIP_OK(hipMemcpy(p->tiles_dev, p->sgd_tiles.data(), p->sgd_tiles.size() * sizeof(SgdTile), hipMemcpyHostToDevice));
+            }
         }
         *out = p;
         return 0;
@@ -1306,6 +1367,30 @@
         launch_sgd(params, grads, mom, p->n_param_elems, p->segs_dev, p->nseg, partial, nblk, lr, momentum, nesterov, wd, clip_norm,
                    grad_scale, norm_out, s);
         check_launch();
+        return 0;
+    } catch (const std::exception& e) { return fail(e.what()); }
+}
+
+int unet_sgd_step_packed(const unet_plan* p, float* params, float* grads, float* mom, float lr, float momentum, int nesterov, float wd,
+                         float clip_norm, float grad_scale, float* norm_out, void* workspace, int with_dgrad, int* made, void* scratch,
+                         void* stream) {
+    try {
+        if (!p || !params || !grads || !mom || !scratch || !made) throw std::runtime_error("unet_sgd_step_packed: null argument");
+        *made = 0;
+        if (!p->tiles_dev || !p->jobs_dev || !workspace)
+            return unet_sgd_step(p, params, grads, mom, lr, momentum, nesterov, wd, clip_norm, grad_scale, norm_out, scratch, stream);
+        if ((reinterpret_cast<uintptr_t>(params) | reinterpret_cast<uintptr_t>(grads) | reinterpret_cast<uintptr_t>(mom)) & 15)
+            throw std::runtime_error("unet_sgd_step_packed: misaligned buffer");
+        DeviceGuard dg(p->device);
+        hipStream_t s = (hipStream_t)stream;
+        const int nblk = 1024;
+        float* partial = (float*)scratch;
+        launch_sumsq_partial(grads, p->n_param_elems, grad_scale, partial, nblk, s);
+        launch_sgd_pack(params, grads, mom, p->tiles_dev, (int)p->sgd_tiles.size(), p->jobs_dev, workspace, with_dgrad,
+                        p->deep_part_bytes ? (int*)((char*)workspace + p->deep_cnt_off) : nullptr, p->deep_ncnt, partial, nblk, lr, momentum,
+                        nesterov, wd, clip_norm, grad_scale, norm_out, s);
+        check_launch();
+        *made = 1;
         return 0;
     } catch (const std::exception& e) { return fail(e.what()); }
 }
diff --git a/unet-studio_amd/csrc/kernels.h b/unet-studio_amd/csrc/kernels.h
--- a/unet-studio_amd/csrc/kernels.h
+++ b/unet-studio_amd/csrc/kernels.h
@@ -108,7 +108,22 @@
                 float lr, float momentum, int nesterov, float weight_decay, float clip_norm, float grad_scale, float* norm_out,
                 hipStream_t s);
 
+struct PackJob;
+struct SgdTile { int64_t off, count; float wd; int job_fwd, job_dgrad, D1, T, d0, n0, d1, n1, pad; };
+constexpr int SGD_TILE_MAX = 32;
+int64_t sgd_tile_units(const SgdTile& t, const PackJob& job);
+void launch_sgd_pack(float* p, float* g, float* m, const SgdTile* tiles_dev, int ntiles, const PackJob* jobs_dev, void* ws, int with_dgrad,
+                     int* zero, int nzero, const float* partial, int nblk, float lr, float momentum, int nesterov, float weight_decay,
+                     float clip_norm, float grad_scale, float* norm_out, hipStream_t s);
+
 struct PackJob { int64_t src_off, dst_off, total, blk0; int Ci, Co, CK, T, mode, A, B, pad; };
+enum PackMode {
+    PK_CONV_FWD = 0,
+    PK_CONV_DGRAD = 1,
+    PK_CONVT_DGRAD = 2,
+    PK_CONVT_FWD = 3,
+    PK_CONV_S2_DGRAD = 4
+};
 int mfma_conv_pack_jobs(const ConvGeom& g, bool want_dgrad, PackJob* out2);
 int mfma_convt_pack_jobs(const ConvGeom& g, PackJob* out2);
 void launch_mfma_pack_batched(const float* params_base, void* ws, const PackJob* jobs_dev, int njobs, int64_t nblocks, hipStream_t s,
diff --git a/unet-studio_amd/csrc/kernels_elem.hip b/unet-studio_amd/csrc/kernels_elem.hip
--- a/unet-studio_amd/csrc/kernels_elem.hip
+++ b/unet-studio_amd/csrc/kernels_elem.hip
@@ -1,4 +1,5 @@
 #include "device_util.h"
+#include "sgd_update.h"
 
 namespace unet {
 
@@ -1124,24 +1125,9 @@
     __shared__ float s_coef;
     __shared__ int64_t s_off[SGD_MAXSEG];
     __shared__ float s_wd[SGD_MAXSEG];
-    double part = 0.0;
-    for (int b = threadIdx.x; b < nblk; b += 256) part += partial[b];
-    red[threadIdx.x] = part;
     const int ns = nseg < SGD_MAXSEG ? nseg : SGD_MAXSEG;
     for (int k = threadIdx.x; k < ns; k += 256) { s_off[k] = segs[k].offset; s_wd[k] = segs[k].wd; }
-    __syncthreads();
-    for (int o = 128; o > 0; o >>= 1) {
-        if ((int)threadIdx.x < o) red[threadIdx.x] += red[threadIdx.x + o];
-        __syncthreads();
-    }
-    if (threadIdx.x == 0) {
-        float norm = (float)sqrt(red[0]);
-        float coef = clip_norm / (norm + 1e-6f);
-        s_coef = coef > 1.f ? 1.f : coef;
-        if (blockIdx.x == 0 && norm_out) *norm_out = norm;
-    }
-    __syncthreads();
-    const float coef = s_coef * grad_scale;
+    const SgdUpdate upd{sgd_clip_coef(partial, nblk, clip_norm, norm_out, red, &s_coef) * grad_scale, lr, momentum, nesterov};
     auto seg_of = [&](int64_t i) {
         int lo = 0, hi = nseg - 1;
         while (lo < hi) {
@@ -1152,13 +1138,6 @@
         return lo;
     };
     auto wd_of = [&](int sg) { return (sg < SGD_MAXSEG ? s_wd[sg] : segs[sg].wd) * wdecay; };
-    auto upd = [&](float& pv, float& gv, float& mv, float wd) {
-        float d = fmaf(wd, pv, gv * coef);
-        float b = fmaf(momentum, mv, d);
-        mv = b;
-        pv = pv - lr * (nesterov ? fmaf(momentum, b, d) : b);
-        gv = 0.f;
-    };
     const int64_t n4 = n >> 2;
     for (int64_t q = (int64_t)blockIdx.x * 256 + threadIdx.x; q < n4; q += (int64_t)gridDim.x * 256) {
         const int64_t i = q * 4;
diff --git a/unet-studio_amd/csrc/kernels_mfma_conv.hip b/unet-studio_amd/csrc/kernels_mfma_conv.hip
--- a/unet-studio_amd/csrc/kernels_mfma_conv.hip
+++ b/unet-studio_amd/csrc/kernels_mfma_conv.hip
@@ -4,13 +4,6 @@
 
 namespace unet {
 
-enum PackMode {
-    PK_CONV_FWD = 0,
-    PK_CONV_DGRAD = 1,
-    PK_CONVT_DGRAD = 2,
-    PK_CONVT_FWD = 3,
-    PK_CONV_S2_DGRAD = 4
-};
 constexpr int PACK_LDS_ELEMS = 16 * (32 * 27 + 1);
 template <int CK, int T, int MODE>
 __device__ __forceinline__ void pack_unit_t(const float* __restrict__ w, __bf16* __restrict__ out, int unit, int Co, int A, int B, __bf16* lds) {
diff --git a/unet-studio_amd/csrc/kernels_sgd_pack.hip b/unet-studio_amd/csrc/kernels_sgd_pack.hip
--- /dev/null
+++ b/unet-studio_amd/csrc/kernels_sgd_pack.hip
@@ -0,0 +1,145 @@
+#include "mfma_util.h"
+#include "sgd_update.h"
+
+namespace unet {
+
+constexpr int SGDP_THREADS = 512;
+constexpr int SGDP_LDS_ELEMS = SGD_TILE_MAX * (SGD_TILE_MAX * 27 + 1);
+
+struct SgdQuad {
+    float4 p, g, m;
+    int64_t qb;
+    int kind;
+};
+__device__ __forceinline__ void quad_load(SgdQuad& q, const float* p, const float* g, const float* m, int64_t qb, int64_t lo, int64_t hi, bool on) {
+    q.qb = qb;
+    q.kind = !on ? 0 : (qb >= lo && qb + 4 <= hi) ? 1 : 2;
+    q.p = q.g = q.m = make_float4(0.f, 0.f, 0.f, 0.f);
+    if (q.kind == 1) {
+        q.p = *(const float4*)(p + qb); q.g = *(const float4*)(g + qb); q.m = *(const float4*)(m + qb);
+    } else if (q.kind == 2) {
+        float* pv = &q.p.x; float* gv = &q.g.x; float* mv = &q.m.x;
+#pragma unroll
+        for (int e = 0; e < 4; ++e)
+            if (qb + e >= lo && qb + e < hi) { pv[e] = p[qb + e]; gv[e] = g[qb + e]; mv[e] = m[qb + e]; }
+    }
+}
+__device__ __forceinline__ void quad_finish(SgdQuad& q, float* p, float* g, float* m, int64_t lo, int64_t hi, const SgdUpdate& upd, float wd,
+                                            __bf16* row) {
+    if (q.kind == 0) return;
+    upd(q.p.x, q.g.x, q.m.x, wd); upd(q.p.y, q.g.y, q.m.y, wd); upd(q.p.z, q.g.z, q.m.z, wd); upd(q.p.w, q.g.w, q.m.w, wd);
+    const float* pv = &q.p.x; const float* mv = &q.m.x;
+    if (q.kind == 1) {
+        *(float4*)(p + q.qb) = q.p; *(float4*)(m + q.qb) = q.m; *(float4*)(g + q.qb) = q.g;
+    } else {
+#pragma unroll
+        for (int e = 0; e < 4; ++e)
+            if (q.qb + e >= lo && q.qb + e < hi) { p[q.qb + e] = pv[e]; m[q.qb + e] = mv[e]; g[q.qb + e] = 0.f; }
+    }
+    if (row) {
+#pragma unroll
+        for (int e = 0; e < 4; ++e)
+            if (q.qb + e >= lo && q.qb + e < hi) row[q.qb + e - lo] = (__bf16)pv[e];
+    }
+}
+
+__device__ __forceinline__ void tile_pack(const SgdTile& t, const PackJob& jb, const __bf16* lds, int RS, char* ws) {
+    const int CK = jb.CK, T = jb.T, mode = jb.mode;
+    const int KSTEPS = CK == 32 ? T : (T + 1) / 2;
+    const int NTT = jb.Co / 16;
+    const bool row0 = mode == PK_CONV_FWD || mode == PK_CONVT_DGRAD;
+    const int P = (mode == PK_CONVT_FWD || mode == PK_CONV_S2_DGRAD) ? 8 : 1;
+    const int nq = (row0 ? t.n1 : t.n0) / CK, nr = (row0 ? t.n0 : t.n1) / 16;
+    const int q0 = (row0 ? t.d1 : t.d0) / CK;
+    const int plane = mode == PK_CONV_S2_DGRAD ? jb.A : jb.B;
+    __bf16* out = (__bf16*)(ws + jb.dst_off);
+    const int items = P * nq * nr * KSTEPS * 64;
+    for (int it = threadIdx.x; it < items; it += SGDP_THREADS) {
+        const int lane = it & 63, row = lane & 15;
+        int x = it >> 6;
+        const int ks = x % KSTEPS; x /= KSTEPS;
+        const int ri = x % nr; x /= nr;
+        const int qi = x % nq, pp = x / nq;
+        int tap, c0;
+        if (CK == 32) { tap = ks; c0 = 8 * (lane >> 4); }
+        else { tap = 2 * ks + (lane >> 5); c0 = 8 * ((lane >> 4) & 1); }
+        const int rr = ri * 16 + row, cc = qi * CK + c0;
+        int base = -1, step = 0;
+        if (tap < T) {
+            if (row0) { base = rr * RS + cc * t.T + tap; step = t.T; }
+            else if (mode == PK_CONV_DGRAD) { base = cc * RS + rr * 27 + 26 - tap; step = RS; }
+            else if (mode == PK_CONVT_FWD) { base = cc * RS + rr * 8 + pp; step = RS; }
+            else {
+                const int pk[3] = {(pp >> 2) & 1, (pp >> 1) & 1, pp & 1}, kk[3] = {(tap >> 2) & 1, (tap >> 1) & 1, tap & 1};
+                int ft[3];
+                bool ok = true;
+#pragma unroll
+                for (int d = 0; d < 3; ++d) {
+                    if (pk[d] == 0) { ok = ok && kk[d] == 0; ft[d] = 1; }
+                    else ft[d] = kk[d] == 0 ? 2 : 0;
+                }
+                if (ok) { base = cc * RS + rr * 27 + ft[0] * 9 + ft[1] * 3 + ft[2]; step = RS; }
+            }
+        }
+        bf16x8 o;
+#pragma unroll
+        for (int e = 0; e < 8; ++e) o[e] = base >= 0 ? lds[base + e * step] : (__bf16)0.f;
+        const int q = q0 + qi;
+        const int nt = (row0 ? t.d0 : (P == 8 ? pp * plane : 0) + t.d1) / 16 + ri;
+        *(bf16x8*)(out + ((((int64_t)q * KSTEPS + ks) * NTT + nt) * 64 + lane) * 8) = o;
+    }
+}
+
+__global__ void __launch_bounds__(SGDP_THREADS) k_sgd_pack(float* p, float* g, float* m, const SgdTile* __restrict__ tiles,
+                                                           const PackJob* __restrict__ jobs, char* ws, int with_dgrad,
+                                                           int* __restrict__ zero, int nzero, const float* __restrict__ partial, int nblk,
+                                                           float lr, float momentum, int nesterov, float wdecay, float clip_norm,
+                                                           float grad_scale, float* norm_out) {
+    __shared__ double red[256];
+    __shared__ float s_coef;
+    __shared__ __bf16 lds[SGDP_LDS_ELEMS];
+    if (zero && blockIdx.x == 0)
+        for (int i = threadIdx.x; i < nzero; i += SGDP_THREADS) zero[i] = 0;
+    const SgdUpdate upd{sgd_clip_coef(partial, nblk, clip_norm, norm_out, red, &s_coef) * grad_scale, lr, momentum, nesterov};
+    const SgdTile t = tiles[blockIdx.x];
+    const float wd = t.wd * wdecay;
+    const bool filter = t.job_fwd >= 0;
+    const int nrun = filter ? t.n0 : 1;
+    const int64_t len = filter ? (int64_t)t.n1 * t.T : t.count, pitch = filter ? (int64_t)t.D1 * t.T : 0;
+    const int64_t first = filter ? t.off + ((int64_t)t.d0 * t.D1 + t.d1) * t.T : t.off;
+    const int qr = (int)(((first + len + 3) >> 2) - (first >> 2));
+    const int RS = SGD_TILE_MAX * t.T + 1;
+    const int items = nrun * qr;
+    for (int it = threadIdx.x; it < items; it += 2 * SGDP_THREADS) {
+        SgdQuad a, b;
+        const int ib = it + SGDP_THREADS;
+        const int ra = it / qr, rb = ib / qr;
+        const int64_t la = first + ra * pitch, lb = first + rb * pitch;
+        quad_load(a, p, g, m, (la & ~(int64_t)3) + 4 * (it - ra * qr), la, la + len, true);
+        quad_load(b, p, g, m, (lb & ~(int64_t)3) + 4 * (ib - rb * qr), lb, lb + len, ib < items);
+        quad_finish(a, p, g, m, la, la + len, upd, wd, filter ? lds + ra * RS : nullptr);
+        quad_finish(b, p, g, m, lb, lb + len, upd, wd, filter ? lds + rb * RS : nullptr);
+    }
+    if (!filter) return;
+    __syncthreads();
+    tile_pack(t, jobs[t.job_fwd], lds, RS, ws);
+    if (with_dgrad && t.job_dgrad >= 0) tile_pack(t, jobs[t.job_dgrad], lds, RS, ws);
+}
+
+int64_t sgd_tile_units(const SgdTile& t, const PackJob& jb) {
+    const bool row0 = jb.mode == PK_CONV_FWD || jb.mode == PK_CONVT_DGRAD;
+    const int P = (jb.mode == PK_CONVT_FWD || jb.mode == PK_CONV_S2_DGRAD) ? 8 : 1;
+    const int ni = row0 ? t.n1 : t.n0, no = row0 ? t.n0 : t.n1;
+    if (ni % jb.CK || no % 16 || t.d0 % SGD_TILE_MAX || t.d1 % SGD_TILE_MAX) return -1;
+    return (int64_t)P * (ni / jb.CK) * (no / 16);
+}
+
+void launch_sgd_pack(float* p, float* g, float* m, const SgdTile* tiles_dev, int ntiles, const PackJob* jobs_dev, void* ws, int with_dgrad,
+                     int* zero, int nzero, const float* partial, int nblk, float lr, float momentum, int nesterov, float wdecay,
+                     float clip_norm, float grad_scale, float* norm_out, hipStream_t s) {
+    if (ntiles <= 0) return;
+    k_sgd_pack<<<(unsigned)ntiles, SGDP_THREADS, 0, s>>>(p, g, m, tiles_dev, jobs_dev, (char*)ws, with_dgrad, zero, nzero, partial, nblk, lr,
+                                                         momentum, nesterov, wdecay, clip_norm, grad_scale, norm_out);
+}
+
+}
diff --git a/unet-studio_amd/csrc/sgd_update.h b/unet-studio_amd/csrc/sgd_update.h
--- /dev/null
+++ b/unet-studio_amd/csrc/sgd_update.h
@@ -0,0 +1,41 @@
+#pragma once
+#include <hip/hip_runtime.h>
+
+namespace unet {
+
+__device__ __forceinline__ float sgd_clip_coef(const float* __restrict__ partial, int nblk, float clip_norm, float* norm_out, double* red,
+                                               float* s_coef) {
+    const int tid = threadIdx.x;
+    if (tid < 256) {
+        double part = 0.0;
+        for (int b = tid; b < nblk; b += 256) part += partial[b];
+        red[tid] = part;
+    }
+    __syncthreads();
+    for (int o = 128; o > 0; o >>= 1) {
+        if (tid < o) red[tid] += red[tid + o];
+        __syncthreads();
+    }
+    if (tid == 0) {
+        float norm = (float)sqrt(red[0]);
+        float coef = clip_norm / (norm + 1e-6f);
+        *s_coef = coef > 1.f ? 1.f : coef;
+        if (blockIdx.x == 0 && norm_out) *norm_out = norm;
+    }
+    __syncthreads();
+    return *s_coef;
+}
+
+struct SgdUpdate {
+    float coef, lr, momentum;
+    int nesterov;
+    __device__ __forceinline__ void operator()(float& pv, float& gv, float& mv, float wd) const {
+        float d = fmaf(wd, pv, gv * coef);
+        float b = fmaf(momentum, mv, d);
+        mv = b;
+        pv = pv - lr * (nesterov ? fmaf(momentum, b, d) : b);
+        gv = 0.f;
+    }
+};
+
+}
diff --git a/unet-studio_amd/csrc/unet_host.cpp b/unet-studio_amd/csrc/unet_host.cpp
--- a/unet-studio_amd/csrc/unet_host.cpp
+++ b/unet-studio_amd/csrc/unet_host.cpp
@@ -159,6 +159,9 @@
         }
         scratch_ = torch::Tensor();
         std::scoped_lock<std::mutex> lock(plans_mutex_);
+        last_plan_ = packed_plan_ = nullptr;
+        last_ws_ = torch::Tensor();
+        packed_ws_ = torch::Tensor();
         for (auto& kv : plans_) unet_plan_destroy(kv.second);
         plans_.clear();
         if (ws_pool_) ws_pool_->clear();
@@ -245,6 +248,38 @@
         if (e.ev) (void)hipEventDestroy(e.ev);
     };
     return torch::from_blob(e.buf.data_ptr(), e.buf.sizes(), back, e.buf.options());
+}
+
+uint64_t UNet3dImpl::params_stamp(void) const
+{
+    uint64_t s = (uint64_t)reinterpret_cast<uintptr_t>(flat_params.data_ptr()) * 1000003u + flat_params._version();
+    for (auto& p : params_) s = s * 1000003u + p._version();
+    return s;
+}
+
+void UNet3dImpl::drop_packs(void)
+{
+    std::scoped_lock<std::mutex> lock(plans_mutex_);
+    last_plan_ = packed_plan_ = nullptr;
+    last_ws_ = torch::Tensor();
+    packed_ws_ = torch::Tensor();
+}
+
+torch::Tensor UNet3dImpl::training_workspace(unet_plan* plan, int* mode)
+{
+    {
+        std::scoped_lock<std::mutex> lock(plans_mutex_);
+        if (packed_plan_ == plan && packed_ws_.defined() && packed_stamp_ == params_stamp()) {
+            torch::Tensor ws = std::move(packed_ws_);
+            packed_plan_ = nullptr;
+            packed_ws_ = torch::Tensor();
+            *mode |= UNET_MODE_PACKS_CURRENT;
+            return ws;
+        }
+        packed_plan_ = nullptr;
+        packed_ws_ = torch::Tensor();
+    }
+    return workspace_for(plan);
 }
 
 std::vector<torch::Tensor> UNet3dImpl::run_forward(unet_plan* plan, torch::Tensor ws, torch::Tensor x, int mode)
@@ -403,8 +438,9 @@
     ensure_flat();
     auto x = input.to(torch::kFloat32).contiguous();
     unet_plan* plan = plan_for(x.size(2), x.size(3), x.size(4));
-    auto ws = workspace_for(plan);
-    auto outs = run_forward(plan, ws, x, 1);
+    int mode = 1;
+    auto ws = training_workspace(plan, &mode);
+    auto outs = run_forward(plan, ws, x, mode);
     size_t sb = 0;
     unet_loss_scratch_bytes(plan, &sb);
     auto sc = torch::empty({(int64_t)sb}, torch::TensorOptions().dtype(torch::kUInt8).device(x.device()));
@@ -422,6 +458,10 @@
     check(unet_loss(plan, op.data(), t.data_ptr<int64_t>(), mask, collapse_before, gp.data(), losses.data_ptr<float>(), sc.data_ptr(),
                     stream_of(x.device())));
     run_backward(plan, ws, gouts);
+    {
+        std::scoped_lock<std::mutex> lock(plans_mutex_);
+        last_plan_ = plan; last_ws_ = ws;
+    }
     return losses;
 }
 
@@ -430,6 +470,7 @@
     if (!comm_) throw std::runtime_error("broadcast_parameters: no communicator attached");
     ensure_flat();
     void* st = stream_of(flat_params.device());
+    drop_packs();
     check(unet_comm_broadcast(comm_, flat_params.data_ptr<float>(), flat_params.numel(), root, st));
     for (auto& b : buffers_) check(unet_comm_broadcast(comm_, b.data_ptr<float>(), b.numel(), root, st));
     check(unet_comm_join(comm_, st));
@@ -465,8 +506,9 @@
     rebind_grads();
     auto x = input.to(torch::kFloat32).contiguous();
     unet_plan* plan = plan_for(x.size(2), x.size(3), x.size(4));
-    auto ws = workspace_for(plan);
-    auto outs = run_forward(plan, ws, x, 1);
+    int mode = 1;
+    auto ws = training_workspace(plan, &mode);
+    auto outs = run_forward(plan, ws, x, mode);
     size_t sb = 0;
     unet_loss_scratch_bytes(plan, &sb);
     auto sc = torch::empty({(int64_t)sb}, torch::TensorOptions().dtype(torch::kUInt8).device(x.device()));
@@ -501,6 +543,10 @@
         }
         op_hi = op_lo[k]; elem_hi = elem_lo[k];
     }
+    {
+        std::scoped_lock<std::mutex> lock(plans_mutex_);
+        last_plan_ = plan; last_ws_ = ws;
+    }
     return losses;
 }
 
@@ -560,7 +606,26 @@
     bind_optimizer_state();
     if (!scratch_.defined()) scratch_ = torch::empty({65536 + 16}, torch::TensorOptions().dtype(torch::kUInt8).device(flat_params.device()));
     if (plans_.empty()) throw std::runtime_error("sgd_step before any forward");
-    check(unet_sgd_step(plans_.begin()->second, flat_params.data_ptr<float>(), flat_grads.data_ptr<float>(), momentum_.data_ptr<float>(), lr,
-                        0.99f, 1, 3e-5f, clip_norm, grad_scale, (float*)((char*)scratch_.data_ptr() + 65536), scratch_.data_ptr(),
-                        stream_of(flat_params.device())));
-}
+    unet_plan* plan = nullptr;
+    torch::Tensor ws;
+    {
+        std::scoped_lock<std::mutex> lock(plans_mutex_);
+        if (pack_in_update && last_plan_ && last_ws_.defined()) { plan = last_plan_; ws = std::move(last_ws_); }
+        last_plan_ = packed_plan_ = nullptr;
+        last_ws_ = torch::Tensor();
+        packed_ws_ = torch::Tensor();
+    }
+    int made = 0;
+    if (plan)
+        check(unet_sgd_step_packed(plan, flat_params.data_ptr<float>(), flat_grads.data_ptr<float>(), momentum_.data_ptr<float>(), lr, 0.99f, 1,
+                                   3e-5f, clip_norm, grad_scale, (float*)((char*)scratch_.data_ptr() + 65536), ws.data_ptr(), 1, &made,
+                                   scratch_.data_ptr(), stream_of(flat_params.device())));
+    else
+        check(unet_sgd_step(plans_.begin()->second, flat_params.data_ptr<float>(), flat_grads.data_ptr<float>(), momentum_.data_ptr<float>(), lr,
+                            0.99f, 1, 3e-5f, clip_norm, grad_scale, (float*)((char*)scratch_.data_ptr() + 65536), scratch_.data_ptr(),
+                            stream_of(flat_params.device())));
+    if (made) {
+        std::scoped_lock<std::mutex> lock(plans_mutex_);
+        packed_plan_ = plan; packed_ws_ = ws; packed_stamp_ = params_stamp();
+    }
+}
diff --git a/unet-studio_amd/engine.py b/unet-studio_amd/engine.py
--- a/unet-studio_amd/engine.py
+++ b/unet-studio_amd/engine.py
@@ -63,6 +63,7 @@
 _sig("unet_plan_side_cu_range", _i, _vp, _i, _i)
 _sig("unet_pack_filters", _i, _vp, _vp, _vp, _i, _vp, _vp)
 _sig("unet_sgd_step", _i, _vp, _vp, _vp, _vp, _f, _f, _i, _f, _f, _f, _vp, _vp, _vp)
+_sig("unet_sgd_step_packed", _i, _vp, _vp, _vp, _vp, _f, _f, _i, _f, _f, _f, _vp, _vp, _i, _vp, _vp, _vp)
 _sig("unet_set_error", None, C.c_char_p)
 _sig("unet_comm_unique_id", _i, _vp)
 _sig("unet_comm_create", _i, _i, _i, _vp, _i, C.POINTER(_vp))
@@ -94,7 +95,7 @@
     "unet_plan_param_shape", "unet_plan_param_name", "unet_plan_param_decay", "unet_plan_param_fan_in", "unet_plan_buffer_count",
     "unet_plan_buffer_shape", "unet_plan_output_count", "unet_plan_output_shape", "unet_plan_workspace_bytes",
     "unet_plan_flops", "unet_plan_describe", "unet_plan_op_count", "unet_plan_op_info", "unet_profile_begin", "unet_profile_end", "unet_forward", "unet_backward", "unet_backward_part", "unet_plan_backward_buckets", "unet_loss_scratch_bytes", "unet_loss", "unet_forward_loss", "unet_forward_loss_mode", "unet_sum_buffers",
-    "unet_sgd_step", "unet_pack_filters", "unet_stream_create_cu_range", "unet_stream_destroy", "unet_plan_side_cu_range", "unet_set_error", "unet_comm_unique_id", "unet_comm_create", "unet_comm_create_all", "unet_comm_destroy", "unet_comm_rank",
+    "unet_sgd_step", "unet_sgd_step_packed", "unet_pack_filters", "unet_stream_create_cu_range", "unet_stream_destroy", "unet_plan_side_cu_range", "unet_set_error", "unet_comm_unique_id", "unet_comm_create", "unet_comm_create_all", "unet_comm_destroy", "unet_comm_rank",
     "unet_allreduce_grads", "unet_allreduce_grads_all", "unet_comm_broadcast", "unet_comm_join", "unet_op_scratch_bytes", "unet_op_conv3d_fwd", "unet_op_conv3d_fwd_fused", "unet_op_conv3d_pack", "unet_op_conv3d_fwd_packed", "unet_op_conv3d_bwd_data", "unet_op_conv3d_fwd_norm", "unet_op_conv3d_bwd_data_norm", "unet_op_conv3d_bwd_weight",
     "unet_op_convt_fwd", "unet_op_convt_bwd_data", "unet_op_convt_bwd_weight", "unet_op_pack_ndhwc", "unet_op_unpack_ncdhw",
 ]
diff --git a/unet-studio_amd/train.py b/unet-studio_amd/train.py
--- a/unet-studio_amd/train.py
+++ b/unet-studio_amd/train.py
@@ -41,6 +41,7 @@
         self.packs_reuse = hasattr(model, "_run_forward_loss")
         self.in_flight = max(1, int(os.environ.get("UNET_MICRO_IN_FLIGHT", "1")))
         self.pack_after_update = False
+        self.pack_in_update = True
         self._packed_size, self._packed_version = None, None
         self.stats_direct = hasattr(model, "_run_forward_loss")
         self._lanes, self._gbufs, self._gptrs = None, [], []
@@ -131,9 +132,13 @@
             dist.all_reduce(stats, op=dist.ReduceOp.SUM, group=self.group)
             for w in works:
                 w.wait()
-        m.optimizer.step(grad_scale=1.0 / p.batch_size, clip_norm=12.0)
         self._packed_size = None
-        if self.pack_after_update and mine and not lanes_on and m.pack_filters(last_size):
+        if self.pack_in_update and self.packs_reuse and mine and not lanes_on:
+            made = m.optimizer.step(grad_scale=1.0 / p.batch_size, clip_norm=12.0, pack_size=last_size)
+        else:
+            made = False
+            m.optimizer.step(grad_scale=1.0 / p.batch_size, clip_norm=12.0)
+        if made or (self.pack_after_update and mine and not lanes_on and m.pack_filters(last_size)):
             self._packed_size, self._packed_version = last_size, m._params_version
         if self.comm is not None and self.world_size > 1:
             for b in m.buffers():
diff --git a/unet-studio_amd/unet3d.py b/unet-studio_amd/unet3d.py
--- a/unet-studio_amd/unet3d.py
+++ b/unet-studio_amd/unet3d.py
@@ -1,3 +1,4 @@
+import ctypes
 import math
 import threading
 
@@ -25,15 +26,25 @@
         self.last_grad_norm = torch.zeros(1, device=model.flat_params.device, dtype=torch.float32)
         self._scratch = torch.empty(65536, dtype=torch.uint8, device=model.flat_params.device)
 
-    def step(self, grad_scale=1.0, clip_norm=12.0):
+    def step(self, grad_scale=1.0, clip_norm=12.0, pack_size=None):
         m = self.model
         lr = self.param_groups[0]["lr"]
-        plan = m._any_plan()
-        E.check(E.lib.unet_sgd_step(plan.handle, m.flat_params.data_ptr(), m.flat_grads.data_ptr(),
-                                    self.momentum_buffer.data_ptr(), lr, self.momentum, int(self.nesterov),
-                                    self.weight_decay, clip_norm, grad_scale, self.last_grad_norm.data_ptr(),
-                                    self._scratch.data_ptr(), _stream_ptr(m.device())))
+        made = ctypes.c_int(0)
+        if pack_size is not None:
+            plan = m.plan_for(tuple(pack_size))
+            E.check(E.lib.unet_sgd_step_packed(plan.handle, m.flat_params.data_ptr(), m.flat_grads.data_ptr(),
+                                               self.momentum_buffer.data_ptr(), lr, self.momentum, int(self.nesterov),
+                                               self.weight_decay, clip_norm, grad_scale, self.last_grad_norm.data_ptr(),
+                                               m._workspace(plan).data_ptr(), 1, ctypes.byref(made), self._scratch.data_ptr(),
+                                               _stream_ptr(m.device())))
+        else:
+            plan = m._any_plan()
+            E.check(E.lib.unet_sgd_step(plan.handle, m.flat_params.data_ptr(), m.flat_grads.data_ptr(),
+                                        self.momentum_buffer.data_ptr(), lr, self.momentum, int(self.nesterov),
+                                        self.weight_decay, clip_norm, grad_scale, self.last_grad_norm.data_ptr(),
+                                        self._scratch.data_ptr(), _stream_ptr(m.device())))
         m._params_version += 1
+        return bool(made.value)
 
     def zero_grad(self):
         self.model.flat_grads.zero_()
```

Measured after the change: 819.7 million (median of 6 runs). 1.02x the previous value.
